# UBC-ECE-Sasha/PIM-Embedding-Lookup

Hardware: AMD Instinct MI355X
Metric: pooled-lookups/sec + achieved HBM GB/s, 26-table dim-16 Kaggle, 1/2/4/8 GPU (higher is better)
Workload: dtype f32

## Files before the change

include/pimemb.h:

```cpp
#ifndef PIMEMB_H
#define PIMEMB_H

#include <stddef.h>
#include <stdint.h>

#ifdef __cplusplus
extern "C" {
#endif

#define EMB_OK 0
#define EMB_ERR_INVALID (-1)
#define EMB_ERR_NOMEM (-2)
#define EMB_ERR_DEVICE (-3)
#define EMB_ERR_UNSUPPORTED (-4)
#define EMB_ERR_RANGE (-5)

typedef enum emb_dtype {
    EMB_F32 = 0,
    EMB_F16 = 1,
    EMB_FIXED32 = 2,
    EMB_BF16 = 3
} emb_dtype;
#define EMB_F8_E4M3 ((emb_dtype)8)
#define EMB_F8_E5M2 ((emb_dtype)9)
#define EMB_MXFP4 ((emb_dtype)10)
#define EMB_MXFP4_ROW_BYTES(dim) ((dim) / 2u + (dim) / 32u)
#define EMB_MXFP4_ROW_STRIDE(dim) ((EMB_MXFP4_ROW_BYTES(dim) + 15u) & ~15u)

typedef enum emb_index_type { EMB_IDX_U32 = 0, EMB_IDX_I64 = 1 } emb_index_type;

typedef enum emb_memspace {
    EMB_MEM_HOST = 0,
    EMB_MEM_DEVICE = 1
} emb_memspace;

typedef struct emb_engine emb_engine;
typedef struct emb_plan emb_plan;

typedef struct emb_config {
    int32_t device;
    uint32_t max_tables;
    uint32_t flags;
} emb_config;
#define EMB_FLAG_STAGE_TIMING 1u
#define EMB_FLAG_CHECK_INPUTS 2u
#define EMB_FLAG_DEFER_CHECK 4u

typedef struct emb_lookup_desc {
    uint32_t table_id;
    uint32_t fixed_pooling;
    const void *indices;
    const void *offsets;
    uint64_t n_indices;
    uint64_t n_bags;
    float *pooled;
} emb_lookup_desc;

typedef struct emb_stats {
    uint64_t n_lookup_calls;
    uint64_t n_kernel_launches;
    uint64_t n_bags;
    uint64_t n_indices;
    uint64_t table_bytes;
    double us_copy_in_indices;
    double us_copy_in_lengths;
    double us_launch;
    double us_copy_out;
    double us_post_process;
    double us_sync;
    uint64_t n_launches_by_kind[5];
} emb_stats;


const char *emb_last_error(void);

const char *emb_version(void);

int emb_create(const emb_config *cfg, emb_engine **out);

int emb_destroy(emb_engine *e);

int emb_load_table(emb_engine *e, uint32_t table_id, uint64_t nr_rows, uint32_t dim, emb_dtype dtype,
                   const void *rows, emb_memspace space);

int emb_alloc_table(emb_engine *e, uint32_t table_id, uint64_t nr_rows, uint32_t dim, emb_dtype dtype);

int emb_load_table_column(emb_engine *e, uint32_t table_id, uint32_t col, const int32_t *column,
                          uint64_t nr_rows);

int emb_set_hot_rows(emb_engine *e, uint32_t table_id, const uint64_t *row_ids, uint32_t n_rows);
int emb_learn_hot_rows(emb_engine *e, uint32_t table_id, const void *indices, uint64_t n_indices, emb_index_type itype,
                       emb_memspace space, uint32_t max_rows, float min_share, void *stream, uint32_t *n_chosen, float *share);

int emb_table_info(emb_engine *e, uint32_t table_id, void **device_rows, uint64_t *nr_rows,
                   uint32_t *dim, emb_dtype *dtype);

int emb_lookup(emb_engine *e, uint32_t table_id, const void *indices, uint64_t n_indices,
               const void *offsets, uint64_t n_bags, float *pooled, emb_index_type itype,
               emb_memspace space, void *stream);

int emb_lookup_batched(emb_engine *e, const emb_lookup_desc *descs, uint32_t n_descs,
                       emb_index_type itype, emb_memspace space, void *stream);

int emb_lookup_ranged(emb_engine *e, const emb_lookup_desc *descs, const uint64_t *row_lo, uint32_t n_descs, void *stream);
int emb_plan_create_ranged(emb_engine *e, const emb_lookup_desc *descs, const uint64_t *row_lo, uint32_t n_descs,
                           emb_plan **out);
#define EMB_SERVED_LANES 64u
#define EMB_SERVED_STRIDE 256u
#define EMB_SERVED_BYTES (EMB_SERVED_LANES * EMB_SERVED_STRIDE)
int emb_lookup_ranged_counted(emb_engine *e, const emb_lookup_desc *descs, const uint64_t *row_lo, uint32_t *const *served,
                              uint32_t n_descs, void *stream);
int emb_plan_create_ranged_counted(emb_engine *e, const emb_lookup_desc *descs, const uint64_t *row_lo,
                                   uint32_t *const *served, uint32_t n_descs, emb_plan **out);
#define EMB_RANGE_OPEN_END (1ull << 63)
int emb_lookup_ranged_typed(emb_engine *e, const emb_lookup_desc *descs, const uint64_t *row_lo, uint32_t *const *served,
                            uint32_t n_descs, emb_index_type itype, void *stream);
int emb_plan_create_ranged_typed(emb_engine *e, const emb_lookup_desc *descs, const uint64_t *row_lo, uint32_t *const *served,
                                 uint32_t n_descs, emb_index_type itype, emb_plan **out);

int emb_plan_create(emb_engine *e, const emb_lookup_desc *descs, uint32_t n_descs,
                    emb_index_type itype, emb_plan **out);
int emb_plan_launch(emb_plan *p, void *stream);
int emb_plan_destroy(emb_plan *p);
int emb_plan_bytes(const emb_plan *p, uint64_t *algorithmic_bytes, uint64_t *n_bags,
                   uint64_t *n_indices);
int emb_plan_signature(const emb_plan *p, uint64_t *signature);
int emb_plan_describe(const emb_plan *p, char *buf, size_t capacity);
int emb_plan_time(emb_plan *p, void *stream, uint32_t warmup, uint32_t iters, float *avg_us);

#define EMB_POOL_SUM 0u
#define EMB_POOL_MEAN 1u
#define EMB_POOL_MAX 2u
#define EMB_POOL_PADDING 1u
#define EMB_POOL_OUT_TABLE_DTYPE 2u
typedef struct emb_pool_spec {
    uint32_t mode;
    uint32_t flags;
    const float *per_sample_weights;
    int64_t padding_idx;
} emb_pool_spec;
int emb_lookup_pooled(emb_engine *e, const emb_lookup_desc *descs, const emb_pool_spec *pools, uint32_t n_descs,
                      emb_index_type itype, emb_memspace space, void *stream, uint32_t check, uint64_t *n_bad);
int emb_plan_create_pooled(emb_engine *e, const emb_lookup_desc *descs, const emb_pool_spec *pools, uint32_t n_descs,
                           emb_index_type itype, emb_plan **out);

int emb_validate_inputs(emb_engine *e, const emb_lookup_desc *descs, uint32_t n_descs,
                        emb_index_type itype, emb_memspace space, uint64_t *n_bad);
int emb_validate_inputs_on(emb_engine *e, const emb_lookup_desc *descs, uint32_t n_descs,
                           emb_index_type itype, emb_memspace space, void *stream, uint64_t *n_bad);
int emb_lookup_batched_checked(emb_engine *e, const emb_lookup_desc *descs, uint32_t n_descs,
                               emb_index_type itype, emb_memspace space, void *stream, uint64_t *n_bad);
int emb_lookup_batched_checked_deferred(emb_engine *e, const emb_lookup_desc *descs, uint32_t n_descs,
                                        emb_index_type itype, emb_memspace space, void *stream);
int emb_check_report(emb_engine *e, uint64_t *n_bad);

int emb_get_stats(emb_engine *e, emb_stats *out);
int emb_reset_stats(emb_engine *e);
int emb_set_stage_timing(emb_engine *e, int on);

#define EMB_STAGE_COPY_IN 0
#define EMB_STAGE_DESCRIPTORS 1
#define EMB_STAGE_LAUNCH 2
#define EMB_STAGE_COPY_OUT 3
#define EMB_STAGE_SYNC 4
typedef struct emb_trace_event {
    uint32_t stage;
    uint32_t call_id;
    double start_us;
    double stop_us;
} emb_trace_event;
int emb_trace_enable(emb_engine *e, uint32_t capacity);
int emb_trace_read(emb_engine *e, emb_trace_event *out, uint32_t max_events, uint32_t *n_events);

int emb_device_alloc(emb_engine *e, size_t bytes, void **out);
int emb_device_free(emb_engine *e, void *ptr);
int emb_copy_to_device(emb_engine *e, void *dst_device, const void *src_host, size_t bytes);
int emb_copy_to_host(emb_engine *e, void *dst_host, const void *src_device, size_t bytes);
int emb_memset_device(emb_engine *e, void *dst_device, int value, size_t bytes);
int emb_synchronize(emb_engine *e, void *stream);
int emb_stream_create(emb_engine *e, void **stream);
int emb_stream_destroy(emb_engine *e, void *stream);
int emb_device_of(emb_engine *e, int32_t *device);

typedef struct emb_queue emb_queue;
int emb_queue_create(emb_engine *e, emb_index_type itype, emb_memspace space, emb_queue **out);
int emb_queue_add(emb_queue *q, const emb_lookup_desc *descs, uint32_t n_descs, uint64_t *ticket);
int emb_queue_add_many(emb_queue *q, const emb_lookup_desc *descs, const uint32_t *n_descs, uint32_t n_requests,
                       uint64_t *first_ticket);
int emb_queue_flush(emb_queue *q, void *stream, uint32_t *n_requests);
int emb_queue_wait(emb_queue *q, uint64_t ticket);
int emb_queue_destroy(emb_queue *q);

typedef struct emb_route_table {
    const void *indices;
    const void *offsets;
    uint64_t n_indices;
    uint32_t fixed_pooling;
    uint32_t rows_per_shard;
} emb_route_table;
int emb_route_bags_sizes(uint32_t n_tables, uint64_t n_bags, uint64_t total_indices, uint32_t n_shards,
                         uint64_t *send_bytes, uint64_t *meta_bytes, uint64_t *slots_bytes, uint64_t *work_bytes);
int emb_route_bags(emb_engine *e, const emb_route_table *tables , uint32_t n_tables,
                   uint64_t n_bags, uint32_t n_shards, void *send, uint32_t *meta, uint32_t *slots,
                   void *work, void *stream);
int emb_route_bags_typed(emb_engine *e, const emb_route_table *tables , uint32_t n_tables,
                         emb_index_type itype, uint64_t n_bags, uint32_t n_shards, void *send, uint32_t *meta,
                         uint32_t *slots, void *work, void *stream);
int emb_unroute_bags(emb_engine *e, const float *recv, const uint32_t *meta, const uint32_t *slots,
                     uint32_t n_tables, uint64_t n_bags, uint32_t n_shards, uint32_t dim,
                     float *pooled , void *stream);

int emb_route_exchange_sizes(const uint32_t *sent, const uint32_t *received, uint32_t n_tables, uint32_t n_shards,
                             uint32_t dim, uint64_t *req_out_words, uint64_t *req_in_words, uint64_t *ret_rows_back,
                             uint64_t *ret_rows_served, uint64_t *peak_req_bytes, uint64_t *peak_ret_bytes);
int emb_route_serve_descs(const uint32_t *received, uint32_t n_tables, uint32_t n_shards, uint32_t dim,
                          const uint32_t *shard_table_ids, const void *req_recv, float *ret_send,
                          emb_lookup_desc *descs, uint32_t *n_descs, uint64_t *algorithmic_bytes);

typedef struct emb_comm emb_comm;
int emb_comm_unique_id(void *id128);
int emb_comm_create(emb_engine *e, const void *id128, int32_t rank, int32_t world, emb_comm **out);
int emb_comm_all_to_all(emb_comm *c, const void *send, const uint64_t *send_off, void *recv,
                        const uint64_t *recv_off, void *stream);
int emb_comm_destroy(emb_comm *c);

typedef struct emb_comm_op {
    int32_t peer;
    int32_t is_recv;
    void *ptr;
    uint64_t bytes;
} emb_comm_op;
int emb_comm_exchange(emb_comm *c, const emb_comm_op *ops, uint32_t n_ops, void *stream);
int emb_comm_rank(const emb_comm *c, int32_t *rank, int32_t *world);

typedef struct emb_peer emb_peer;
int emb_peer_create(emb_engine *e, const char *job_tag, int32_t rank, int32_t world, uint64_t arena_bytes, emb_peer **out);
int emb_peer_alloc(emb_peer *p, uint64_t bytes, void **ptr);
int emb_peer_info(emb_peer *p, int32_t *rank, int32_t *world, void **arena, uint64_t *arena_bytes, uint64_t *used,
                  int32_t *fine_grained);
int emb_peer_barrier(emb_peer *p);
int emb_peer_destroy(emb_peer *p);
int emb_peer_last_words(const char *line, int fd, int status);

typedef struct emb_shard emb_shard;
#define EMB_PLACE_REPLICATED 0u
#define EMB_PLACE_WHOLE 1u
#define EMB_PLACE_ROWS 2u
typedef struct emb_shard_table {
    uint32_t placement;
    int32_t owner;
    uint32_t engine_table;
    uint32_t rows_per_shard;
} emb_shard_table;
typedef struct emb_shard_input {
    const void *indices;
    const void *offsets;
    uint64_t n_indices;
    uint32_t fixed_pooling;
    uint32_t index_type;
    float *pooled;
} emb_shard_input;
#define EMB_SHARD_SELF_VIA_COMM 1u
#define EMB_SHARD_CHECK_SERVED 2u
#define EMB_SHARD_PEER_STORES 4u
#define EMB_SHARD_NO_DIRECT 8u
#define EMB_SHARD_DEFER_REPORT 16u
typedef struct emb_shard_config {
    uint32_t n_tables;
    uint32_t dim;
    uint32_t depth;
    uint32_t flags;
    const emb_shard_table *tables;
    emb_peer *peer;
} emb_shard_config;
typedef struct emb_shard_stats {
    uint64_t n_batches;
    uint64_t bytes_to_peers;
    uint64_t bytes_to_self;
    uint64_t served_algorithmic_bytes;
    uint64_t local_algorithmic_bytes;
    uint64_t served_sub_bags, served_indices;
    double us_host_submit;
    double us_host_wait_counts;
    double us_host_wait_served;
    double us_kernel_route, us_kernel_local, us_kernel_serve, us_kernel_unroute;
    uint64_t n_timed_batches;
    double us_kernel_direct;
} emb_shard_stats;
int emb_shard_create(emb_engine *e, emb_comm *comm, const emb_shard_config *cfg, emb_shard **out);
int emb_shard_submit(emb_shard *s, const emb_shard_input *in, uint64_t n_bags, void *stream, uint64_t *seq);
int emb_shard_flush(emb_shard *s);
int emb_shard_wait(emb_shard *s, uint64_t seq, void *stream);
int emb_shard_lookup(emb_shard *s, const emb_shard_input *in, uint64_t n_bags, void *stream);
int emb_shard_report(emb_shard *s);
int emb_shard_get_stats(emb_shard *s, emb_shard_stats *out, int reset);
int emb_shard_set_kernel_timing(emb_shard *s, int on);
int emb_shard_sent_counts(emb_shard *s, uint64_t seq, uint32_t *counts, uint32_t capacity_words);
int emb_shard_destroy(emb_shard *s);


struct dpu_set_t;

typedef struct dpu_runtime_totals {
    double execution_time_prepare;
    double execution_time_populate_copy_in;
    double execution_time_copy_in;
    double execution_time_copy_out;
    double execution_time_aggregate_result;
    double execution_time_launch;
} dpu_runtime_totals;

int emb_configure(uint32_t nr_tables, uint32_t nr_cols, uint32_t max_nr_batches,
                  uint32_t max_indices_per_batch);

struct dpu_set_t *populate_mram(uint32_t table_id, uint64_t nr_rows, uint32_t col,
                                int32_t *table_data, dpu_runtime_totals *runtime);

int32_t *lookup(uint32_t **indices, uint32_t **offsets, float **final_results,
                void *dpu_set_ptr_untyped, int64_t latency_print);

emb_engine *emb_compat_engine(void);
int emb_compat_reset(void);

#ifdef __cplusplus
}
#endif
#endif
```

pim-embedding-lookup_amd/csrc/pimemb_engine.cpp:

```cpp
#include <algorithm>
#include <atomic>
#include <chrono>
#include <condition_variable>
#include <cstdarg>
#include <cstdio>
#include <cstring>
#include <deque>
#include <map>
#include <mutex>
#include <new>
#include <string>
#include <thread>
#include <tuple>
#include <utility>
#include <unordered_map>
#include <vector>

#include "pimemb_hostcopy.h"
#include "pimemb_hot_rows.h"
#include "pimemb_internal.h"
#include "pimemb_xcd_map.h"

namespace pimemb {
hipError_t launch_store_word(volatile unsigned long long *dst, unsigned long long value, hipStream_t stream);
}
using pimemb::DevDesc;
using pimemb::KernelKind;
using pimemb::LaunchGeom;

namespace {

thread_local std::string g_last_error;
using pimemb::fail;

#define HIP_TRY(expr)                                                                       \
    do {                                                                                    \
        hipError_t _e = (expr);                                                             \
        if (_e != hipSuccess)                                                               \
            return fail(_e == hipErrorOutOfMemory ? EMB_ERR_NOMEM : EMB_ERR_DEVICE,         \
                        "%s failed: %s (%s:%d)", #expr, hipGetErrorString(_e), __FILE__,    \
                        __LINE__);                                                          \
    } while (0)
#define EMB_TRY(expr)                  \
    do {                               \
        int _rc = (expr);              \
        if (_rc != EMB_OK) return _rc; \
    } while (0)

double now_us() {
    using namespace std::chrono;
    return duration<double, std::micro>(steady_clock::now().time_since_epoch()).count();
}

size_t row_stride(int dtype, uint32_t dim) { return (size_t)pimemb::row_stride_bytes(dtype, dim); }
size_t index_size(emb_index_type t) { return t == EMB_IDX_I64 ? 8 : 4; }

struct Table {
    void *rows = nullptr;
    uint64_t nr_rows = 0;
    uint32_t dim = 0;
    int dtype = EMB_F32;
    LaunchGeom geom{};
    size_t bytes = 0;
    uint64_t generation = 0;
    void *hot_rows = nullptr;
    uint64_t *hot_hash = nullptr;
    uint32_t n_hot = 0, hot_log2 = 0;
    size_t hot_lds = 0;
};

struct DescSlot {
    char *h = nullptr;
    char *d = nullptr;
    size_t cap = 0;
    size_t used = 0;
    hipStream_t stream = nullptr;
    hipEvent_t done = nullptr;
    bool pending = false;
};
constexpr int kSlots = 4;
constexpr size_t kSlotBytes = 256u << 10;
constexpr int kRingPool = 8;
inline int ring_of_thread() {
    static const bool one = getenv("PIMEMB_RING_POOL") && atoi(getenv("PIMEMB_RING_POOL")) == 1;
    return one ? 0 : (int)(std::hash<std::thread::id>()(std::this_thread::get_id()) % (size_t)kRingPool);
}
struct ImageRing {
    DescSlot slots[kSlots];
    int next_slot = 0;
    int desc_mode = 1;
    unsigned slot_flags = 0;
    void release() {
        for (DescSlot &sl : slots) {
            if (sl.h) (void)hipHostFree(sl.h);
            if (sl.d) (void)hipFree(sl.d);
            if (sl.done) (void)hipEventDestroy(sl.done);
            sl = DescSlot{};
        }
    }
};

struct XmapCacheEntry {
    std::vector<uint64_t> key;
    uint32_t *d_map = nullptr;
    uint32_t xgrid = 0;
    bool direct = false;
    uint64_t last_use = 0;
    size_t bytes = 0;
    hipStream_t streams[4] = {};
    uint32_t n_streams = 0;
    bool many_streams = false;
};
struct XmapGrave {
    uint32_t *d_map = nullptr;
    size_t bytes = 0;
    hipEvent_t ev[4] = {};
    uint32_t n_ev = 0;
    bool needs_device_wait = false;
};
constexpr size_t kXmapCacheEntries = 32;
constexpr size_t kXmapSeenEntries = 256;
constexpr size_t kXmapGraveBytes = 64u << 20;

}

struct emb_engine {
    int device = 0;
    std::vector<Table> tables;
    std::mutex mu;
    std::mutex host_mu;
    pimemb::HostCopier copier;
    hipEvent_t pipe_ev[4] = {};
    hipStream_t host_s2 = nullptr;
    hipEvent_t split_ev[2] = {};
    ImageRing ring[kRingPool];
    std::mutex ring_mu[kRingPool];
    std::vector<XmapCacheEntry> xmap_cache;
    uint64_t xmap_clock = 0;
    std::vector<uint64_t> xmap_seen;
    size_t xmap_seen_at = 0;
    std::vector<XmapGrave> xmap_graveyard;
    size_t xmap_grave_bytes = 0;
    char *h_stage = nullptr;
    size_t h_stage_cap = 0;
    char *d_stage = nullptr;
    size_t d_stage_cap = 0;
    static constexpr uint32_t kValSlots = 64;
    pimemb::ValidateCtl *d_val = nullptr;
    unsigned long long val_seq = 0;
    struct PendingVerdict {
        unsigned long long seq;
        hipStream_t stream;
        uint32_t n_groups;
        KernelKind kinds[8];
        bool launched;
    };
    std::deque<PendingVerdict> val_pending;
    bool defer_check = false;
    unsigned long long val_owed_bad = 0, val_owed_first = 0;
    std::mutex val_mu;
    volatile unsigned long long *val_result = nullptr;
    volatile unsigned long long *host_done = nullptr;
    unsigned long long host_seq = 0;
    std::atomic<uint64_t> n_lookup_calls{0}, n_kernel_launches{0}, n_bags{0}, n_indices{0};
    std::atomic<uint64_t> n_by_kind[5] = {};
    uint64_t table_bytes = 0;
    double us_copy_in_indices = 0, us_copy_in_lengths = 0, us_launch = 0, us_copy_out = 0,
           us_sync = 0;
    bool stage_timing = false;
    bool check_inputs = false;
    std::atomic<uint32_t> live_plans{0};
    uint64_t next_generation = 1;
    std::deque<emb_trace_event> trace;
    uint32_t trace_cap = 0;
    uint32_t host_call_id = 0;
    void record(uint32_t stage, double a, double b) {
        if (!trace_cap) return;
        if (trace.size() >= trace_cap) trace.pop_front();
        trace.push_back(emb_trace_event{stage, host_call_id, a, b});
    }
};

struct PlanGroup {
    DevDesc *d_descs = nullptr;
    uint32_t n = 0;
    uint32_t max_tiles = 0;
    int dtype = EMB_F32;
    LaunchGeom geom{};
    KernelKind kind = pimemb::KERNEL_WAVEBATCH;
    uint32_t *d_xmap = nullptr;
    uint32_t xgrid = 0;
    bool xdirect = false;
    uint32_t hot_wgs = 0;
    uint32_t hot_lds = 0;
    uint32_t *cached_xmap = nullptr;
    bool ranged = false;
    uint32_t pool = 0;
    uint32_t n_weighted = 0, n_padding = 0;
    bool out_half = false;
    size_t desc_off = 0, xmap_off = 0;
    std::vector<uint32_t> xmap_words;
};

struct emb_plan {
    emb_engine *e = nullptr;
    emb_index_type itype = EMB_IDX_U32;
    std::vector<PlanGroup> groups;
    char *d_image = nullptr;
    uint64_t bytes = 0, n_bags = 0, n_indices = 0;
    uint64_t signature = 0;
    std::vector<std::pair<uint32_t, uint64_t>> table_gens;
};

namespace {

void clear_hot(Table &t) {
    if (t.hot_rows) (void)hipFree(t.hot_rows);
    if (t.hot_hash) (void)hipFree(t.hot_hash);
    t.hot_rows = nullptr;
    t.hot_hash = nullptr;
    t.n_hot = t.hot_log2 = 0;
    t.hot_lds = 0;
}

struct DeviceGuard {
    int prev = -1;
    bool switched = false;
    explicit DeviceGuard(int dev) {
        if (hipGetDevice(&prev) == hipSuccess && prev != dev) {
            switched = hipSetDevice(dev) == hipSuccess;
        }
    }
    ~DeviceGuard() {
        if (switched) (void)hipSetDevice(prev);
    }
};

struct Resolved {
    std::vector<DevDesc> descs;
    std::vector<PlanGroup> groups;
    uint64_t bytes = 0, n_bags = 0, n_indices = 0;
    std::vector<char> image;
    hipStream_t stream = nullptr;

    void build_image() {
        size_t off = 0, di = 0;
        for (PlanGroup &g : groups) {
            g.desc_off = off;
            off += sizeof(DevDesc) * g.n;
        }
        for (PlanGroup &g : groups) {
            g.xmap_off = off;
            off += (g.xmap_words.size() * 4 + 63) / 64 * 64;
        }
        image.assign(off ? off : 64, 0);
        for (PlanGroup &g : groups) {
            memcpy(image.data() + g.desc_off, descs.data() + di, sizeof(DevDesc) * g.n);
            di += g.n;
            if (!g.xmap_words.empty())
                memcpy(image.data() + g.xmap_off, g.xmap_words.data(), g.xmap_words.size() * 4);
        }
    }
    void bind(char *d_base) {
        for (PlanGroup &g : groups) {
            g.d_descs = reinterpret_cast<DevDesc *>(d_base + g.desc_off);
            g.d_xmap = g.cached_xmap ? g.cached_xmap
                       : g.xmap_words.empty() ? nullptr : reinterpret_cast<uint32_t *>(d_base + g.xmap_off);
        }
    }
};

void reap_xmap_graveyard(emb_engine *e, bool wait_oldest) {
    size_t kept = 0;
    for (size_t i = 0; i < e->xmap_graveyard.size(); i++) {
        XmapGrave &gv = e->xmap_graveyard[i];
        const bool over = wait_oldest && e->xmap_grave_bytes > kXmapGraveBytes;
        bool done = !gv.needs_device_wait;
        if (gv.needs_device_wait && over) done = hipDeviceSynchronize() == hipSuccess;
        for (uint32_t k = 0; k < gv.n_ev && done; k++) {
            hipError_t q = over ? hipEventSynchronize(gv.ev[k]) : hipEventQuery(gv.ev[k]);
            if (q != hipSuccess) {
                (void)hipGetLastError();
                done = false;
            }
        }
        if (done) {
            for (uint32_t k = 0; k < gv.n_ev; k++) (void)hipEventDestroy(gv.ev[k]);
            (void)hipFree(gv.d_map);
            e->xmap_grave_bytes -= gv.bytes;
        } else {
            e->xmap_graveyard[kept++] = gv;
        }
    }
    e->xmap_graveyard.resize(kept);
}

int cached_xcd_map(emb_engine *e, PlanGroup &g, uint32_t bpt, const std::vector<uint32_t> &tiles_of,
                   const std::vector<uint64_t> &bytes_of, hipStream_t stream) {
    std::vector<uint64_t> key;
    key.reserve(2 + 2 * tiles_of.size());
    key.push_back((uint64_t)g.kind);
    key.push_back(bpt);
    for (size_t i = 0; i < tiles_of.size(); i++) {
        key.push_back(tiles_of[i]);
        key.push_back(bytes_of[i]);
    }
    static const bool cache_off = getenv("PIMEMB_XMAP_CACHE") && atoi(getenv("PIMEMB_XMAP_CACHE")) == 0;
    if (cache_off) return EMB_ERR_UNSUPPORTED;
    std::lock_guard<std::mutex> lk(e->mu);
    ++e->xmap_clock;
    auto note_stream = [stream](XmapCacheEntry &c) {
        for (uint32_t k = 0; k < c.n_streams; k++)
            if (c.streams[k] == stream) return;
        if (c.n_streams < 4) c.streams[c.n_streams++] = stream;
        else c.many_streams = true;
    };
    for (XmapCacheEntry &c : e->xmap_cache)
        if (c.key == key) {
            c.last_use = e->xmap_clock;
            note_stream(c);
            g.cached_xmap = c.d_map;
            g.xgrid = c.xgrid;
            g.xdirect = c.direct;
            return EMB_OK;
        }
    uint64_t h = 1469598103934665603ull;
    for (uint64_t v : key) h = (h ^ v) * 1099511628211ull;
    bool seen = false;
    for (uint64_t v : e->xmap_seen) seen = seen || v == h;
    if (!seen) {
        if (e->xmap_seen.size() < kXmapSeenEntries) e->xmap_seen.push_back(h);
        else e->xmap_seen[e->xmap_seen_at++ % kXmapSeenEntries] = h;
        return EMB_ERR_UNSUPPORTED;
    }
    size_t victim = 0;
    if (e->xmap_cache.size() >= kXmapCacheEntries) {
        for (size_t i = 1; i < e->xmap_cache.size(); i++)
            if (e->xmap_cache[i].last_use < e->xmap_cache[victim].last_use) victim = i;
        if (e->xmap_clock - e->xmap_cache[victim].last_use < 4 * kXmapCacheEntries) return EMB_ERR_UNSUPPORTED;
    }
    XmapCacheEntry n;
    std::vector<uint32_t> words;
    n.xgrid = pimemb::build_xcd_map(tiles_of, bytes_of, &words, 1);
    if (n.xgrid <= (1u << 20)) {
        std::vector<uint32_t> direct;
        pimemb::expand_xcd_map(words, n.xgrid, &direct);
        words.swap(direct);
        n.direct = true;
    }
    if (hipMalloc((void **)&n.d_map, words.size() * 4) != hipSuccess) return EMB_ERR_NOMEM;
    if (hipMemcpy(n.d_map, words.data(), words.size() * 4, hipMemcpyHostToDevice) != hipSuccess) {
        (void)hipFree(n.d_map);
        return EMB_ERR_DEVICE;
    }
    if (e->xmap_cache.size() >= kXmapCacheEntries) {
        const XmapCacheEntry &v = e->xmap_cache[victim];
        XmapGrave gv;
        gv.d_map = v.d_map;
        gv.bytes = v.bytes;
        gv.needs_device_wait = v.many_streams;
        for (uint32_t k = 0; k < v.n_streams && !gv.needs_device_wait; k++) {
            hipEvent_t ev = nullptr;
            if (hipEventCreateWithFlags(&ev, hipEventDisableTiming) == hipSuccess && hipEventRecord(ev, v.streams[k]) == hipSuccess) {
                gv.ev[gv.n_ev++] = ev;
            } else {
                if (ev) (void)hipEventDestroy(ev);
                (void)hipGetLastError();
                gv.needs_device_wait = true;
            }
        }
        e->xmap_grave_bytes += gv.bytes;
        e->xmap_graveyard.push_back(gv);
        e->xmap_cache.erase(e->xmap_cache.begin() + (long)victim);
        reap_xmap_graveyard(e, true);
    }
    n.key.swap(key);
    n.bytes = words.size() * 4;
    note_stream(n);
    n.last_use = e->xmap_clock;
    g.cached_xmap = n.d_map;
    g.xgrid = n.xgrid;
    g.xdirect = n.direct;
    e->xmap_cache.push_back(std::move(n));
    return EMB_OK;
}

bool is_plain_sum(const emb_pool_spec &ps) {
    return ps.mode == EMB_POOL_SUM && ps.per_sample_weights == nullptr && ps.flags == 0;
}
bool is_plain_sum_half_out(const emb_pool_spec &ps) {
    return ps.mode == EMB_POOL_SUM && ps.per_sample_weights == nullptr && ps.flags == EMB_POOL_OUT_TABLE_DTYPE;
}
bool wants_half_out(const emb_pool_spec *pools, uint32_t i) { return pools && (pools[i].flags & EMB_POOL_OUT_TABLE_DTYPE) != 0; }
size_t out_elem_size(const emb_pool_spec *pools, uint32_t i) { return wants_half_out(pools, i) ? 2 : 4; }

int resolve(emb_engine *e, const emb_lookup_desc *descs, uint32_t n_descs, emb_index_type itype,
            const std::vector<const void *> *st_indices, const std::vector<const void *> *st_offsets,
            const std::vector<float *> *st_out, Resolved *r, bool cache_maps = false, const uint64_t *row_lo = nullptr,
            uint32_t *const *served = nullptr, const emb_pool_spec *pools = nullptr,
            const std::vector<const float *> *st_weights = nullptr) {
    if (itype != EMB_IDX_U32 && itype != EMB_IDX_I64) return fail(EMB_ERR_INVALID, "bad index type");
    std::map<std::tuple<int, uint32_t, uint32_t, uint32_t>, std::vector<uint32_t>> by_shape;
    for (uint32_t i = 0; i < n_descs; i++) {
        const emb_lookup_desc &u = descs[i];
        if (u.table_id >= e->tables.size() || e->tables[u.table_id].rows == nullptr)
            return fail(EMB_ERR_INVALID, "desc %u: table %u is not loaded", i, u.table_id);
        if (u.n_bags > 0 && u.pooled == nullptr) return fail(EMB_ERR_INVALID, "desc %u: pooled is NULL", i);
        if (u.n_indices > 0 && u.indices == nullptr)
            return fail(EMB_ERR_INVALID, "desc %u: indices is NULL", i);
        if (u.offsets == nullptr) {
            if (u.n_bags > 0 && u.fixed_pooling == 0)
                return fail(EMB_ERR_INVALID, "desc %u: offsets is NULL and fixed_pooling is 0", i);
            if ((uint64_t)u.fixed_pooling * u.n_bags != u.n_indices)
                return fail(EMB_ERR_INVALID, "desc %u: fixed_pooling*n_bags != n_indices", i);
        }
        const Table &t = e->tables[u.table_id];
        if (row_lo) {
            if (u.offsets != nullptr || u.fixed_pooling != 1)
                return fail(EMB_ERR_INVALID, "ranged lookup: desc %u: one index per bag only (offsets NULL, fixed_pooling 1)", i);
            if (t.geom.scalar_lanes)
                return fail(EMB_ERR_UNSUPPORTED, "ranged lookup: desc %u: rows must be 16-byte multiples up to 1 KiB", i);
            if (t.dtype == pimemb::kMXFP4)
                return fail(EMB_ERR_UNSUPPORTED, "ranged lookup: desc %u: table %u is MXFP4, which the lane-group kernels serve only "
                            "(no ranged, counted or typed lookup)", i, u.table_id);
        }
        uint32_t pool_kind = 0;
        if (pools && !is_plain_sum(pools[i])) {
            const emb_pool_spec &ps = pools[i];
            if (ps.mode > EMB_POOL_MAX || (ps.flags & ~(EMB_POOL_PADDING | EMB_POOL_OUT_TABLE_DTYPE)) != 0)
                return fail(EMB_ERR_INVALID, "desc %u: bad pooling spec (mode %u, flags 0x%x)", i, ps.mode, ps.flags);
            if ((ps.flags & EMB_POOL_OUT_TABLE_DTYPE) && t.dtype == pimemb::kMXFP4)
                return fail(EMB_ERR_UNSUPPORTED, "desc %u: EMB_POOL_OUT_TABLE_DTYPE: table %u is MXFP4, whose pooled rows are fp32 only", i, u.table_id);
            if ((ps.flags & EMB_POOL_OUT_TABLE_DTYPE) && t.dtype != EMB_F16 && t.dtype != EMB_BF16)
                return fail(EMB_ERR_UNSUPPORTED, "desc %u: EMB_POOL_OUT_TABLE_DTYPE needs an fp16 or bf16 table (table %u has dtype %d)", i,
                            u.table_id, (int)t.dtype);
            if (ps.per_sample_weights != nullptr && ps.mode != EMB_POOL_SUM)
                return fail(EMB_ERR_INVALID, "desc %u: per_sample_weights need EMB_POOL_SUM (as in torch)", i);
            if (t.dtype == EMB_FIXED32)
                return fail(EMB_ERR_UNSUPPORTED, "desc %u: fixed-point tables pool by plain sum only", i);
            if ((ps.flags & EMB_POOL_PADDING) && (ps.padding_idx < 0 || (uint64_t)ps.padding_idx >= t.nr_rows))
                return fail(EMB_ERR_INVALID, "desc %u: padding_idx %lld outside table %u (%llu rows)", i, (long long)ps.padding_idx,
                            u.table_id, (unsigned long long)t.nr_rows);
            if (row_lo) return fail(EMB_ERR_UNSUPPORTED, "ranged lookups pool by plain sum only");
            if (!is_plain_sum_half_out(ps)) pool_kind = 1u + ps.mode;
        }
        by_shape[{(int)t.dtype, t.dim, pool_kind, wants_half_out(pools, i) ? 1u : 0u}].push_back(i);
    }
    const size_t isz = index_size(itype);
    for (auto &kv : by_shape) {
        PlanGroup g;
        g.dtype = std::get<0>(kv.first);
        g.pool = std::get<2>(kv.first);
        g.out_half = std::get<3>(kv.first) != 0;
        g.n = (uint32_t)kv.second.size();
        const Table &t0 = e->tables[descs[kv.second[0]].table_id];
        g.geom = t0.geom;
        uint64_t group_bags = 0, group_idx = 0;
        for (uint32_t i : kv.second) {
            group_bags += descs[i].n_bags;
            group_idx += descs[i].n_indices;
        }
        g.kind = pimemb::choose_kernel(group_bags, group_idx, g.geom);
        {
            static const char *force = getenv("PIMEMB_FORCE_KERNEL");
            if (force && g.kind != pimemb::KERNEL_ANYDIM && group_idx <= 2 * group_bags)
                g.kind = force[0] == 'g' ? pimemb::KERNEL_GROUP : pimemb::KERNEL_WAVEBATCH;
        }
        if (g.dtype == pimemb::kMXFP4) g.kind = pimemb::KERNEL_GROUP;
        g.ranged = row_lo != nullptr;
        if (g.ranged && g.kind == pimemb::KERNEL_GROUP) g.kind = pimemb::KERNEL_WAVEBATCH;
        if (g.pool && g.kind == pimemb::KERNEL_WAVEBATCH2) g.kind = pimemb::KERNEL_WAVEBATCH;
        if (g.kind == pimemb::KERNEL_GROUP && !g.pool && !g.out_half) {
            for (uint32_t i : kv.second) {
                const Table &t = e->tables[descs[i].table_id];
                if (t.n_hot && t.hot_lds > g.hot_lds) g.hot_lds = (uint32_t)t.hot_lds;
            }
            if (g.hot_lds) g.kind = pimemb::KERNEL_HOT;
        }
        const uint32_t bpt = pimemb::bags_per_tile(g.kind, g.geom);
        std::vector<uint32_t> tiles_of;
        std::vector<uint64_t> bytes_of;
        for (uint32_t i : kv.second) {
            const emb_lookup_desc &u = descs[i];
            const Table &t = e->tables[u.table_id];
            uint64_t tiles = (u.n_bags + bpt - 1) / bpt;
            if (tiles > 0x0fffffffull) return fail(EMB_ERR_UNSUPPORTED, "desc %u: too many bags", i);
            DevDesc d{};
            d.weights = t.rows;
            d.indices = st_indices ? (*st_indices)[i] : u.indices;
            d.offsets = st_offsets ? (*st_offsets)[i] : u.offsets;
            d.out = st_out ? (*st_out)[i] : u.pooled;
            d.n_idx = u.n_indices;
            d.n_bags = u.n_bags;
            d.nr_rows = t.nr_rows;
            d.fixed_pooling = u.offsets ? 0u : u.fixed_pooling;
            d.n_tiles = (uint32_t)tiles;
            if (row_lo) d.ranged.row_lo = row_lo[i];
            if (row_lo && served) d.ranged.served = served[i];
            if (g.pool) {
                const emb_pool_spec &ps = pools[i];
                const bool weighted = ps.per_sample_weights != nullptr, padded = (ps.flags & EMB_POOL_PADDING) != 0;
                const uint32_t op = ps.mode == EMB_POOL_MAX ? pimemb::kPoolOpMax
                                    : !weighted          ? pimemb::kPoolOpAdd
                                    : padded             ? pimemb::kPoolOpMulAdd
                                                         : pimemb::kPoolOpFma;
                d.pool.weights = st_weights && weighted ? (*st_weights)[i] : ps.per_sample_weights;
                d.pool.padding_row = padded ? (uint64_t)ps.padding_idx : ~0ull;
                d.pool.op = op | (ps.mode == EMB_POOL_MEAN ? pimemb::kPoolMean : 0u);
                g.n_weighted += weighted;
                g.n_padding += padded;
                if (weighted) r->bytes += u.n_indices * 4;
            }
            if (g.kind == pimemb::KERNEL_HOT) {
                d.hot_rows = t.hot_rows;
                d.hot_hash = t.hot_hash;
                d.n_hot = t.n_hot;
                d.hot_log2 = t.hot_log2;
            }
            if (d.n_tiles > g.max_tiles) g.max_tiles = d.n_tiles;
            tiles_of.push_back(d.n_tiles);
            bytes_of.push_back(t.bytes);
            r->descs.push_back(d);
            r->n_bags += u.n_bags;
            r->n_indices += u.n_indices;
            r->bytes += u.n_indices * ((uint64_t)row_stride(t.dtype, t.dim) + isz) +
                        (u.offsets ? u.n_bags * isz : 0) + u.n_bags * (uint64_t)t.dim * (g.out_half ? 2 : 4);
        }
        if (g.n > 1 && g.max_tiles > 0 &&
            (g.kind == pimemb::KERNEL_WAVEBATCH || g.kind == pimemb::KERNEL_WAVEBATCH2)) {
            if (cache_maps)
                for (uint32_t &v : tiles_of)
                    if (v > 16) {
                        uint32_t q = 1;
                        while ((q << 1) <= v) q <<= 1;
                        q >>= 4;
                        v = (v + q - 1) / q * q;
                    }
            uint64_t total_tiles = 0;
            for (uint32_t t : tiles_of) total_tiles += t;
            if (total_tiles + 8 * (uint64_t)g.n > 0x7fffffffull)
                return fail(EMB_ERR_UNSUPPORTED, "launch too large for one grid");
            if (!cache_maps || cached_xcd_map(e, g, bpt, tiles_of, bytes_of, r->stream) != EMB_OK) {
                g.xgrid = pimemb::build_xcd_map(tiles_of, bytes_of, &g.xmap_words, 1);
                if (g.xgrid <= (1u << 20)) {
                    std::vector<uint32_t> direct;
                    pimemb::expand_xcd_map(g.xmap_words, g.xgrid, &direct);
                    g.xmap_words.swap(direct);
                    g.xdirect = true;
                }
            }
        } else if (g.n > 65535u) {
            return fail(EMB_ERR_UNSUPPORTED, "more than 65535 descriptors of one shape");
        }
        if (g.kind == pimemb::KERNEL_HOT) {
            static const uint32_t total = getenv("PIMEMB_HOT_WGS_TOTAL") ? (uint32_t)atoi(getenv("PIMEMB_HOT_WGS_TOTAL")) : 8192u;
            const uint32_t cap = g.max_tiles / 2u ? g.max_tiles / 2u : 1u;
            uint32_t w = total / g.n;
            g.hot_wgs = w < 1u ? 1u : (w > cap ? cap : w);
        }
        r->groups.push_back(std::move(g));
    }
    r->build_image();
    return EMB_OK;
}

int launch_groups(emb_engine *e, const std::vector<PlanGroup> &groups, emb_index_type itype,
                  hipStream_t s) {
    for (const PlanGroup &g : groups) {
        if (g.pool)
            HIP_TRY(pimemb::launch_bag_pool(g.d_descs, g.n, g.max_tiles, g.dtype, itype, g.geom, g.kind, g.d_xmap, g.xgrid,
                                            g.xdirect, s, g.out_half));
        else if (g.kind == pimemb::KERNEL_HOT)
            HIP_TRY(pimemb::launch_bag_sum_hot(g.d_descs, g.n, g.hot_wgs, g.hot_lds, g.dtype, itype, g.geom, s));
        else
            HIP_TRY(pimemb::launch_bag_sum(g.d_descs, g.n, g.max_tiles, g.dtype, itype, g.geom, g.kind, g.d_xmap,
                                           g.xgrid, g.xdirect, s, g.ranged, g.out_half));
        e->n_kernel_launches.fetch_add(1, std::memory_order_relaxed);
        e->n_by_kind[g.kind].fetch_add(1, std::memory_order_relaxed);
    }
    return EMB_OK;
}

int take_image_space(ImageRing &r, size_t n, hipStream_t s, char **h, char **d) {
    n = (n + 127) / 128 * 128;
    DescSlot *sl = &r.slots[r.next_slot];
    if (sl->used && (sl->used + n > sl->cap || sl->stream != s)) {
        if (hipEventRecord(sl->done, sl->stream) == hipSuccess) {
            sl->pending = true;
            r.next_slot = (r.next_slot + 1) % kSlots;
            sl = &r.slots[r.next_slot];
        } else {
            (void)hipGetLastError();
            HIP_TRY(hipDeviceSynchronize());
            sl->used = 0;
        }
    }
    if (sl->pending) {
        HIP_TRY(hipEventSynchronize(sl->done));
        sl->pending = false;
        sl->used = 0;
    }
    if (sl->cap < n) {
        if (sl->used) {
            HIP_TRY(hipDeviceSynchronize());
            sl->used = 0;
        }
        if (sl->h) (void)hipHostFree(sl->h);
        if (sl->d) (void)hipFree(sl->d);
        sl->h = nullptr;
        sl->d = nullptr;
        sl->cap = 0;
        const size_t cap = n < kSlotBytes ? kSlotBytes : n + n / 4;
        HIP_TRY(hipHostMalloc((void **)&sl->h, cap, r.slot_flags));
        if (r.desc_mode == 0) HIP_TRY(hipMalloc((void **)&sl->d, cap));
        sl->cap = cap;
    }
    if (!sl->done) HIP_TRY(hipEventCreateWithFlags(&sl->done, hipEventDisableTiming));
    *h = sl->h + sl->used;
    *d = sl->d ? sl->d + sl->used : nullptr;
    sl->used += n;
    sl->stream = s;
    return EMB_OK;
}

struct HostProfile {
    bool on = getenv("PIMEMB_HOST_PROFILE") != nullptr;
    double resolve = 0, slot = 0, image = 0, h2d = 0, launch = 0;
    uint64_t calls = 0;
};
HostProfile g_prof;

int launch_resolved(emb_engine *e, Resolved &r, emb_index_type itype, hipStream_t s,
                    bool descriptors_in_host_memory = false) {
    if (r.descs.empty()) return EMB_OK;
    const int rk = ring_of_thread();
    std::lock_guard<std::mutex> lk(e->ring_mu[rk]);
    const double p0 = g_prof.on ? now_us() : 0;
    char *h = nullptr, *d = nullptr;
    int rc = take_image_space(e->ring[rk], r.image.size(), s, &h, &d);
    if (rc) return rc;
    const double p1 = g_prof.on ? now_us() : 0;
    memcpy(h, r.image.data(), r.image.size());
    const double p2 = g_prof.on ? now_us() : 0;
    if (d == nullptr || descriptors_in_host_memory) {
        r.bind(h);
    } else {
        HIP_TRY(hipMemcpyAsync(d, h, r.image.size(), hipMemcpyHostToDevice, s));
        r.bind(d);
    }
    const double p3 = g_prof.on ? now_us() : 0;
    rc = launch_groups(e, r.groups, itype, s);
    if (rc) return rc;
    if (g_prof.on) {
        g_prof.slot += p1 - p0; g_prof.image += p2 - p1; g_prof.h2d += p3 - p2; g_prof.launch += now_us() - p3;
        g_prof.calls++;
    }
    return EMB_OK;
}

int ensure_stage(emb_engine *e, size_t h_bytes, size_t d_bytes) {
    if (e->h_stage_cap < h_bytes) {
        if (e->h_stage) (void)hipHostFree(e->h_stage);
        e->h_stage = nullptr;
        e->h_stage_cap = 0;
        size_t cap = h_bytes + h_bytes / 4 + 4096;
        HIP_TRY(hipHostMalloc((void **)&e->h_stage, cap, hipHostMallocMapped | hipHostMallocCoherent));
        e->h_stage_cap = cap;
    }
    if (e->d_stage_cap < d_bytes) {
        if (e->d_stage) (void)hipFree(e->d_stage);
        e->d_stage = nullptr;
        e->d_stage_cap = 0;
        size_t cap = d_bytes + d_bytes / 4 + 4096;
        HIP_TRY(hipMalloc((void **)&e->d_stage, cap));
        e->d_stage_cap = cap;
        if (cap >= (8u << 20) && !e->host_s2) {
            HIP_TRY(hipStreamCreateWithFlags(&e->host_s2, hipStreamNonBlocking));
            for (hipEvent_t &ev : e->split_ev)
                if (!ev) HIP_TRY(hipEventCreateWithFlags(&ev, hipEventDisableTiming));
            HIP_TRY(pimemb::launch_zero_words(reinterpret_cast<uint32_t *>(e->d_stage), 1, e->host_s2));
            HIP_TRY(hipStreamSynchronize(e->host_s2));
        }
    }
    return EMB_OK;
}

size_t align_up(size_t v, size_t a) { return (v + a - 1) / a * a; }

struct HostStage {
    std::vector<const void *> d_indices, d_offsets;
    std::vector<const float *> d_weights;
    std::vector<float *> d_out;
    size_t in_bytes = 0, out_bytes = 0;
    char *h_out = nullptr;
    bool zero_copy = false;
    bool h2d_deferred = false;
};

static const size_t kZeroCopyBytes = getenv("PIMEMB_ZERO_COPY_BYTES") ? strtoull(getenv("PIMEMB_ZERO_COPY_BYTES"), nullptr, 10) : (40u << 20);
static const size_t kStagedOutBytes = kZeroCopyBytes > (1u << 20) ? kZeroCopyBytes : (1u << 20);
static const size_t kFastPieceBytes = getenv("PIMEMB_FAST_PIECE_BYTES") ? strtoull(getenv("PIMEMB_FAST_PIECE_BYTES"), nullptr, 10) : 1500000;

static const size_t kSplitInBytes = getenv("PIMEMB_HOST_SPLIT_BYTES") ? strtoull(getenv("PIMEMB_HOST_SPLIT_BYTES"), nullptr, 10) : (1u << 20);

int stage_host_inputs(emb_engine *e, const emb_lookup_desc *descs, uint32_t n, emb_index_type itype,
                      hipStream_t s, HostStage *hs, bool with_outputs, bool allow_zero_copy = false, bool allow_split = false,
                      const emb_pool_spec *pools = nullptr) {
    const size_t isz = index_size(itype);
    size_t in_bytes = 0, out_bytes = 0, min_piece = SIZE_MAX;
    for (uint32_t i = 0; i < n; i++) {
        if (descs[i].table_id >= e->tables.size() || !e->tables[descs[i].table_id].rows)
            return fail(EMB_ERR_INVALID, "desc %u: table %u is not loaded", i, descs[i].table_id);
        in_bytes += align_up(descs[i].n_indices * isz, 16);
        if (descs[i].offsets) in_bytes += align_up(descs[i].n_bags * isz, 16);
        if (pools && pools[i].per_sample_weights) in_bytes += align_up(descs[i].n_indices * 4, 16);
        const size_t piece = descs[i].n_bags * (size_t)e->tables[descs[i].table_id].dim * out_elem_size(pools, i);
        out_bytes += align_up(piece, 16);
        if (piece && piece < min_piece) min_piece = piece;
    }
    const bool fast_pieces = min_piece != SIZE_MAX && min_piece >= kFastPieceBytes;
    if (!with_outputs) out_bytes = 0;
    const size_t h_out_bytes = (out_bytes <= kStagedOutBytes && !fast_pieces) ? out_bytes : 0;
    int rc = ensure_stage(e, in_bytes + h_out_bytes, in_bytes + out_bytes);
    if (rc) return rc;
    hs->h_out = h_out_bytes ? e->h_stage + in_bytes : nullptr;
    hs->zero_copy = allow_zero_copy && with_outputs && h_out_bytes == out_bytes && !fast_pieces &&
                    in_bytes + out_bytes <= kZeroCopyBytes;
    char *in_base = hs->zero_copy ? e->h_stage : e->d_stage;
    size_t off = 0;
    hs->d_indices.resize(n);
    hs->d_offsets.resize(n);
    hs->d_weights.assign(n, nullptr);
    hs->d_out.resize(n);
    std::vector<pimemb::CopyPiece> pack;
    pack.reserve(3 * n);
    for (uint32_t i = 0; i < n; i++) {
        const emb_lookup_desc &u = descs[i];
        if (u.n_indices && !u.indices) return fail(EMB_ERR_INVALID, "desc %u: indices is NULL", i);
        pack.push_back({e->h_stage + off, u.indices, u.n_indices * isz});
        hs->d_indices[i] = in_base + off;
        off += align_up(u.n_indices * isz, 16);
        if (u.offsets) {
            pack.push_back({e->h_stage + off, u.offsets, u.n_bags * isz});
            hs->d_offsets[i] = in_base + off;
            off += align_up(u.n_bags * isz, 16);
        } else {
            hs->d_offsets[i] = nullptr;
        }
        if (pools && pools[i].per_sample_weights) {
            pack.push_back({e->h_stage + off, pools[i].per_sample_weights, u.n_indices * 4});
            hs->d_weights[i] = reinterpret_cast<const float *>(in_base + off);
            off += align_up(u.n_indices * 4, 16);
        }
    }
    e->copier.copy(pack);
    size_t oo = in_bytes;
    for (uint32_t i = 0; i < n; i++) {
        hs->d_out[i] = reinterpret_cast<float *>((hs->zero_copy ? e->h_stage : e->d_stage) + oo);
        if (with_outputs)
            oo += align_up(descs[i].n_bags * (size_t)e->tables[descs[i].table_id].dim * out_elem_size(pools, i), 16);
    }
    hs->in_bytes = in_bytes;
    hs->out_bytes = out_bytes;
    hs->h2d_deferred = allow_split && !hs->zero_copy && with_outputs && fast_pieces && n >= 2 && in_bytes >= kSplitInBytes;
    if (in_bytes && !hs->zero_copy && !hs->h2d_deferred)
        HIP_TRY(hipMemcpyAsync(e->d_stage, e->h_stage, in_bytes, hipMemcpyHostToDevice, s));
    return EMB_OK;
}

constexpr size_t kPipelineBytes = 4u << 20;

int lookup_host_pipelined(emb_engine *e, const emb_lookup_desc *descs, uint32_t n, emb_index_type itype,
                          hipStream_t s, const HostStage &hs, double t0) {
    auto piece = [&](uint32_t i) { return descs[i].n_bags * (size_t)e->tables[descs[i].table_id].dim * 4; };
    const uint32_t parts = n < 4 ? n : 4;
    uint32_t bounds[5] = {0, 0, 0, 0, 0};
    {
        size_t acc = 0;
        uint32_t k = 1;
        for (uint32_t i = 0; i < n && k < parts; i++) {
            acc += piece(i);
            if (acc * parts >= hs.out_bytes * k && n - (i + 1) >= parts - k) bounds[k++] = i + 1;
        }
        for (; k < parts; k++) bounds[k] = bounds[k - 1] + 1;
        bounds[parts] = n;
    }
    uint64_t bags = 0, idx = 0;
    for (uint32_t k = 0; k < parts; k++) {
        const uint32_t lo = bounds[k], cnt = bounds[k + 1] - lo;
        std::vector<const void *> di(hs.d_indices.begin() + lo, hs.d_indices.begin() + lo + cnt);
        std::vector<const void *> dof(hs.d_offsets.begin() + lo, hs.d_offsets.begin() + lo + cnt);
        std::vector<float *> dout(hs.d_out.begin() + lo, hs.d_out.begin() + lo + cnt);
        Resolved r;
        r.stream = s;
        int rc = resolve(e, descs + lo, cnt, itype, &di, &dof, &dout, &r, true);
        if (rc == EMB_OK) rc = launch_resolved(e, r, itype, s, true);
        if (rc) {
            (void)hipStreamSynchronize(s);
            return rc;
        }
        if (!e->pipe_ev[k]) HIP_TRY(hipEventCreateWithFlags(&e->pipe_ev[k], hipEventDisableTiming));
        HIP_TRY(hipEventRecord(e->pipe_ev[k], s));
        bags += r.n_bags;
        idx += r.n_indices;
    }
    std::vector<pimemb::CopyPiece> unpack;
    for (uint32_t k = 0; k < parts; k++) {
        HIP_TRY(hipEventSynchronize(e->pipe_ev[k]));
        unpack.clear();
        for (uint32_t i = bounds[k]; i < bounds[k + 1]; i++)
            if (piece(i)) unpack.push_back({descs[i].pooled, hs.d_out[i], piece(i)});
        e->copier.copy(unpack);
    }
    e->us_sync += now_us() - t0;
    e->n_bags.fetch_add(bags, std::memory_order_relaxed);
    e->n_indices.fetch_add(idx, std::memory_order_relaxed);
    return EMB_OK;
}

int lookup_host_split(emb_engine *e, const emb_lookup_desc *descs, uint32_t n, emb_index_type itype, hipStream_t s, const HostStage &hs, double t0) {
    if (!e->host_s2) HIP_TRY(hipStreamCreateWithFlags(&e->host_s2, hipStreamNonBlocking));
    for (hipEvent_t &ev : e->split_ev)
        if (!ev) HIP_TRY(hipEventCreateWithFlags(&ev, hipEventDisableTiming));
    const char *in_base = e->d_stage;
    auto in_off = [&](uint32_t i) { return i < n ? (size_t)(static_cast<const char *>(hs.d_indices[i]) - in_base) : hs.in_bytes; };
    auto out_bytes_of = [&](uint32_t i) { return descs[i].n_bags * (double)e->tables[descs[i].table_id].dim * 4.0; };
    uint32_t m = 1;
    {
        double best = 1e300, out_a = 0;
        for (uint32_t c = 1; c < n; c++) {
            out_a += out_bytes_of(c - 1);
            const double in_a = (double)in_off(c), in_b = (double)hs.in_bytes - in_a, out_b = (double)hs.out_bytes - out_a;
            const double second_ready = in_b / 53e3 + 30.0, first_out = out_a / 46e3;
            const double total = in_a / 53e3 + 20.0 + (first_out > second_ready ? first_out : second_ready) + out_b / 46e3;
            if (total < best) {
                best = total;
                m = c;
            }
        }
    }
    const uint32_t bounds[3] = {0, m, n};
    hipStream_t on[2] = {s, e->host_s2};
    HIP_TRY(hipEventRecord(e->split_ev[0], s));
    HIP_TRY(hipStreamWaitEvent(e->host_s2, e->split_ev[0], 0));
    uint64_t bags = 0, idx = 0;
    for (uint32_t k = 0; k < 2; k++) {
        const uint32_t lo = bounds[k], cnt = bounds[k + 1] - lo;
        const size_t b0 = in_off(lo), b1 = in_off(bounds[k + 1]);
        int rc = EMB_OK;
        if (b1 > b0 && hipMemcpyAsync(e->d_stage + b0, e->h_stage + b0, b1 - b0, hipMemcpyHostToDevice, on[k]) != hipSuccess)
            rc = fail(EMB_ERR_DEVICE, "host-pointer call: copy-in of part %u failed: %s", k, hipGetErrorString(hipGetLastError()));
        std::vector<const void *> di(hs.d_indices.begin() + lo, hs.d_indices.begin() + lo + cnt);
        std::vector<const void *> dof(hs.d_offsets.begin() + lo, hs.d_offsets.begin() + lo + cnt);
        std::vector<float *> dout(hs.d_out.begin() + lo, hs.d_out.begin() + lo + cnt);
        Resolved r;
        r.stream = on[k];
        if (rc == EMB_OK) rc = resolve(e, descs + lo, cnt, itype, &di, &dof, &dout, &r, true);
        if (rc == EMB_OK) rc = launch_resolved(e, r, itype, on[k], false);
        if (rc) {
            (void)hipStreamSynchronize(s);
            (void)hipStreamSynchronize(e->host_s2);
            return rc;
        }
        bags += r.n_bags;
        idx += r.n_indices;
    }
    hipError_t err = hipEventRecord(e->split_ev[1], e->host_s2);
    for (uint32_t k = 0; k < 2 && err == hipSuccess; k++) {
        if (k == 1) err = hipStreamWaitEvent(s, e->split_ev[1], 0);
        for (uint32_t i = bounds[k]; i < bounds[k + 1] && err == hipSuccess; i++) {
            const size_t bytes = descs[i].n_bags * (size_t)e->tables[descs[i].table_id].dim * 4;
            if (bytes) err = hipMemcpyAsync(descs[i].pooled, hs.d_out[i], bytes, hipMemcpyDeviceToHost, s);
        }
    }
    if (err == hipSuccess) err = hipStreamSynchronize(s);
    if (err != hipSuccess) {
        (void)hipStreamSynchronize(e->host_s2);
        (void)hipStreamSynchronize(s);
        return fail(EMB_ERR_DEVICE, "host-pointer call (two parts): %s", hipGetErrorString(err));
    }
    e->us_sync += now_us() - t0;
    e->n_bags.fetch_add(bags, std::memory_order_relaxed);
    e->n_indices.fetch_add(idx, std::memory_order_relaxed);
    return EMB_OK;
}

int lookup_host(emb_engine *e, const emb_lookup_desc *descs, uint32_t n, emb_index_type itype,
                hipStream_t s, const emb_pool_spec *pools = nullptr) {
    std::lock_guard<std::mutex> host_lk(e->host_mu);
    const bool timed = e->stage_timing || e->trace_cap != 0;
    HostStage hs;
    const double t0 = now_us();
    {
        std::lock_guard<std::mutex> lk(e->mu);
        int rc = stage_host_inputs(e, descs, n, itype, s, &hs, true, true, !timed && !pools, pools);
        if (rc) return rc;
    }
    if (hs.h2d_deferred) return lookup_host_split(e, descs, n, itype, s, hs, t0);
    if (timed) HIP_TRY(hipStreamSynchronize(s));
    const double t1 = now_us();
    if (hs.zero_copy && !timed && hs.out_bytes >= kPipelineBytes && n >= 2 && !pools)
        return lookup_host_pipelined(e, descs, n, itype, s, hs, t0);
    Resolved r;
    r.stream = s;
    int rc = resolve(e, descs, n, itype, &hs.d_indices, &hs.d_offsets, &hs.d_out, &r, true, nullptr, nullptr,
                     pools, &hs.d_weights);
    if (rc) return rc;
    rc = launch_resolved(e, r, itype, s, hs.zero_copy);
    if (rc) return rc;
    const double t2 = now_us();
    if (timed) HIP_TRY(hipStreamSynchronize(s));
    const double t3 = now_us();
    const bool staged_out = hs.out_bytes > 0 && hs.out_bytes <= kStagedOutBytes && hs.h_out != nullptr;
    if (hs.zero_copy) {
    } else if (staged_out) {
        HIP_TRY(hipMemcpyAsync(hs.h_out, hs.d_out[0], hs.out_bytes, hipMemcpyDeviceToHost, s));
    } else {
        for (uint32_t i = 0; i < n; i++) {
            size_t bytes = descs[i].n_bags * (size_t)e->tables[descs[i].table_id].dim * out_elem_size(pools, i);
            if (bytes)
                HIP_TRY(hipMemcpyAsync(descs[i].pooled, hs.d_out[i], bytes, hipMemcpyDeviceToHost, s));
        }
    }
    const double t4 = now_us();
    if (hs.zero_copy && !timed) {
        if (!e->host_done) {
            void *p = nullptr;
            HIP_TRY(hipHostMalloc(&p, 64, hipHostMallocMapped | hipHostMallocCoherent));
            e->host_done = static_cast<volatile unsigned long long *>(p);
            *e->host_done = 0;
        }
        const unsigned long long seq = ++e->host_seq;
        HIP_TRY(pimemb::launch_store_word(e->host_done, seq, s));
        bool done = false;
        for (int spin = 0; spin < 400000 && !(done = *e->host_done == seq); spin++) {
        }
        if (!done) HIP_TRY(hipStreamSynchronize(s));
    } else {
        HIP_TRY(hipStreamSynchronize(s));
    }
    if (staged_out) {
        std::vector<pimemb::CopyPiece> unpack;
        unpack.reserve(n);
        for (uint32_t i = 0; i < n; i++) {
            size_t bytes = descs[i].n_bags * (size_t)e->tables[descs[i].table_id].dim * out_elem_size(pools, i);
            if (bytes)
                unpack.push_back({descs[i].pooled, hs.h_out + (reinterpret_cast<char *>(hs.d_out[i]) -
                                                                reinterpret_cast<char *>(hs.d_out[0])), bytes});
        }
        e->copier.copy(unpack);
    }
    const double t5 = now_us();
    if (timed) {
        e->us_copy_in_indices += t1 - t0;
        e->us_copy_in_lengths += t2 - t1;
        e->us_launch += t3 - t2;
        e->us_copy_out += t4 - t3;
        e->us_sync += t5 - t4;
        if (e->trace_cap) {
            std::lock_guard<std::mutex> lk(e->mu);
            e->record(EMB_STAGE_COPY_IN, t0, t1);
            e->record(EMB_STAGE_DESCRIPTORS, t1, t2);
            e->record(EMB_STAGE_LAUNCH, t2, t3);
            e->record(EMB_STAGE_COPY_OUT, t3, t4);
            e->record(EMB_STAGE_SYNC, t4, t5);
            e->host_call_id++;
        }
    } else {
        e->us_sync += t5 - t0;
    }
    e->n_bags.fetch_add(r.n_bags, std::memory_order_relaxed);
    e->n_indices.fetch_add(r.n_indices, std::memory_order_relaxed);
    return EMB_OK;
}

}

int pimemb::fail(int code, const char *fmt, ...) {
    char buf[512];
    va_list ap;
    va_start(ap, fmt);
    vsnprintf(buf, sizeof buf, fmt, ap);
    va_end(ap);
    g_last_error = buf;
    return code;
}

extern "C" {

const char *emb_last_error(void) { return g_last_error.c_str(); }

const char *emb_version(void) { return "pimemb 0.1 gfx950"; }

int emb_create(const emb_config *cfg, emb_engine **out) {
    if (!out) return fail(EMB_ERR_INVALID, "emb_create: out is NULL");
    *out = nullptr;
    int dev = cfg ? cfg->device : -1;
    int count = 0;
    HIP_TRY(hipGetDeviceCount(&count));
    if (count <= 0) return fail(EMB_ERR_DEVICE, "emb_create: no HIP device visible");
    if (dev < 0) HIP_TRY(hipGetDevice(&dev));
    if (dev >= count) return fail(EMB_ERR_INVALID, "emb_create: device %d of %d", dev, count);
    emb_engine *e = new (std::nothrow) emb_engine();
    if (!e) return fail(EMB_ERR_NOMEM, "emb_create: out of host memory");
    e->device = dev;
    e->stage_timing = cfg && (cfg->flags & EMB_FLAG_STAGE_TIMING);
    e->check_inputs = cfg && (cfg->flags & EMB_FLAG_CHECK_INPUTS);
    e->defer_check = cfg && (cfg->flags & EMB_FLAG_DEFER_CHECK);
    {
        const char *m = getenv("PIMEMB_DESC_MODE");
        for (ImageRing &rg : e->ring) {
            rg.desc_mode = (m && m[0] == 'c') ? 0 : 1;
            rg.slot_flags = hipHostMallocMapped | hipHostMallocCoherent;
        }
    }
    uint32_t max_tables = (cfg && cfg->max_tables) ? cfg->max_tables : 1024;
    e->tables.resize(max_tables);
    *out = e;
    return EMB_OK;
}

static int read_verdicts(emb_engine *e, bool wait, unsigned long long own_seq = 0, unsigned long long *own_bad = nullptr);

int emb_destroy(emb_engine *e) {
    if (!e) return EMB_OK;
    if (e->live_plans.load() != 0)
        return fail(EMB_ERR_INVALID, "emb_destroy: %u prepared plan(s) still reference this engine; destroy them first",
                    e->live_plans.load());
    DeviceGuard g(e->device);
    (void)hipDeviceSynchronize();
    {
        std::lock_guard<std::mutex> vlk(e->val_mu);
        if (!e->val_pending.empty()) (void)read_verdicts(e, true);
        if (e->val_owed_bad)
            fprintf(stderr, "[pimemb] emb_destroy: an unread verdict: %llu out-of-range indices / broken offsets in checked call number %llu\n",
                    e->val_owed_bad, e->val_owed_first);
    }
    if (g_prof.on && g_prof.calls) {
        const double n = (double)g_prof.calls;
        fprintf(stderr, "[pimemb host profile] %llu transient calls, us/call: resolve %.2f  slot %.2f  image memcpy %.2f  "
                        "h2d enqueue %.2f  kernel enqueue %.2f\n", (unsigned long long)g_prof.calls,
                g_prof.resolve / n, g_prof.slot / n, g_prof.image / n, g_prof.h2d / n, g_prof.launch / n);
    }
    for (Table &t : e->tables) {
        clear_hot(t);
        if (t.rows) (void)hipFree(t.rows);
    }
    for (ImageRing &rg : e->ring) rg.release();
    for (XmapCacheEntry &c : e->xmap_cache) (void)hipFree(c.d_map);
    for (XmapGrave &gv : e->xmap_graveyard) {
        for (uint32_t k = 0; k < gv.n_ev; k++) (void)hipEventDestroy(gv.ev[k]);
        (void)hipFree(gv.d_map);
    }
    for (hipEvent_t ev : e->pipe_ev)
        if (ev) (void)hipEventDestroy(ev);
    for (hipEvent_t ev : e->split_ev)
        if (ev) (void)hipEventDestroy(ev);
    if (e->host_s2) (void)hipStreamDestroy(e->host_s2);
    if (e->h_stage) (void)hipHostFree(e->h_stage);
    if (e->d_stage) (void)hipFree(e->d_stage);
    if (e->d_val) (void)hipFree(e->d_val);
    if (e->val_result) (void)hipHostFree(const_cast<unsigned long long *>(e->val_result));
    if (e->host_done) (void)hipHostFree(const_cast<unsigned long long *>(e->host_done));
    delete e;
    return EMB_OK;
}

static int alloc_table(emb_engine *e, uint32_t table_id, uint64_t nr_rows, uint32_t dim, int dtype,
                       bool zero_fill) {
    if (!e) return fail(EMB_ERR_INVALID, "engine is NULL");
    if (table_id >= e->tables.size())
        return fail(EMB_ERR_INVALID, "table id %u >= max_tables %zu", table_id, e->tables.size());
    if (nr_rows == 0) return fail(EMB_ERR_INVALID, "table %u: nr_rows is 0", table_id);
    LaunchGeom geom;
    int rc = pimemb::geometry_for(dtype, dim, &geom);
    if (dtype == pimemb::kMXFP4 && rc == EMB_ERR_INVALID)
        return fail(rc, "table %u: MXFP4 rows are blocks of 32 elements: dim %u is no multiple of 32", table_id, dim);
    if (dtype == pimemb::kMXFP4 && rc == EMB_ERR_UNSUPPORTED)
        return fail(rc, "table %u: MXFP4 tables take dim 32 .. 2048 (64 lanes per row), not %u", table_id, dim);
    if (rc == EMB_ERR_UNSUPPORTED)
        return fail(rc, "table %u: dim %u of dtype %d is not supported (dim must be > 0)", table_id, dim, (int)dtype);
    if (rc) return fail(rc, "table %u: bad dtype %d", table_id, (int)dtype);
    DeviceGuard g(e->device);
    std::lock_guard<std::mutex> lk(e->mu);
    Table &t = e->tables[table_id];
    size_t bytes = (size_t)nr_rows * row_stride(dtype, dim);
    if (t.n_hot) {
        HIP_TRY(hipDeviceSynchronize());
        clear_hot(t);
        t.generation = e->next_generation++;
    }
    if (t.rows && t.bytes != bytes) {
        HIP_TRY(hipDeviceSynchronize());
        HIP_TRY(hipFree(t.rows));
        e->table_bytes -= t.bytes;
        t = Table{};
    }
    if (!t.rows) {
        HIP_TRY(hipMalloc(&t.rows, bytes));
        e->table_bytes += bytes;
        t.generation = e->next_generation++;
    }
    if (zero_fill) HIP_TRY(hipMemset(t.rows, 0, bytes));
    if (t.nr_rows != nr_rows || t.dim != dim || t.dtype != dtype)
        t.generation = e->next_generation++;
    t.nr_rows = nr_rows;
    t.dim = dim;
    t.dtype = dtype;
    t.geom = geom;
    t.bytes = bytes;
    return EMB_OK;
}

int emb_alloc_table(emb_engine *e, uint32_t table_id, uint64_t nr_rows, uint32_t dim, emb_dtype dtype) {
    return alloc_table(e, table_id, nr_rows, dim, pimemb::dtype_value(dtype), true);
}

int emb_load_table(emb_engine *e, uint32_t table_id, uint64_t nr_rows, uint32_t dim, emb_dtype dtype,
                   const void *rows, emb_memspace space) {
    if (!rows) return fail(EMB_ERR_INVALID, "table %u: rows is NULL", table_id);
    int rc = alloc_table(e, table_id, nr_rows, dim, pimemb::dtype_value(dtype), false);
    if (rc) return rc;
    DeviceGuard g(e->device);
    Table &t = e->tables[table_id];
    HIP_TRY(hipMemcpy(t.rows, rows, t.bytes,
                      space == EMB_MEM_DEVICE ? hipMemcpyDeviceToDevice : hipMemcpyHostToDevice));
    return EMB_OK;
}

int emb_load_table_column(emb_engine *e, uint32_t table_id, uint32_t col, const int32_t *column,
                          uint64_t nr_rows) {
    if (!e || !column) return fail(EMB_ERR_INVALID, "engine or column is NULL");
    if (table_id >= e->tables.size() || !e->tables[table_id].rows)
        return fail(EMB_ERR_INVALID, "table %u is not allocated", table_id);
    Table &t = e->tables[table_id];
    if (t.dtype == pimemb::kMXFP4)
        return fail(EMB_ERR_UNSUPPORTED, "emb_load_table_column: table %u is MXFP4: a row interleaves 32-element blocks and their scales, it has no columns to load", table_id);
    if (t.dtype != EMB_FIXED32) return fail(EMB_ERR_INVALID, "table %u is not EMB_FIXED32", table_id);
    if (col >= t.dim) return fail(EMB_ERR_INVALID, "table %u: col %u >= dim %u", table_id, col, t.dim);
    if (nr_rows > t.nr_rows)
        return fail(EMB_ERR_INVALID, "table %u: %llu rows > allocated %llu", table_id,
                    (unsigned long long)nr_rows, (unsigned long long)t.nr_rows);
    DeviceGuard g(e->device);
    std::lock_guard<std::mutex> host_lk(e->host_mu);
    std::lock_guard<std::mutex> lk(e->mu);
    if (t.n_hot) {
        HIP_TRY(hipDeviceSynchronize());
        clear_hot(t);
        t.generation = e->next_generation++;
    }
    size_t bytes = nr_rows * sizeof(int32_t);
    int rc = ensure_stage(e, bytes, bytes);
    if (rc) return rc;
    std::vector<pimemb::CopyPiece> pack{{e->h_stage, column, bytes}};
    e->copier.copy(pack);
    HIP_TRY(hipMemcpyAsync(e->d_stage, e->h_stage, bytes, hipMemcpyHostToDevice, nullptr));
    HIP_TRY(pimemb::launch_scatter_column(static_cast<int32_t *>(t.rows),
                                          reinterpret_cast<const int32_t *>(e->d_stage), nr_rows,
                                          t.dim, col, nullptr));
    HIP_TRY(hipStreamSynchronize(nullptr));
    return EMB_OK;
}

int emb_set_hot_rows(emb_engine *e, uint32_t table_id, const uint64_t *row_ids, uint32_t n_rows) {
    if (!e) return fail(EMB_ERR_INVALID, "engine is NULL");
    if (table_id >= e->tables.size() || !e->tables[table_id].rows)
        return fail(EMB_ERR_INVALID, "table %u is not loaded", table_id);
    if (n_rows && !row_ids) return fail(EMB_ERR_INVALID, "row_ids is NULL");
    if (e->tables[table_id].dtype == pimemb::kMXFP4)
        return fail(EMB_ERR_UNSUPPORTED, "emb_set_hot_rows: table %u is MXFP4, which has no hot-row kernel", table_id);
    DeviceGuard g(e->device);
    std::lock_guard<std::mutex> lk(e->mu);
    Table &t = e->tables[table_id];
    HIP_TRY(hipDeviceSynchronize());
    clear_hot(t);
    t.generation = e->next_generation++;
    if (n_rows == 0) return EMB_OK;
    if (t.geom.scalar_lanes) return EMB_OK;
    const uint32_t row_bytes = t.geom.chunks * 16u;
    pimemb::HotSet hs = pimemb::build_hot_set(row_ids, n_rows, t.nr_rows, row_bytes, pimemb::kHotLdsBudget);
    if (hs.rows.empty()) return EMB_OK;
    HIP_TRY(hipMalloc(&t.hot_rows, hs.rows.size() * (size_t)row_bytes));
    hipError_t err = hipMalloc((void **)&t.hot_hash, hs.hash.size() * 8);
    {
        unsigned long long *d_ids = nullptr;
        std::vector<unsigned long long> ids(hs.rows.begin(), hs.rows.end());
        if (err == hipSuccess) err = hipMalloc((void **)&d_ids, ids.size() * 8);
        if (err == hipSuccess) err = hipMemcpy(d_ids, ids.data(), ids.size() * 8, hipMemcpyHostToDevice);
        if (err == hipSuccess) err = pimemb::launch_gather_rows(t.hot_rows, t.rows, d_ids, (uint32_t)ids.size(), row_bytes, nullptr);
        if (err == hipSuccess) err = hipStreamSynchronize(nullptr);
        if (d_ids) (void)hipFree(d_ids);
    }
    if (err == hipSuccess) err = hipMemcpy(t.hot_hash, hs.hash.data(), hs.hash.size() * 8, hipMemcpyHostToDevice);
    if (err != hipSuccess) {
        clear_hot(t);
        return fail(EMB_ERR_DEVICE, "emb_set_hot_rows: %s", hipGetErrorString(err));
    }
    t.n_hot = (uint32_t)hs.rows.size();
    t.hot_log2 = hs.log2size;
    t.hot_lds = hs.lds_bytes(row_bytes);
    return EMB_OK;
}

int emb_learn_hot_rows(emb_engine *e, uint32_t table_id, const void *indices, uint64_t n_indices, emb_index_type itype,
                       emb_memspace space, uint32_t max_rows, float min_share, void *stream, uint32_t *n_chosen, float *share) {
    if (!e) return fail(EMB_ERR_INVALID, "engine is NULL");
    if (table_id >= e->tables.size() || !e->tables[table_id].rows) return fail(EMB_ERR_INVALID, "table %u is not loaded", table_id);
    if (itype != EMB_IDX_U32 && itype != EMB_IDX_I64) return fail(EMB_ERR_INVALID, "bad index type");
    if (n_indices && !indices) return fail(EMB_ERR_INVALID, "emb_learn_hot_rows: indices is NULL");
    if (e->tables[table_id].dtype == pimemb::kMXFP4)
        return fail(EMB_ERR_UNSUPPORTED, "emb_learn_hot_rows: table %u is MXFP4, which has no hot-row kernel", table_id);
    if (n_chosen) *n_chosen = 0;
    if (share) *share = 0.f;
    constexpr uint64_t kRun = 65536, kRuns = 4;
    const size_t isz = index_size(itype);
    std::vector<char> host;
    uint64_t n_sample = 0;
    if (n_indices) {
        DeviceGuard g(e->device);
        const uint64_t runs = n_indices <= kRun * kRuns ? 1 : kRuns;
        const uint64_t len = runs == 1 ? n_indices : kRun;
        host.resize((size_t)(runs * len) * isz);
        hipStream_t s = static_cast<hipStream_t>(stream);
        for (uint64_t r = 0; r < runs; r++) {
            const uint64_t at = runs == 1 ? 0 : r * ((n_indices - len) / (runs - 1));
            const char *src = static_cast<const char *>(indices) + at * isz;
            if (space == EMB_MEM_DEVICE) HIP_TRY(hipMemcpyAsync(host.data() + (size_t)(r * len) * isz, src, (size_t)len * isz, hipMemcpyDeviceToHost, s));
            else memcpy(host.data() + (size_t)(r * len) * isz, src, (size_t)len * isz);
        }
        if (space == EMB_MEM_DEVICE) HIP_TRY(hipStreamSynchronize(s));
        n_sample = runs * len;
    }
    const uint64_t nr_rows = e->tables[table_id].nr_rows;
    std::unordered_map<uint64_t, uint32_t> count;
    count.reserve((size_t)std::min<uint64_t>(n_sample, 1u << 20));
    for (uint64_t i = 0; i < n_sample; i++) {
        const uint64_t id = itype == EMB_IDX_I64 ? (uint64_t)reinterpret_cast<const int64_t *>(host.data())[i]
                                                 : (uint64_t)reinterpret_cast<const uint32_t *>(host.data())[i];
        if (id < nr_rows) count[id]++;
    }
    std::vector<std::pair<uint32_t, uint64_t>> by_count;
    by_count.reserve(count.size());
    for (const auto &kv : count) by_count.emplace_back(kv.second, kv.first);
    const size_t k = std::min<size_t>(max_rows, by_count.size());
    std::partial_sort(by_count.begin(), by_count.begin() + (long)k, by_count.end(),
                      [](const std::pair<uint32_t, uint64_t> &a, const std::pair<uint32_t, uint64_t> &b) {
                          return a.first != b.first ? a.first > b.first : a.second < b.second;
                      });
    uint64_t covered = 0;
    std::vector<uint64_t> ids(k);
    for (size_t i = 0; i < k; i++) {
        ids[i] = by_count[i].second;
        covered += by_count[i].first;
    }
    const float sh = n_sample ? (float)((double)covered / (double)n_sample) : 0.f;
    if (share) *share = sh;
    if (k == 0 || sh < min_share) return emb_set_hot_rows(e, table_id, nullptr, 0);
    int rc = emb_set_hot_rows(e, table_id, ids.data(), (uint32_t)k);
    if (rc == EMB_OK && n_chosen) *n_chosen = e->tables[table_id].n_hot;
    return rc;
}

int emb_table_info(emb_engine *e, uint32_t table_id, void **device_rows, uint64_t *nr_rows,
                   uint32_t *dim, emb_dtype *dtype) {
    if (!e) return fail(EMB_ERR_INVALID, "engine is NULL");
    if (table_id >= e->tables.size() || !e->tables[table_id].rows)
        return fail(EMB_ERR_INVALID, "table %u is not loaded", table_id);
    const Table &t = e->tables[table_id];
    if (device_rows) *device_rows = t.rows;
    if (nr_rows) *nr_rows = t.nr_rows;
    if (dim) *dim = t.dim;
    if (dtype) pimemb::dtype_store(dtype, t.dtype);
    return EMB_OK;
}

static int validate_on(emb_engine *e, const emb_lookup_desc *descs, uint32_t n_descs, emb_index_type itype,
                       emb_memspace space, hipStream_t s, uint64_t *n_bad);
static int checked_launch(emb_engine *e, Resolved &r, emb_index_type itype, hipStream_t s, bool launch, uint64_t *n_bad, bool defer = false);

static int lookup_batched_impl(emb_engine *e, const emb_lookup_desc *descs, uint32_t n_descs, emb_index_type itype,
                               emb_memspace space, void *stream, bool check, uint64_t *n_bad, bool defer = false,
                               const emb_pool_spec *pools = nullptr) {
    if (n_bad) *n_bad = 0;
    if (!e) return fail(EMB_ERR_INVALID, "engine is NULL");
    if (n_descs == 0) return EMB_OK;
    if (!descs) return fail(EMB_ERR_INVALID, "descs is NULL");
    DeviceGuard g(e->device);
    hipStream_t s = static_cast<hipStream_t>(stream);
    e->n_lookup_calls.fetch_add(1, std::memory_order_relaxed);
    if (space == EMB_MEM_HOST) {
        if (check) {
            int vrc = validate_on(e, descs, n_descs, itype, space, s, n_bad);
            if (vrc) return vrc;
        }
        return lookup_host(e, descs, n_descs, itype, s, pools);
    }
    Resolved r;
    r.stream = s;
    const double p0 = g_prof.on ? now_us() : 0;
    int rc = resolve(e, descs, n_descs, itype, nullptr, nullptr, nullptr, &r, true, nullptr, nullptr, pools);
    if (rc) return rc;
    if (g_prof.on) g_prof.resolve += now_us() - p0;
    rc = check ? checked_launch(e, r, itype, s, true, n_bad, defer) : launch_resolved(e, r, itype, s);
    if (rc != EMB_OK && !(defer && rc == EMB_ERR_RANGE)) return rc;
    e->n_bags.fetch_add(r.n_bags, std::memory_order_relaxed);
    e->n_indices.fetch_add(r.n_indices, std::memory_order_relaxed);
    return rc;
}

int emb_lookup_batched(emb_engine *e, const emb_lookup_desc *descs, uint32_t n_descs,
                       emb_index_type itype, emb_memspace space, void *stream) {
    return lookup_batched_impl(e, descs, n_descs, itype, space, stream, e && e->check_inputs, nullptr, e && e->defer_check);
}

int emb_lookup_batched_checked_deferred(emb_engine *e, const emb_lookup_desc *descs, uint32_t n_descs,
                                        emb_index_type itype, emb_memspace space, void *stream) {
    return lookup_batched_impl(e, descs, n_descs, itype, space, stream, true, nullptr, space == EMB_MEM_DEVICE);
}

int emb_lookup_batched_checked(emb_engine *e, const emb_lookup_desc *descs, uint32_t n_descs,
                               emb_index_type itype, emb_memspace space, void *stream, uint64_t *n_bad) {
    return lookup_batched_impl(e, descs, n_descs, itype, space, stream, true, n_bad);
}

static const emb_pool_spec *live_pools(const emb_pool_spec *pools, uint32_t n_descs) {
    if (pools)
        for (uint32_t i = 0; i < n_descs; i++)
            if (!is_plain_sum(pools[i])) return pools;
    return nullptr;
}

int emb_lookup_pooled(emb_engine *e, const emb_lookup_desc *descs, const emb_pool_spec *pools, uint32_t n_descs,
                      emb_index_type itype, emb_memspace space, void *stream, uint32_t check, uint64_t *n_bad) {
    if (n_bad) *n_bad = 0;
    if (!e) return fail(EMB_ERR_INVALID, "engine is NULL");
    if (check > 2) return fail(EMB_ERR_INVALID, "emb_lookup_pooled: check must be 0, 1 or 2 (got %u)", check);
    if (n_descs && !descs) return fail(EMB_ERR_INVALID, "descs is NULL");
    const emb_pool_spec *live = live_pools(pools, n_descs);
    if (check == 0)
        return lookup_batched_impl(e, descs, n_descs, itype, space, stream, e->check_inputs, nullptr, e->defer_check, live);
    return lookup_batched_impl(e, descs, n_descs, itype, space, stream, true, n_bad, check == 2 && space == EMB_MEM_DEVICE, live);
}

int emb_lookup(emb_engine *e, uint32_t table_id, const void *indices, uint64_t n_indices,
               const void *offsets, uint64_t n_bags, float *pooled, emb_index_type itype,
               emb_memspace space, void *stream) {
    emb_lookup_desc d{};
    d.table_id = table_id;
    d.indices = indices;
    d.offsets = offsets;
    d.n_indices = n_indices;
    d.n_bags = n_bags;
    d.pooled = pooled;
    if (!offsets && n_bags) {
        if (n_indices % n_bags) return fail(EMB_ERR_INVALID, "offsets is NULL and n_indices %% n_bags != 0");
        d.fixed_pooling = (uint32_t)(n_indices / n_bags);
    }
    return emb_lookup_batched(e, &d, 1, itype, space, stream);
}

int emb_lookup_ranged(emb_engine *e, const emb_lookup_desc *descs, const uint64_t *row_lo, uint32_t n_descs, void *stream) {
    return emb_lookup_ranged_counted(e, descs, row_lo, nullptr, n_descs, stream);
}

int emb_lookup_ranged_counted(emb_engine *e, const emb_lookup_desc *descs, const uint64_t *row_lo, uint32_t *const *served,
                              uint32_t n_descs, void *stream) {
    return emb_lookup_ranged_typed(e, descs, row_lo, served, n_descs, EMB_IDX_U32, stream);
}

int emb_lookup_ranged_typed(emb_engine *e, const emb_lookup_desc *descs, const uint64_t *row_lo, uint32_t *const *served,
                            uint32_t n_descs, emb_index_type itype, void *stream) {
    if (!e) return fail(EMB_ERR_INVALID, "engine is NULL");
    if (n_descs == 0) return EMB_OK;
    if (!descs || !row_lo) return fail(EMB_ERR_INVALID, "emb_lookup_ranged: NULL argument");
    DeviceGuard g(e->device);
    Resolved r;
    r.stream = static_cast<hipStream_t>(stream);
    int rc = resolve(e, descs, n_descs, itype, nullptr, nullptr, nullptr, &r, true, row_lo, served);
    if (rc) return rc;
    rc = launch_resolved(e, r, itype, static_cast<hipStream_t>(stream));
    if (rc) return rc;
    e->n_lookup_calls.fetch_add(1, std::memory_order_relaxed);
    e->n_bags.fetch_add(r.n_bags, std::memory_order_relaxed);
    e->n_indices.fetch_add(r.n_indices, std::memory_order_relaxed);
    return EMB_OK;
}

static int plan_create(emb_engine *e, const emb_lookup_desc *descs, const uint64_t *row_lo, uint32_t *const *served,
                       uint32_t n_descs, emb_index_type itype, emb_plan **out, const emb_pool_spec *pools = nullptr);

int emb_plan_create_ranged(emb_engine *e, const emb_lookup_desc *descs, const uint64_t *row_lo, uint32_t n_descs,
                           emb_plan **out) {
    if (!row_lo) return fail(EMB_ERR_INVALID, "emb_plan_create_ranged: row_lo is NULL");
    return plan_create(e, descs, row_lo, nullptr, n_descs, EMB_IDX_U32, out);
}

int emb_plan_create_ranged_counted(emb_engine *e, const emb_lookup_desc *descs, const uint64_t *row_lo, uint32_t *const *served,
                                   uint32_t n_descs, emb_plan **out) {
    if (!row_lo) return fail(EMB_ERR_INVALID, "emb_plan_create_ranged_counted: row_lo is NULL");
    return plan_create(e, descs, row_lo, served, n_descs, EMB_IDX_U32, out);
}

int emb_plan_create_ranged_typed(emb_engine *e, const emb_lookup_desc *descs, const uint64_t *row_lo, uint32_t *const *served,
                                 uint32_t n_descs, emb_index_type itype, emb_plan **out) {
    if (!row_lo) return fail(EMB_ERR_INVALID, "emb_plan_create_ranged_typed: row_lo is NULL");
    return plan_create(e, descs, row_lo, served, n_descs, itype, out);
}

int emb_plan_create(emb_engine *e, const emb_lookup_desc *descs, uint32_t n_descs,
                    emb_index_type itype, emb_plan **out) {
    return plan_create(e, descs, nullptr, nullptr, n_descs, itype, out);
}

int emb_plan_create_pooled(emb_engine *e, const emb_lookup_desc *descs, const emb_pool_spec *pools, uint32_t n_descs,
                           emb_index_type itype, emb_plan **out) {
    return plan_create(e, descs, nullptr, nullptr, n_descs, itype, out, live_pools(pools, n_descs));
}

static int plan_create(emb_engine *e, const emb_lookup_desc *descs, const uint64_t *row_lo, uint32_t *const *served,
                       uint32_t n_descs, emb_index_type itype, emb_plan **out, const emb_pool_spec *pools) {
    if (!e || !out) return fail(EMB_ERR_INVALID, "engine or out is NULL");
    *out = nullptr;
    if (!descs || n_descs == 0) return fail(EMB_ERR_INVALID, "plan needs at least one descriptor");
    DeviceGuard g(e->device);
    Resolved r;
    int rc = resolve(e, descs, n_descs, itype, nullptr, nullptr, nullptr, &r, false, row_lo, served, pools);
    if (rc) return rc;
    emb_plan *p = new (std::nothrow) emb_plan();
    if (!p) return fail(EMB_ERR_NOMEM, "out of host memory");
    p->e = e;
    p->itype = itype;
    {
        uint64_t h = 1469598103934665603ull;
        auto mix = [&h](uint64_t v) { h = (h ^ v) * 1099511628211ull; };
        mix((uint64_t)itype);
        size_t di = 0;
        for (const PlanGroup &g : r.groups) {
            mix(g.kind); mix((uint64_t)g.dtype); mix(g.geom.lanes_per_row); mix(g.geom.chunks); mix(g.geom.scalar_lanes); mix(g.n); mix(g.max_tiles);
            mix(g.xgrid); mix(g.xdirect); mix(g.ranged); mix(g.hot_wgs); mix(g.hot_lds); mix(pimemb::bags_per_tile(g.kind, g.geom));
            if (g.pool) mix(0x706f6f6c00ull | g.pool);
            if (g.out_half) mix(0x6f757400ull | 1u);
            for (uint32_t w : g.xmap_words) mix(w);
            for (uint32_t i = 0; i < g.n; i++, di++) {
                const DevDesc &d = r.descs[di];
                mix(d.n_tiles); mix(d.n_bags); mix(d.n_idx); mix(d.nr_rows); mix(d.fixed_pooling); mix(d.offsets != nullptr); mix(d.n_hot);
                if (g.pool) {
                    mix(d.pool.weights != nullptr); mix(d.pool.padding_row); mix(d.pool.op);
                } else {
                    mix(d.ranged.row_lo); mix(d.ranged.served != nullptr);
                }
            }
        }
        p->signature = h;
    }
    p->bytes = r.bytes;
    p->n_bags = r.n_bags;
    p->n_indices = r.n_indices;
    char *d = nullptr;
    hipError_t err = hipMalloc((void **)&d, r.image.size());
    if (err == hipSuccess) err = hipMemcpy(d, r.image.data(), r.image.size(), hipMemcpyHostToDevice);
    if (err != hipSuccess) {
        if (d) (void)hipFree(d);
        delete p;
        return fail(EMB_ERR_DEVICE, "emb_plan_create: %s", hipGetErrorString(err));
    }
    r.bind(d);
    p->d_image = d;
    p->groups = r.groups;
    for (uint32_t i = 0; i < n_descs; i++)
        p->table_gens.emplace_back(descs[i].table_id, e->tables[descs[i].table_id].generation);
    e->live_plans.fetch_add(1);
    *out = p;
    return EMB_OK;
}

int emb_plan_launch(emb_plan *p, void *stream) {
    if (!p) return fail(EMB_ERR_INVALID, "plan is NULL");
    emb_engine *e = p->e;
    for (const auto &tg : p->table_gens)
        if (e->tables[tg.first].generation != tg.second)
            return fail(EMB_ERR_INVALID, "plan is stale: table %u was re-allocated after emb_plan_create", tg.first);
    DeviceGuard g(e->device);
    int rc = launch_groups(e, p->groups, p->itype, static_cast<hipStream_t>(stream));
    if (rc) return rc;
    e->n_lookup_calls.fetch_add(1, std::memory_order_relaxed);
    e->n_bags.fetch_add(p->n_bags, std::memory_order_relaxed);
    e->n_indices.fetch_add(p->n_indices, std::memory_order_relaxed);
    return EMB_OK;
}

int emb_plan_destroy(emb_plan *p) {
    if (!p) return EMB_OK;
    DeviceGuard g(p->e->device);
    (void)hipDeviceSynchronize();
    if (p->d_image) (void)hipFree(p->d_image);
    p->e->live_plans.fetch_sub(1);
    delete p;
    return EMB_OK;
}

int emb_plan_bytes(const emb_plan *p, uint64_t *algorithmic_bytes, uint64_t *n_bags,
                   uint64_t *n_indices) {
    if (!p) return fail(EMB_ERR_INVALID, "plan is NULL");
    if (algorithmic_bytes) *algorithmic_bytes = p->bytes;
    if (n_bags) *n_bags = p->n_bags;
    if (n_indices) *n_indices = p->n_indices;
    return EMB_OK;
}

int emb_plan_describe(const emb_plan *p, char *buf, size_t capacity) {
    if (!p || !buf || capacity == 0) return fail(EMB_ERR_INVALID, "emb_plan_describe: NULL argument");
    size_t at = 0;
    buf[0] = 0;
    for (const PlanGroup &g : p->groups) {
        const uint32_t block = g.kind == pimemb::KERNEL_ANYDIM ? 256u : (g.geom.lanes_per_row ? pimemb::bags_per_tile(g.kind, g.geom) : 0u);
        const int n = snprintf(buf + at, capacity - at, "%skind=%u dtype=%d itype=%d lanes_per_row=%u chunks=%u scalar_lanes=%u anydim_vec=%d ranged=%d descs=%u "
                               "grid=%u bags_per_tile=%u", at ? ";" : "", (unsigned)g.kind, (int)g.dtype, (int)p->itype, g.geom.lanes_per_row, g.geom.chunks,
                               g.geom.scalar_lanes, (int)g.geom.anydim_vec, (int)g.ranged, g.n, g.d_xmap ? g.xgrid : g.max_tiles * g.n, block);
        if (n < 0 || (size_t)n >= capacity - at) return fail(EMB_ERR_INVALID, "emb_plan_describe: %zu bytes do not hold the text", capacity);
        at += (size_t)n;
        if (g.pool) {
            const int m = snprintf(buf + at, capacity - at, " pool=%u weighted=%u padding=%u", g.pool - 1u, g.n_weighted, g.n_padding);
            if (m < 0 || (size_t)m >= capacity - at) return fail(EMB_ERR_INVALID, "emb_plan_describe: %zu bytes do not hold the text", capacity);
            at += (size_t)m;
        }
        if (g.out_half) {
            const int m = snprintf(buf + at, capacity - at, " out=1");
            if (m < 0 || (size_t)m >= capacity - at) return fail(EMB_ERR_INVALID, "emb_plan_describe: %zu bytes do not hold the text", capacity);
            at += (size_t)m;
        }
    }
    return EMB_OK;
}

int emb_plan_signature(const emb_plan *p, uint64_t *signature) {
    if (!p || !signature) return fail(EMB_ERR_INVALID, "emb_plan_signature: NULL argument");
    *signature = p->signature;
    return EMB_OK;
}

int emb_plan_time(emb_plan *p, void *stream, uint32_t warmup, uint32_t iters, float *avg_us) {
    if (!p || !avg_us || iters == 0) return fail(EMB_ERR_INVALID, "bad argument to emb_plan_time");
    DeviceGuard g(p->e->device);
    hipStream_t s = static_cast<hipStream_t>(stream);
    for (uint32_t i = 0; i < warmup; i++) {
        int rc = emb_plan_launch(p, stream);
        if (rc) return rc;
    }
    hipEvent_t a, b;
    HIP_TRY(hipEventCreate(&a));
    HIP_TRY(hipEventCreate(&b));
    HIP_TRY(hipEventRecord(a, s));
    for (uint32_t i = 0; i < iters; i++) {
        int rc = emb_plan_launch(p, stream);
        if (rc) return rc;
    }
    HIP_TRY(hipEventRecord(b, s));
    HIP_TRY(hipEventSynchronize(b));
    float ms = 0.f;
    HIP_TRY(hipEventElapsedTime(&ms, a, b));
    (void)hipEventDestroy(a);
    (void)hipEventDestroy(b);
    *avg_us = ms * 1000.f / (float)iters;
    return EMB_OK;
}

static void resync_validation(emb_engine *e) {
    (void)hipDeviceSynchronize();
    if (e->d_val) (void)hipMemset(e->d_val, 0, sizeof(pimemb::ValidateCtl) * emb_engine::kValSlots);
    e->val_pending.clear();
    (void)hipGetLastError();
}

static int read_verdicts(emb_engine *e, bool wait, unsigned long long own_seq, unsigned long long *own_bad) {
    if (own_bad) *own_bad = 0;
    while (!e->val_pending.empty()) {
        const emb_engine::PendingVerdict pv = e->val_pending.front();
        const uint32_t slot = (uint32_t)(pv.seq % emb_engine::kValSlots);
        volatile unsigned long long *result = e->val_result + slot;
        unsigned long long word = *result;
        if ((word >> 24) != pv.seq) {
            if (!wait) break;
            for (int spin = 0; spin < 200000 && ((word = *result) >> 24) != pv.seq; spin++) {
            }
            if ((word >> 24) != pv.seq) {
                if (hipStreamSynchronize(pv.stream) != hipSuccess) {
                    (void)hipGetLastError();
                    HIP_TRY(hipDeviceSynchronize());
                }
                if (((word = *result) >> 24) != pv.seq) {
                    resync_validation(e);
                    return fail(EMB_ERR_DEVICE, "validation kernel of checked call %llu did not report", pv.seq);
                }
            }
        }
        e->val_pending.pop_front();
        const unsigned long long bad = word & pimemb::kValCountMask;
        if (bad) {
            if (own_bad && pv.seq == own_seq) {
                *own_bad = bad;
            } else {
                if (!e->val_owed_bad) e->val_owed_first = pv.seq;
                e->val_owed_bad += bad;
            }
            if (pv.launched) {
                e->n_kernel_launches.fetch_sub(pv.n_groups, std::memory_order_relaxed);
                for (uint32_t g = 0; g < pv.n_groups && g < 8; g++) e->n_by_kind[pv.kinds[g]].fetch_sub(1, std::memory_order_relaxed);
            }
        }
    }
    return EMB_OK;
}

static int checked_launch(emb_engine *e, Resolved &r, emb_index_type itype, hipStream_t s, bool launch, uint64_t *n_bad, bool defer) {
    if (n_bad) *n_bad = 0;
    if (r.descs.empty()) return EMB_OK;
    if (r.descs.size() > 65535u) return fail(EMB_ERR_UNSUPPORTED, "a checked call takes at most 65535 descriptors (%zu given)", r.descs.size());
    std::lock_guard<std::mutex> vlk(e->val_mu);
    unsigned long long seq = 0;
    if (defer && !e->val_pending.empty()) EMB_TRY(read_verdicts(e, false));
    if (e->val_pending.size() + 1 >= emb_engine::kValSlots) EMB_TRY(read_verdicts(e, true));
    volatile unsigned long long *result = nullptr;
    uint32_t slot = 0;
    {
        const int rk = ring_of_thread();
        std::lock_guard<std::mutex> lk(e->ring_mu[rk]);
        if (!e->d_val) {
            HIP_TRY(hipMalloc((void **)&e->d_val, sizeof(pimemb::ValidateCtl) * emb_engine::kValSlots));
            HIP_TRY(hipMemset(e->d_val, 0, sizeof(pimemb::ValidateCtl) * emb_engine::kValSlots));
        }
        if (!e->val_result) {
            void *p = nullptr;
            HIP_TRY(hipHostMalloc(&p, 8 * emb_engine::kValSlots, hipHostMallocMapped | hipHostMallocCoherent));
            memset(p, 0, 8 * emb_engine::kValSlots);
            e->val_result = static_cast<volatile unsigned long long *>(p);
        }
        seq = ++e->val_seq;
        slot = (uint32_t)(seq % emb_engine::kValSlots);
        result = e->val_result + slot;
        char *h = nullptr, *d = nullptr;
        int rc = take_image_space(e->ring[rk], r.image.size(), s, &h, &d);
        if (rc) return rc;
        memcpy(h, r.image.data(), r.image.size());
        char *base = h;
        if (d != nullptr) {
            HIP_TRY(hipMemcpyAsync(d, h, r.image.size(), hipMemcpyHostToDevice, s));
            base = d;
        }
        r.bind(base);
        uint64_t max_items = 1;
        for (const DevDesc &dd : r.descs) max_items = std::max<uint64_t>(max_items, std::max<uint64_t>(dd.n_idx, dd.n_bags));
        const uint32_t wgs = pimemb::validate_workgroups(max_items, itype);
        hipError_t err = pimemb::launch_validate(reinterpret_cast<DevDesc *>(base + r.groups[0].desc_off), (uint32_t)r.descs.size(),
                                                 itype, e->d_val + slot, const_cast<unsigned long long *>(result), seq, wgs,
                                                 launch, s);
        if (err != hipSuccess) {
            resync_validation(e);
            return fail(EMB_ERR_DEVICE, "validation kernel: %s", hipGetErrorString(err));
        }
        if (launch) {
            rc = launch_groups(e, r.groups, itype, s);
            if (rc) {
                resync_validation(e);
                return rc;
            }
        }
        emb_engine::PendingVerdict pv{seq, s, (uint32_t)r.groups.size(), {}, launch};
        for (size_t g = 0; g < r.groups.size() && g < 8; g++) pv.kinds[g] = r.groups[g].kind;
        e->val_pending.push_back(pv);
    }
    unsigned long long bad = 0;
    if (!defer) EMB_TRY(read_verdicts(e, true, seq, &bad));
    const unsigned long long earlier_bad = e->val_owed_bad, earlier_seq = e->val_owed_first;
    e->val_owed_bad = e->val_owed_first = 0;
    if (n_bad) *n_bad = bad + earlier_bad;
    if (bad) {
        if (earlier_bad)
            return fail(EMB_ERR_RANGE, "%llu out-of-range indices / broken offsets (and %llu in EARLIER checked calls whose verdict was deferred, "
                        "the first of them number %llu of this engine)", bad, earlier_bad, earlier_seq);
        return fail(EMB_ERR_RANGE, "%llu out-of-range indices / broken offsets", bad);
    }
    if (earlier_bad)
        return fail(EMB_ERR_RANGE, "%llu out-of-range indices / broken offsets in an EARLIER checked call (number %llu of this engine; its "
                    "lookup was disarmed on the device: outputs untouched) -- reported now: the verdict was deferred", earlier_bad, earlier_seq);
    return EMB_OK;
}

static int validate_on(emb_engine *e, const emb_lookup_desc *descs, uint32_t n_descs, emb_index_type itype,
                       emb_memspace space, hipStream_t s, uint64_t *n_bad) {
    HostStage hs;
    Resolved r;
    r.stream = s;
    int rc;
    std::unique_lock<std::mutex> host_lk(e->host_mu, std::defer_lock);
    if (space == EMB_MEM_HOST) host_lk.lock();
    std::vector<emb_lookup_desc> tmp(descs, descs + n_descs);
    for (uint32_t i = 0; i < n_descs; i++)
        if (!tmp[i].pooled) tmp[i].pooled = (float *)16;
    if (space == EMB_MEM_HOST) {
        {
            std::lock_guard<std::mutex> lk(e->mu);
            rc = stage_host_inputs(e, descs, n_descs, itype, s, &hs, false);
        }
        if (rc) return rc;
        rc = resolve(e, tmp.data(), n_descs, itype, &hs.d_indices, &hs.d_offsets, nullptr, &r, true);
    } else {
        rc = resolve(e, tmp.data(), n_descs, itype, nullptr, nullptr, nullptr, &r, true);
    }
    if (rc) return rc;
    return checked_launch(e, r, itype, s, false, n_bad);
}

int emb_validate_inputs(emb_engine *e, const emb_lookup_desc *descs, uint32_t n_descs,
                        emb_index_type itype, emb_memspace space, uint64_t *n_bad) {
    return emb_validate_inputs_on(e, descs, n_descs, itype, space, nullptr, n_bad);
}

int emb_validate_inputs_on(emb_engine *e, const emb_lookup_desc *descs, uint32_t n_descs, emb_index_type itype,
                           emb_memspace space, void *stream, uint64_t *n_bad) {
    if (!e || !descs) return fail(EMB_ERR_INVALID, "engine or descs is NULL");
    DeviceGuard g(e->device);
    return validate_on(e, descs, n_descs, itype, space, static_cast<hipStream_t>(stream), n_bad);
}

int emb_check_report(emb_engine *e, uint64_t *n_bad) {
    if (n_bad) *n_bad = 0;
    if (!e) return fail(EMB_ERR_INVALID, "engine is NULL");
    DeviceGuard g(e->device);
    std::lock_guard<std::mutex> vlk(e->val_mu);
    EMB_TRY(read_verdicts(e, true));
    const unsigned long long bad = e->val_owed_bad, first = e->val_owed_first;
    e->val_owed_bad = e->val_owed_first = 0;
    if (n_bad) *n_bad = bad;
    if (bad)
        return fail(EMB_ERR_RANGE, "%llu out-of-range indices / broken offsets in checked call number %llu of this engine (its lookup was "
                    "disarmed on the device: outputs untouched)", bad, first);
    return EMB_OK;
}

int emb_get_stats(emb_engine *e, emb_stats *out) {
    if (!e || !out) return fail(EMB_ERR_INVALID, "engine or out is NULL");
    memset(out, 0, sizeof *out);
    out->n_lookup_calls = e->n_lookup_calls.load();
    out->n_kernel_launches = e->n_kernel_launches.load();
    out->n_bags = e->n_bags.load();
    out->n_indices = e->n_indices.load();
    out->table_bytes = e->table_bytes;
    out->us_copy_in_indices = e->us_copy_in_indices;
    out->us_copy_in_lengths = e->us_copy_in_lengths;
    out->us_launch = e->us_launch;
    out->us_copy_out = e->us_copy_out;
    out->us_post_process = 0.0;
    out->us_sync = e->us_sync;
    for (int k = 0; k < 5; k++) out->n_launches_by_kind[k] = e->n_by_kind[k].load();
    return EMB_OK;
}

int emb_reset_stats(emb_engine *e) {
    if (!e) return fail(EMB_ERR_INVALID, "engine is NULL");
    e->n_lookup_calls = 0;
    e->n_kernel_launches = 0;
    e->n_bags = 0;
    e->n_indices = 0;
    for (auto &k : e->n_by_kind) k = 0;
    e->us_copy_in_indices = e->us_copy_in_lengths = e->us_launch = e->us_copy_out = e->us_sync = 0;
    return EMB_OK;
}

int emb_set_stage_timing(emb_engine *e, int on) {
    if (!e) return fail(EMB_ERR_INVALID, "engine is NULL");
    e->stage_timing = on != 0;
    return EMB_OK;
}

int emb_trace_enable(emb_engine *e, uint32_t capacity) {
    if (!e) return fail(EMB_ERR_INVALID, "engine is NULL");
    std::lock_guard<std::mutex> lk(e->mu);
    e->trace_cap = capacity;
    e->trace.clear();
    e->host_call_id = 0;
    return EMB_OK;
}

int emb_trace_read(emb_engine *e, emb_trace_event *out, uint32_t max_events, uint32_t *n_events) {
    if (!e || !n_events || (max_events && !out)) return fail(EMB_ERR_INVALID, "bad argument to emb_trace_read");
    std::lock_guard<std::mutex> lk(e->mu);
    uint32_t n = 0;
    while (n < max_events && !e->trace.empty()) {
        out[n++] = e->trace.front();
        e->trace.pop_front();
    }
    *n_events = n;
    return EMB_OK;
}

int emb_device_alloc(emb_engine *e, size_t bytes, void **out) {
    if (!e || !out) return fail(EMB_ERR_INVALID, "engine or out is NULL");
    DeviceGuard g(e->device);
    *out = nullptr;
    HIP_TRY(hipMalloc(out, bytes ? bytes : 16));
    return EMB_OK;
}

int emb_device_free(emb_engine *e, void *ptr) {
    if (!e) return fail(EMB_ERR_INVALID, "engine is NULL");
    if (!ptr) return EMB_OK;
    DeviceGuard g(e->device);
    HIP_TRY(hipFree(ptr));
    return EMB_OK;
}

int emb_copy_to_device(emb_engine *e, void *dst_device, const void *src_host, size_t bytes) {
    if (!e) return fail(EMB_ERR_INVALID, "engine is NULL");
    if (!bytes) return EMB_OK;
    DeviceGuard g(e->device);
    HIP_TRY(hipMemcpy(dst_device, src_host, bytes, hipMemcpyHostToDevice));
    return EMB_OK;
}

int emb_copy_to_host(emb_engine *e, void *dst_host, const void *src_device, size_t bytes) {
    if (!e) return fail(EMB_ERR_INVALID, "engine is NULL");
    if (!bytes) return EMB_OK;
    DeviceGuard g(e->device);
    HIP_TRY(hipMemcpy(dst_host, src_device, bytes, hipMemcpyDeviceToHost));
    return EMB_OK;
}

int emb_memset_device(emb_engine *e, void *dst_device, int value, size_t bytes) {
    if (!e) return fail(EMB_ERR_INVALID, "engine is NULL");
    if (!bytes) return EMB_OK;
    DeviceGuard g(e->device);
    HIP_TRY(hipMemset(dst_device, value, bytes));
    return EMB_OK;
}

int emb_stream_create(emb_engine *e, void **stream) {
    if (!e || !stream) return fail(EMB_ERR_INVALID, "engine or stream is NULL");
    DeviceGuard g(e->device);
    hipStream_t st = nullptr;
    HIP_TRY(hipStreamCreateWithFlags(&st, hipStreamNonBlocking));
// ... 492 lines not shown
```

pim-embedding-lookup_amd/csrc/pimemb_hot_rows.h:

```cpp
#pragma once

#include <stdint.h>

#include <unordered_set>
#include <vector>

namespace pimemb {

struct HotSet {
    std::vector<uint64_t> rows;
    std::vector<uint64_t> hash;
    uint32_t log2size = 0;
    size_t lds_bytes(uint32_t row_bytes) const { return rows.size() * (size_t)row_bytes + hash.size() * 8; }
};

inline HotSet build_hot_set(const uint64_t *ids, uint32_t n, uint64_t nr_rows, uint32_t row_bytes,
                            size_t lds_budget) {
    HotSet hs;
    if (n == 0 || row_bytes == 0) return hs;
    size_t max_rows = lds_budget / ((size_t)row_bytes + 64);
    if (max_rows > n) max_rows = n;
    if (max_rows == 0) return hs;
    uint32_t log2 = 2;
    while ((1ull << log2) < 4 * max_rows) log2++;
    while (max_rows && max_rows * (size_t)row_bytes + (8ull << log2) > lds_budget) max_rows--;
    const uint32_t mask = (1u << log2) - 1u;
    hs.log2size = log2;
    hs.hash.assign((size_t)1 << log2, ~0ull);
    std::unordered_set<uint64_t> seen;
    for (uint32_t i = 0; i < n && hs.rows.size() < max_rows; i++) {
        const uint64_t r = ids[i];
        if (r >= nr_rows || r >= 0xffffffffull || !seen.insert(r).second) continue;
        const uint32_t key = (uint32_t)r, home = (key * 0x9E3779B1u) >> (32u - log2);
        for (uint32_t p = 0; p < 2; p++) {
            uint64_t &e = hs.hash[(home + p) & mask];
            if (e == ~0ull) {
                e = ((uint64_t)hs.rows.size() << 32) | key;
                hs.rows.push_back(r);
                break;
            }
        }
    }
    if (hs.rows.empty()) {
        hs.hash.clear();
        hs.log2size = 0;
    }
    return hs;
}

}
```

pim-embedding-lookup_amd/engine.py:

```python
from __future__ import annotations

import ctypes as C
import struct
import threading
from typing import Sequence

import numpy as np

from . import lib as _l

_NP_TABLE_DTYPES = {np.dtype(np.float32): _l.EMB_F32, np.dtype(np.float16): _l.EMB_F16,
                    np.dtype(np.int32): _l.EMB_FIXED32}
POOL_MODES = {"sum": _l.EMB_POOL_SUM, "mean": _l.EMB_POOL_MEAN, "max": _l.EMB_POOL_MAX}
_HALF_OUT_NP = {_l.EMB_F16: np.dtype(np.float16), _l.EMB_BF16: np.dtype(np.uint16)}
_HALF_OUT_TORCH = {_l.EMB_F16: "torch.float16", _l.EMB_BF16: "torch.bfloat16"}
_F8_TORCH = {_l.EMB_F8_E4M3: "float8_e4m3fn", _l.EMB_F8_E5M2: "float8_e5m2"}


_MARSHAL = [False]


def _marshal():
    m = _MARSHAL[0]
    if m is False:
        import importlib.util
        import os
        m = None
        path = os.path.join(os.path.dirname(os.path.abspath(__file__)), "lib", "_pimemb_marshal.so")
        if os.path.exists(path) and os.environ.get("PIMEMB_NO_MARSHAL") != "1":
            import torch
            try:
                spec = importlib.util.spec_from_file_location("_pimemb_marshal", path)
                m = importlib.util.module_from_spec(spec)
                spec.loader.exec_module(m)
            except (ImportError, OSError) as ex:
                import warnings
                warnings.warn(f"_pimemb_marshal.so could not be loaded ({ex}); tensor lists are unpacked in Python")
                m = None
        _MARSHAL[0] = m
    return m


def _is_torch(x) -> bool:
    return type(x).__module__.startswith("torch") and hasattr(x, "data_ptr")


def _index_type_of(dtype) -> int:
    name = str(dtype).replace("torch.", "")
    if name in ("uint32", "int32"):
        return _l.EMB_IDX_U32
    if name == "int64":
        return _l.EMB_IDX_I64
    raise TypeError(f"indices/offsets must be uint32/int32 or int64, got {dtype}")


def _check_half_out(out, table_dtype: int | None = None, table_id=None) -> None:
    name = str(getattr(out, "dtype", type(out).__name__))
    if table_dtype is None:
        ok = name.replace("torch.", "") in ("float16", "bfloat16", "uint16")
        want = "a 2-byte table dtype"
    else:
        want = _HALF_OUT_TORCH[table_dtype] if _is_torch(out) else str(_HALF_OUT_NP[table_dtype])
        ok = name == want
    if not ok:
        where = "" if table_id is None else f"table {table_id}: "
        raise TypeError(f'{where}out_dtype="table" needs an output of {want}, got {name}')


def _half_out_list(out_dtype, n: int, outs=None) -> list | None:
    if out_dtype is None:
        return None
    per = [out_dtype] * n if isinstance(out_dtype, str) else list(out_dtype)
    if len(per) != n or any(v not in (None, "table") for v in per):
        raise ValueError('out_dtype must be None or "table" (or one of those per table)')
    half = [v == "table" for v in per]
    if outs is not None:
        for h, o in zip(half, outs):
            if h:
                _check_half_out(o)
    return half if any(half) else None


class DeviceBuffer:

    def __init__(self, engine: "EmbeddingEngine", nbytes: int, dtype=np.uint8, shape=None):
        self.engine = engine
        self.nbytes = int(nbytes)
        self.dtype = np.dtype(dtype)
        self.shape = tuple(shape) if shape is not None else (self.nbytes // self.dtype.itemsize,)
        p = C.c_void_p()
        _l.check(engine._L.emb_device_alloc(engine._h, self.nbytes, C.byref(p)))
        self.ptr = p.value

    @classmethod
    def from_numpy(cls, engine: "EmbeddingEngine", a: np.ndarray) -> "DeviceBuffer":
        a = np.ascontiguousarray(a)
        buf = cls(engine, a.nbytes, a.dtype, a.shape)
        if a.nbytes:
            _l.check(engine._L.emb_copy_to_device(engine._h, buf.ptr, a.ctypes.data, a.nbytes))
        return buf

    def numpy(self) -> np.ndarray:
        out = np.empty(self.shape, dtype=self.dtype)
        if out.nbytes:
            _l.check(self.engine._L.emb_copy_to_host(self.engine._h, out.ctypes.data, self.ptr, out.nbytes))
        return out

    def fill(self, byte: int = 0) -> None:
        _l.check(self.engine._L.emb_memset_device(self.engine._h, self.ptr, byte, self.nbytes))

    def free(self) -> None:
        if self.ptr and self.engine._h:
            self.engine._L.emb_device_free(self.engine._h, self.ptr)
        self.ptr = None

    def __len__(self):
        return self.shape[0]


class _Arg:
    __slots__ = ("ptr", "space", "n", "dtype", "keep")

    def __init__(self, x):
        if x is None:
            self.ptr, self.space, self.n, self.dtype, self.keep = None, None, 0, None, None
        elif isinstance(x, DeviceBuffer):
            self.ptr, self.space, self.n, self.dtype, self.keep = x.ptr, _l.EMB_MEM_DEVICE, x.shape[0], x.dtype, x
        elif _is_torch(x):
            if not x.is_contiguous():
                raise ValueError("torch tensors passed to the engine must be contiguous")
            space = _l.EMB_MEM_DEVICE if x.is_cuda else _l.EMB_MEM_HOST
            self.ptr, self.space, self.n, self.dtype, self.keep = x.data_ptr(), space, x.shape[0], x.dtype, x
        else:
            a = np.ascontiguousarray(x)
            self.ptr, self.space, self.n, self.dtype, self.keep = a.ctypes.data, _l.EMB_MEM_HOST, a.shape[0], a.dtype, a


def _current_stream_for(*objs) -> int | None:
    for o in objs:
        if _is_torch(o) and o.is_cuda:
            import torch
            return torch.cuda.current_stream(o.device).cuda_stream
    return None


class Plan:

    def __init__(self, engine: "EmbeddingEngine", handle: int, outputs, keep):
        self.engine, self._p, self.outputs, self._keep = engine, handle, outputs, keep

    def launch(self, stream: int | None = None) -> None:
        _l.check(self.engine._L.emb_plan_launch(self._p, stream))

    def bytes(self) -> tuple[int, int, int]:
        b, nb, ni = C.c_uint64(), C.c_uint64(), C.c_uint64()
        _l.check(self.engine._L.emb_plan_bytes(self._p, C.byref(b), C.byref(nb), C.byref(ni)))
        return b.value, nb.value, ni.value

    def time_us(self, warmup: int = 5, iters: int = 20, stream: int | None = None) -> float:
        us = C.c_float()
        _l.check(self.engine._L.emb_plan_time(self._p, stream, warmup, iters, C.byref(us)))
        return us.value

    def signature(self) -> int:
        v = C.c_uint64()
        _l.check(self.engine._L.emb_plan_signature(self._p, C.byref(v)))
        return v.value

    def describe(self) -> list[dict]:
        buf = C.create_string_buffer(4096)
        _l.check(self.engine._L.emb_plan_describe(self._p, buf, len(buf)))
        return [{k: int(v) for k, v in (kv.split("=") for kv in rec.split())} for rec in buf.value.decode().split(";") if rec]

    def destroy(self) -> None:
        if self._p:
            self.engine._L.emb_plan_destroy(self._p)
            self._p = None


class RequestQueue:

    def __init__(self, engine: "EmbeddingEngine", itype: int = _l.EMB_IDX_U32, space: int = _l.EMB_MEM_HOST):
        self.engine, self._L, self.itype, self.space = engine, engine._L, itype, space
        h = C.c_void_p()
        _l.check(self._L.emb_queue_create(engine._h, itype, space, C.byref(h)))
        self._h = h
        self._keep = {}

    def descriptors(self, table_ids, indices, offsets, outs, fixed_pooling=0):
        arr, n, itype, space, results, keep = self.engine._descs(table_ids, indices, offsets, outs, fixed_pooling)
        if itype != self.itype or space != self.space:
            raise TypeError("request buffers do not match the queue's index width / memory space")
        return arr, n, results, keep

    def add(self, table_ids, indices, offsets, outs, fixed_pooling=0) -> int:
        arr, n, _res, keep = self.descriptors(table_ids, indices, offsets, outs, fixed_pooling)
        t = self.add_descriptors(arr, n)
        self._keep[t] = keep
        return t

    def add_descriptors(self, arr, n: int) -> int:
        t = C.c_uint64()
        _l.check(self._L.emb_queue_add(self._h, arr, n, C.byref(t)))
        return t.value

    def add_many(self, arr, counts) -> int:
        t = C.c_uint64()
        _l.check(self._L.emb_queue_add_many(self._h, arr, counts, len(counts), C.byref(t)))
        return t.value

    def flush(self, stream: int | None = None) -> int:
        n = C.c_uint32()
        _l.check(self._L.emb_queue_flush(self._h, stream, C.byref(n)))
        return n.value

    def wait(self, ticket: int) -> None:
        _l.check(self._L.emb_queue_wait(self._h, ticket))
        self._keep.pop(ticket, None)

    def close(self) -> None:
        if self._h:
            self._L.emb_queue_destroy(self._h)
            self._h = None


class NativeExchange:

    def __init__(self, engine: "EmbeddingEngine", rank: int, world: int, broadcast):
        self._L = engine._L
        buf = C.create_string_buffer(128)
        if rank == 0:
            _l.check(self._L.emb_comm_unique_id(buf))
        uid = broadcast(buf.raw)
        self._h = C.c_void_p()
        _l.check(self._L.emb_comm_create(engine._h, C.create_string_buffer(uid, 128), rank, world, C.byref(self._h)))
        self.world = world
        self._offs = {}

    def offsets(self, offsets):
        return self._arr(offsets)

    def _arr(self, offsets):
        if isinstance(offsets, C.Array):
            return offsets
        key = tuple(int(x) for x in offsets)
        a = self._offs.get(key)
        if a is None:
            if len(key) != self.world + 1:
                raise ValueError("need world+1 byte offsets")
            a = self._offs[key] = (C.c_uint64 * len(key))(*key)
        return a

    def all_to_all(self, send_ptr: int, send_off, recv_ptr: int, recv_off, stream: int | None = None) -> None:
        _l.check(self._L.emb_comm_all_to_all(self._h, send_ptr, self._arr(send_off), recv_ptr, self._arr(recv_off), stream))

    def close(self) -> None:
        if self._h:
            self._L.emb_comm_destroy(self._h)
            self._h = None


class EmbeddingEngine:

    def __init__(self, device: int = -1, max_tables: int = 1024, lib_path: str | None = None,
                 check_inputs: bool | str = False):
        self._L = _l.load(lib_path)
        flags = _l.EMB_FLAG_CHECK_INPUTS if check_inputs else 0
        if check_inputs == "deferred":
            flags |= _l.EMB_FLAG_DEFER_CHECK
        cfg = _l.EmbConfig(device, max_tables, flags)
        h = C.c_void_p()
        _l.check(self._L.emb_create(C.byref(cfg), C.byref(h)))
        self._h = h.value
        self._tables: dict[int, tuple[int, int, int]] = {}
        self._tls = threading.local()
        self._plan_lock = threading.Lock()
        self._plan_cache: dict[tuple, list] = {}
        self._plan_seen: dict[int, int] = {}
        self._plan_clock = 0
        self._plan_last_evict = -(1 << 30)
        self.plan_cache_size = 16
        self._check_inputs = bool(check_inputs)
        if self._check_inputs:
            self.plan_cache_size = 0
        self._same_dim: dict[tuple, int] = {}
        self.plan_cache_hits = 0

    def load_table(self, table_id: int, rows, dtype: int | None = None) -> None:
        if isinstance(rows, (tuple, list)) and len(rows) == 2:
            rows, dtype = self._fuse_mxfp4_pair(rows[0], rows[1], dtype), _l.EMB_MXFP4
        if _is_torch(rows):
            import torch
            tmap = {torch.float32: _l.EMB_F32, torch.float16: _l.EMB_F16, torch.int32: _l.EMB_FIXED32,
                    torch.bfloat16: _l.EMB_BF16, torch.float8_e4m3fn: _l.EMB_F8_E4M3, torch.float8_e5m2: _l.EMB_F8_E5M2}
            dt = tmap[rows.dtype] if dtype is None else dtype
            if not rows.is_contiguous():
                rows = rows.contiguous()
            space = _l.EMB_MEM_DEVICE if rows.is_cuda else _l.EMB_MEM_HOST
            if rows.is_cuda:
                torch.cuda.current_stream(rows.device).synchronize()
            ptr, shape = rows.data_ptr(), tuple(rows.shape)
        else:
            rows = np.ascontiguousarray(rows)
            dt = _NP_TABLE_DTYPES[rows.dtype] if dtype is None else dtype
            space, ptr, shape = _l.EMB_MEM_HOST, rows.ctypes.data, rows.shape
        if len(shape) != 2:
            raise ValueError("table must be 2-D [nr_rows, dim]")
        if dt == _l.EMB_MXFP4:
            from .formats import mxfp4_dim_of_stride
            if str(rows.dtype).replace("torch.", "") != "uint8":
                raise TypeError(f"an MXFP4 table is uint8 fused rows or an (elements, scales) pair, not {rows.dtype}")
            shape = (shape[0], mxfp4_dim_of_stride(shape[1]))
        _l.check(self._L.emb_load_table(self._h, table_id, shape[0], shape[1], dt, ptr, space))
        self._tables[table_id] = (shape[0], shape[1], dt)
        self._same_dim.clear()

    @staticmethod
    def _fuse_mxfp4_pair(elements, scales, dtype):
        if dtype not in (None, _l.EMB_MXFP4):
            raise TypeError("an (elements, scales) pair is an MXFP4 table: dtype is EMB_MXFP4 or left out")
        from .formats import mxfp4_join, mxfp4_row_stride
        if not (_is_torch(elements) and _is_torch(scales)):
            if _is_torch(elements) or _is_torch(scales):
                raise TypeError("MXFP4 pair: both numpy arrays or both torch tensors")
            if dtype is None:
                raise TypeError("a pair of plain uint8 arrays is an MXFP4 table only when dtype=EMB_MXFP4 says so")
            return mxfp4_join(elements, scales)
        import torch
        typed = elements.dtype == torch.float4_e2m1fn_x2 and scales.dtype == torch.float8_e8m0fnu
        if not typed and not (elements.dtype == torch.uint8 and scales.dtype == torch.uint8 and dtype == _l.EMB_MXFP4):
            raise TypeError("MXFP4 pair: torch.float4_e2m1fn_x2 elements with torch.float8_e8m0fnu scales, or two uint8 tensors "
                            f"with dtype=EMB_MXFP4; got {elements.dtype} and {scales.dtype}")
        el, sc = elements.contiguous().view(torch.uint8), scales.contiguous().view(torch.uint8)
        if el.dim() != 2 or sc.dim() != 2 or el.shape[0] != sc.shape[0] or sc.shape[1] == 0 or el.shape[1] != 16 * sc.shape[1] or el.device != sc.device:
            raise ValueError(f"MXFP4 pair: elements [rows, dim/2] and scales [rows, dim/32] on one device, got {tuple(el.shape)} and {tuple(sc.shape)}")
        pad = mxfp4_row_stride(2 * el.shape[1]) - el.shape[1] - sc.shape[1]
        return torch.cat([el, sc, torch.zeros((el.shape[0], pad), dtype=torch.uint8, device=el.device)], dim=1)

    def alloc_table(self, table_id: int, nr_rows: int, dim: int, dtype: int) -> None:
        _l.check(self._L.emb_alloc_table(self._h, table_id, nr_rows, dim, dtype))
        self._tables[table_id] = (nr_rows, dim, dtype)
        self._same_dim.clear()

    def load_table_column(self, table_id: int, col: int, column: np.ndarray) -> None:
        column = np.ascontiguousarray(column, dtype=np.int32)
        _l.check(self._L.emb_load_table_column(self._h, table_id, col, column.ctypes.data, column.shape[0]))

    def set_hot_rows(self, table_id: int, row_ids) -> None:
        ids = np.ascontiguousarray(row_ids, dtype=np.uint64)
        _l.check(self._L.emb_set_hot_rows(self._h, table_id, ids.ctypes.data_as(C.POINTER(C.c_uint64)), ids.shape[0]))

    def learn_hot_rows(self, table_id: int, indices, max_rows: int = 100, min_share: float = 0.05, stream: int | None = None):
        a = _Arg(indices)
        itype = _index_type_of(a.dtype)
        if stream is None and a.space == _l.EMB_MEM_DEVICE:
            stream = _current_stream_for(indices)
        n, sh = C.c_uint32(), C.c_float()
        _l.check(self._L.emb_learn_hot_rows(self._h, table_id, a.ptr, a.n, itype, a.space, int(max_rows), float(min_share), stream,
                                            C.byref(n), C.byref(sh)))
        return n.value, sh.value

    def table_tensor(self, table_id: int):
        import torch
        ptr, n, d, dt = self.table_info(table_id)
        if dt == _l.EMB_MXFP4:
            from .formats import mxfp4_row_stride
            d = mxfp4_row_stride(d)
        typestr = {_l.EMB_F32: "<f4", _l.EMB_F16: "<f2", _l.EMB_FIXED32: "<i4", _l.EMB_BF16: "<u2", _l.EMB_F8_E4M3: "|u1",
                   _l.EMB_F8_E5M2: "|u1", _l.EMB_MXFP4: "|u1"}[dt]

        class _View:
            __cuda_array_interface__ = {"shape": (n, d), "typestr": typestr, "data": (ptr, False), "version": 2,
                                        "strides": None}
        view = torch.as_tensor(_View(), device=torch.device("cuda", self.device))
        if dt in _F8_TORCH:
            return view.view(getattr(torch, _F8_TORCH[dt]))
        return view.view(torch.bfloat16) if dt == _l.EMB_BF16 else view

    def table_info(self, table_id: int):
        ptr, n, d, dt = C.c_void_p(), C.c_uint64(), C.c_uint32(), C.c_int()
        _l.check(self._L.emb_table_info(self._h, table_id, C.byref(ptr), C.byref(n), C.byref(d), C.byref(dt)))
        return ptr.value, n.value, d.value, dt.value

    def _alloc_out(self, like, n_bags: int, dim: int, half_of: int | None = None):
        np_dt = np.dtype(np.float32) if half_of is None else _HALF_OUT_NP[half_of]
        if isinstance(like, DeviceBuffer):
            return DeviceBuffer(self, n_bags * dim * np_dt.itemsize, np_dt, (n_bags, dim))
        if _is_torch(like):
            import torch
            dt = torch.float32 if half_of is None else (torch.float16 if half_of == _l.EMB_F16 else torch.bfloat16)
            return torch.empty((n_bags, dim), dtype=dt, device=like.device)
        return np.empty((n_bags, dim), dtype=np_dt)

    def _descs(self, table_ids, indices, offsets, outs, fixed_pooling, want_outputs=True, half=None):
        n = len(table_ids)
        if not (len(indices) == n and len(offsets) == n):
            raise ValueError("table_ids, indices and offsets must have equal length")
        if half is not None:
            for t, h in zip(table_ids, half):
                if h and t in self._tables and self._tables[t][2] == _l.EMB_MXFP4:
                    raise TypeError(f'table {t}: out_dtype="table" needs an fp16 or bf16 table; an MXFP4 table returns fp32 rows only')
                if h and t in self._tables and self._tables[t][2] in _F8_TORCH:
                    raise TypeError(f'table {t}: out_dtype="table" needs an fp16 or bf16 table; an fp8 table ({_F8_TORCH[self._tables[t][2]]}) '
                                    "returns fp32 rows only")
        arr = (_l.EmbLookupDesc * n)()
        keep, results = [], []
        itype = space = None
        for i, t in enumerate(table_ids):
            if t not in self._tables:
                raise KeyError(f"table {t} is not loaded")
            ia, oa = _Arg(indices[i]), _Arg(offsets[i])
            L = 0
            if oa.ptr is None:
                L = int(fixed_pooling[i] if isinstance(fixed_pooling, (list, tuple)) else fixed_pooling or 0)
                if L <= 0:
                    raise ValueError("offsets=None needs fixed_pooling > 0")
                n_bags = ia.n // L
            else:
                n_bags = oa.n
                if _index_type_of(oa.dtype) != _index_type_of(ia.dtype) or oa.space != ia.space:
                    raise TypeError("indices and offsets must share dtype width and placement")
            it = _index_type_of(ia.dtype)
            if itype is None:
                itype, space = it, ia.space
            elif it != itype or ia.space != space:
                raise TypeError("all tables of one batched lookup must share index width and placement")
            out_ptr = None
            if want_outputs:
                dim, tdt = self._tables[t][1], self._tables[t][2]
                half_of = tdt if half is not None and half[i] and tdt in _HALF_OUT_NP else None
                out = outs[i] if outs is not None else self._alloc_out(indices[i], n_bags, dim, half_of)
                ua = _Arg(out)
                if half_of is not None and outs is not None:
                    _check_half_out(out, half_of, t)
                if ua.space != space:
                    raise TypeError("output placement must match the inputs")
                out_ptr = ua.ptr
                keep.append(ua.keep)
                results.append(out)
            arr[i] = _l.EmbLookupDesc(t, L, ia.ptr, oa.ptr, ia.n, n_bags, out_ptr)
            keep += [ia.keep, oa.keep]
        return arr, n, itype, space, results, keep

    _DESC = struct.Struct("<IIQQQQQ")

    def _drop_plans(self) -> None:
        with self._plan_lock:
            for plan, _ in self._plan_cache.values():
                plan.destroy()
            self._plan_cache.clear()
            self._plan_seen.clear()

    def _desc_slot(self, n: int):
        try:
            bufs = self._tls.bufs
        except AttributeError:
            bufs = self._tls.bufs = {}
        slot = bufs.get(n)
        if slot is None:
            raw = C.create_string_buffer(self._DESC.size * n)
            slot = bufs[n] = (raw, C.cast(raw, C.POINTER(_l.EmbLookupDesc)), C.addressof(raw))
        return slot

    def _launch_cached(self, key, stream) -> bool:
        if self._check_inputs:
            return False
        with self._plan_lock:
            self._plan_clock += 1
            ent = self._plan_cache.get(key)
            if ent is None:
                return False
            if self._L.emb_plan_launch(ent[0]._p, stream) == _l.EMB_OK:
                ent[1] = self._plan_clock
                self.plan_cache_hits += 1
                return True
            ent[0].destroy()
            del self._plan_cache[key]
            return False

    def _raise_range(self, bad):
        raise IndexError(f"{bad} index / offset value(s) out of range for the embedding table(s) "
                         "(checked on the GPU before anything was launched)")

    def _checked_call(self, arr, n, itype, space, stream, check) -> None:
        if check == "deferred" and space == _l.EMB_MEM_DEVICE:
            rc = self._L.emb_lookup_batched_checked_deferred(self._h, arr, n, itype, space, stream)
            if rc == _l.EMB_ERR_RANGE:
                raise IndexError(self._L.emb_last_error().decode(errors="replace"))
            _l.check(rc)
            return
        bad = C.c_uint64()
        rc = self._L.emb_lookup_batched_checked(self._h, arr, n, itype, space, stream, C.byref(bad))
        if rc == _l.EMB_ERR_RANGE:
            if "EARLIER" in self._L.emb_last_error().decode(errors="replace"):
                raise IndexError(self._L.emb_last_error().decode(errors="replace"))
            self._raise_range(bad.value)
        _l.check(rc)

    def check_report(self) -> None:
        bad = C.c_uint64()
        rc = self._L.emb_check_report(self._h, C.byref(bad))
        if rc == _l.EMB_ERR_RANGE:
            raise IndexError(self._L.emb_last_error().decode(errors="replace"))
        _l.check(rc)

    def _lookup_batched_marshal(self, tb, table_ids, indices, offsets, outs, stream, check):
        import torch
        n = len(table_ids)
        _raw, buf_ptr, addr = self._desc_slot(n)
        r = tb.pack(addr, table_ids, indices, offsets, outs, self._tables)
        if r is None:
            return None
        itype, _dev, d0, nbs, key, cur_stream = r
        if outs is None:
            if not d0:
                return None
            one = torch.empty((sum(nbs), d0), dtype=torch.float32, device=indices[0].device)
            key = tb.fill_pooled(addr, n, one.data_ptr(), d0)
            res = list(one.split(nbs))
        else:
            res = list(outs)
        if stream is None:
            stream = cur_stream
        if check:
            self._checked_call(buf_ptr, n, itype, _l.EMB_MEM_DEVICE, stream, check)
            return res
        if self.plan_cache_size:
            key = (key, itype)
            if self._launch_cached(key, stream):
                return res
        _l.check(self._L.emb_lookup_batched(self._h, buf_ptr, n, itype, _l.EMB_MEM_DEVICE, stream))
        if self.plan_cache_size:
            self._remember_call(key, buf_ptr, n, itype)
        return res

    def _lookup_batched_cuda(self, table_ids, indices, offsets, outs, stream, check=False):
        import torch
        tb = _marshal()
        if tb is not None and type(table_ids) is list and type(indices) is list and type(offsets) is list:
            res = self._lookup_batched_marshal(tb, table_ids, indices, offsets, outs, stream, check)
            if res is not None:
                return res
        n = len(table_ids)
        i0 = indices[0]
        if type(i0) is not torch.Tensor or not i0.is_cuda or len(indices) != n or len(offsets) != n:
            return None
        dt, dev, tables = i0.dtype, i0.device, self._tables
        if dt is torch.int64:
            itype = _l.EMB_IDX_I64
        elif dt is torch.int32:
            itype = _l.EMB_IDX_U32
        else:
            return None
        if stream is None:
            stream = torch.cuda.current_stream(dev).cuda_stream
        key = one_buffer = None
        if self.plan_cache_size and not check:
            try:
                ptr = torch.Tensor.data_ptr
                ids_t = tuple(table_ids)
                nbs = tuple(map(len, offsets))
                if outs is None:
                    d0 = self._same_dim.get(ids_t)
                    if d0 is None:
                        ds = {tables[t][1] for t in table_ids}
                        d0 = self._same_dim[ids_t] = ds.pop() if len(ds) == 1 else 0
                    if d0:
                        one_buffer = torch.empty((sum(nbs), d0), dtype=torch.float32, device=dev)
                        out_key = one_buffer.data_ptr()
                else:
                    out_key = tuple(map(ptr, outs))
                if outs is not None or one_buffer is not None:
                    key = (ids_t, tuple(map(ptr, indices)), tuple(map(ptr, offsets)), tuple(map(len, indices)), nbs,
                           dt, offsets[0].dtype, dev.index, out_key)
            except (TypeError, KeyError):
                key = None
        if key is not None and self._launch_cached(key, stream):
            return list(one_buffer.split(nbs)) if outs is None else list(outs)
        buf, buf_ptr, _addr = self._desc_slot(n)
        pack, size = self._DESC.pack_into, self._DESC.size
        nbs, dims = [], []
        for t, ia, oa in zip(table_ids, indices, offsets):
            if type(ia) is not torch.Tensor or type(oa) is not torch.Tensor or ia.dtype is not dt or oa.dtype is not dt \
                    or ia.device != dev or oa.device != dev or not ia.is_contiguous() or not oa.is_contiguous() \
                    or ia.dim() != 1 or oa.dim() != 1:
                return None
            nbs.append(oa.numel())
            dims.append(tables[t][1])
        if outs is None:
            d0 = dims[0]
            if one_buffer is not None:
                outs = one_buffer.split(nbs)
            elif all(d == d0 for d in dims):
                outs = torch.empty((sum(nbs), d0), dtype=torch.float32, device=dev).split(nbs)
            else:
                outs = [torch.empty((b, d), dtype=torch.float32, device=dev) for b, d in zip(nbs, dims)]
        else:
            for o, b, d in zip(outs, nbs, dims):
                if type(o) is not torch.Tensor or o.device != dev or o.dtype is not torch.float32 \
                        or not o.is_contiguous() or o.numel() != b * d:
                    return None
        off = 0
        for t, ia, oa, b, o in zip(table_ids, indices, offsets, nbs, outs):
            pack(buf, off, t, 0, ia.data_ptr(), oa.data_ptr(), ia.numel(), b, o.data_ptr())
            off += size
        if check:
            self._checked_call(buf_ptr, n, itype, _l.EMB_MEM_DEVICE, stream, check)
            return list(outs)
        _l.check(self._L.emb_lookup_batched(self._h, buf_ptr, n, itype, _l.EMB_MEM_DEVICE, stream))
        if key is not None:
            self._remember_call(key, buf_ptr, n, itype)
        return list(outs)

    def _remember_call(self, key, desc_ptr, n, itype, pools=None) -> None:
        with self._plan_lock:
            self._remember_locked(key, desc_ptr, n, itype, pools)

    def _remember_locked(self, key, desc_ptr, n, itype, pools=None) -> None:
        if key in self._plan_cache or self._check_inputs:
            return
        h = hash(key)
        if self._plan_seen.pop(h, 0) < 1:
            if len(self._plan_seen) >= 4096:
                for old in list(self._plan_seen)[:2048]:
                    del self._plan_seen[old]
            self._plan_seen[h] = 1
            return
        if len(self._plan_cache) >= self.plan_cache_size:
            if self._plan_clock - self._plan_last_evict < 64:
                return
            self._plan_last_evict = self._plan_clock
            victim = min(self._plan_cache, key=lambda k: self._plan_cache[k][1])
            self._plan_cache.pop(victim)[0].destroy()
        p = C.c_void_p()
        rc = (self._L.emb_plan_create(self._h, desc_ptr, n, itype, C.byref(p)) if pools is None else
              self._L.emb_plan_create_pooled(self._h, desc_ptr, pools, n, itype, C.byref(p)))
        if rc != _l.EMB_OK:
            return
        self._plan_cache[key] = [Plan(self, p.value, None, None), self._plan_clock]

    _DESC_DT = np.dtype([("table_id", "<u4"), ("fixed_pooling", "<u4"), ("indices", "<u8"), ("offsets", "<u8"),
                         ("n_indices", "<u8"), ("n_bags", "<u8"), ("pooled", "<u8")])

    def lookup_stacked(self, table_ids: Sequence[int], indices, offsets, out=None, stream: int | None = None,
                       check: bool = False):
        import torch
        T = len(table_ids)
        if indices.dim() != 2 or offsets.dim() != 2 or indices.shape[0] != T or offsets.shape[0] != T:
            raise ValueError("indices must be [T, N] and offsets [T, B]")
        if not (indices.is_cuda and offsets.is_cuda and indices.is_contiguous() and offsets.is_contiguous()):
            raise ValueError("lookup_stacked needs contiguous CUDA tensors")
        if indices.dtype != offsets.dtype:
            raise TypeError("indices and offsets must share dtype width")
        itype = _index_type_of(indices.dtype)
        key = tuple(table_ids)
        try:
            stacked = self._tls.stacked
        except AttributeError:
            stacked = self._tls.stacked = {}
        cached = stacked.get(key)
        if cached is None:
            dims = {self._tables[t][1] for t in table_ids}
            if len(dims) != 1:
                raise ValueError("lookup_stacked needs tables of one dim")
            arr = np.zeros(T, dtype=self._DESC_DT)
            arr["table_id"] = np.asarray(table_ids, dtype=np.uint32)
            cached = stacked[key] = (arr, np.arange(T, dtype=np.uint64), dims.pop(),
                                           C.cast(arr.ctypes.data, C.POINTER(_l.EmbLookupDesc)))
        arr, steps, dim, arr_ptr = cached
        N, B = indices.shape[1], offsets.shape[1]
        if out is None:
            out = torch.empty((T, B, dim), dtype=torch.float32, device=indices.device)
        elif tuple(out.shape) != (T, B, dim) or not out.is_contiguous() or out.dtype != torch.float32:
            raise ValueError("out must be a contiguous float32 [T, B, dim] tensor")
        if stream is None:
            stream = torch.cuda.current_stream(indices.device).cuda_stream
        i_ptr, o_ptr, out_ptr = indices.data_ptr(), offsets.data_ptr(), out.data_ptr()
        pkey = None
        if self.plan_cache_size and not check:
            pkey = ("stacked", key, i_ptr, o_ptr, out_ptr, N, B, itype)
            if self._launch_cached(pkey, stream):
                return out
        esz = indices.element_size()
        arr["indices"] = i_ptr + steps * np.uint64(N * esz)
        arr["offsets"] = o_ptr + steps * np.uint64(B * esz)
        arr["pooled"] = out_ptr + steps * np.uint64(B * dim * 4)
        arr["n_indices"] = N
        arr["n_bags"] = B
        if check:
            self._checked_call(arr_ptr, T, itype, _l.EMB_MEM_DEVICE, stream, check)
            return out
        _l.check(self._L.emb_lookup_batched(self._h, arr_ptr, T, itype, _l.EMB_MEM_DEVICE, stream))
        if pkey is not None:
            self._remember_call(pkey, arr_ptr, T, itype)
        return out

    def lookup_descs(self, descs: np.ndarray, itype: int = _l.EMB_IDX_U32, stream: int | None = None) -> None:
        if descs.dtype != self._DESC_DT or not descs.flags["C_CONTIGUOUS"]:
            raise TypeError("descs must be a contiguous array of EmbeddingEngine._DESC_DT records")
        _l.check(self._L.emb_lookup_batched(self._h, C.cast(descs.ctypes.data, C.POINTER(_l.EmbLookupDesc)), len(descs),
                                            itype, _l.EMB_MEM_DEVICE, stream))

    def lookup_batched(self, table_ids: Sequence[int], indices: Sequence, offsets: Sequence,
                       outs: Sequence | None = None, fixed_pooling=0, stream: int | None = None, check: bool | str = False,
                       out_dtype=None):
        if _half_out_list(out_dtype, len(table_ids), outs) is not None:
            return self.lookup_pooled(table_ids, indices, offsets, "sum", outs=outs, fixed_pooling=fixed_pooling, stream=stream,
                                      check=check, out_dtype=out_dtype)
        if not fixed_pooling and len(table_ids) and _is_torch(indices[0]):
            res = self._lookup_batched_cuda(table_ids, indices, offsets, outs, stream, check)
            if res is not None:
                return res
        arr, n, itype, space, results, _keep = self._descs(table_ids, indices, offsets, outs, fixed_pooling)
        if stream is None and space == _l.EMB_MEM_DEVICE:
            stream = _current_stream_for(*indices)
        if check:
            self._checked_call(arr, n, itype, space, stream, check)
            return results
        _l.check(self._L.emb_lookup_batched(self._h, arr, n, itype, space, stream))
        return results

    def lookup(self, table_id: int, indices, offsets, out=None, fixed_pooling: int = 0,
               stream: int | None = None, check: bool = False, out_dtype=None):
        return self.lookup_batched([table_id], [indices], [offsets], None if out is None else [out],
                                   fixed_pooling, stream, check, out_dtype)[0]

    def plan(self, table_ids, indices, offsets, outs=None, fixed_pooling=0, modes=None, per_sample_weights=None,
             padding_idx=None, out_dtype=None) -> Plan:
        if modes is not None or per_sample_weights is not None or padding_idx is not None or out_dtype is not None:
            return self.plan_pooled(table_ids, indices, offsets, "sum" if modes is None else modes, per_sample_weights, padding_idx,
                                    outs, fixed_pooling, out_dtype)
        arr, n, itype, space, results, keep = self._descs(table_ids, indices, offsets, outs, fixed_pooling)
        if space != _l.EMB_MEM_DEVICE:
            raise TypeError("plans need device-resident buffers (torch CUDA tensors or DeviceBuffer)")
        p = C.c_void_p()
        _l.check(self._L.emb_plan_create(self._h, arr, n, itype, C.byref(p)))
        return Plan(self, p.value, results, keep)

    def _pools(self, n, descs, modes, per_sample_weights, padding_idx, space, half=None):
        def per_table(v, what):
            if v is None or isinstance(v, (str, int, np.integer)):
                return [v] * n
            v = list(v)
            if len(v) != n:
                raise ValueError(f"{what}: one entry per table expected ({n}), got {len(v)}")
            return v
        modes, weights, pads = per_table(modes, "modes"), per_table(per_sample_weights, "per_sample_weights"), \
            per_table(padding_idx, "padding_idx")
        arr = (_l.EmbPoolSpec * n)()
        keep = []
        for i in range(n):
            m = modes[i]
            mode = POOL_MODES[m] if isinstance(m, str) else int(m if m is not None else _l.EMB_POOL_SUM)
            wptr = None
            if weights[i] is not None:
                w = weights[i]
                if _is_torch(w):
                    if str(w.dtype) != "torch.float32":
                        raise TypeError("per_sample_weights must be float32")
                elif not isinstance(w, DeviceBuffer):
                    w = np.ascontiguousarray(w, dtype=np.float32)
                wa = _Arg(w)
                if wa.space != space:
                    raise TypeError("per_sample_weights must be placed like the indices")
                if wa.n != descs[i].n_indices:
                    raise ValueError(f"table {descs[i].table_id}: {wa.n} per_sample_weights for {descs[i].n_indices} indices")
                wptr = wa.ptr
                keep.append(wa.keep)
            flags, pad = (0, 0) if pads[i] is None else (_l.EMB_POOL_PADDING, int(pads[i]))
            if half is not None and half[i]:
                flags |= _l.EMB_POOL_OUT_TABLE_DTYPE
            arr[i] = _l.EmbPoolSpec(mode, flags, wptr, pad)
        return arr, keep

    def lookup_pooled(self, table_ids: Sequence[int], indices: Sequence, offsets: Sequence, modes, per_sample_weights=None,
                      padding_idx=None, outs: Sequence | None = None, fixed_pooling=0, stream: int | None = None,
                      check: bool | str = False, out_dtype=None):
        half = _half_out_list(out_dtype, len(table_ids), outs)
        arr, n, itype, space, results, keep = self._descs(table_ids, indices, offsets, outs, fixed_pooling, half=half)
        pools, pkeep = self._pools(n, arr, modes, per_sample_weights, padding_idx, space, half)
        if stream is None and space == _l.EMB_MEM_DEVICE:
            stream = _current_stream_for(*indices)
        c = 0 if not check else (2 if check == "deferred" else 1)
        key = None
        if c == 0 and space == _l.EMB_MEM_DEVICE and self.plan_cache_size:
            key = ("pooled", bytes(arr), bytes(pools), itype)
            if self._launch_cached(key, stream):
                return results
        bad = C.c_uint64()
        rc = self._L.emb_lookup_pooled(self._h, arr, pools, n, itype, space, stream, c, C.byref(bad))
        if rc == _l.EMB_ERR_RANGE:
            text = self._L.emb_last_error().decode(errors="replace")
            if c == 2 or "EARLIER" in text:
                raise IndexError(text)
            self._raise_range(bad.value)
        _l.check(rc)
        if key is not None:
            self._remember_call(key, arr, n, itype, pools)
        return results

    def plan_pooled(self, table_ids, indices, offsets, modes, per_sample_weights=None, padding_idx=None, outs=None,
                    fixed_pooling=0, out_dtype=None) -> Plan:
        half = _half_out_list(out_dtype, len(table_ids), outs)
        arr, n, itype, space, results, keep = self._descs(table_ids, indices, offsets, outs, fixed_pooling, half=half)
        if space != _l.EMB_MEM_DEVICE:
            raise TypeError("plans need device-resident buffers (torch CUDA tensors or DeviceBuffer)")
        pools, pkeep = self._pools(n, arr, modes, per_sample_weights, padding_idx, space, half)
        p = C.c_void_p()
        _l.check(self._L.emb_plan_create_pooled(self._h, arr, pools, n, itype, C.byref(p)))
        return Plan(self, p.value, results, keep + pkeep)

    def validate(self, table_ids, indices, offsets, fixed_pooling=0) -> int:
        arr, n, itype, space, _r, _k = self._descs(table_ids, indices, offsets, None, fixed_pooling,
                                                   want_outputs=False)
        bad = C.c_uint64()
        stream = _current_stream_for(*indices) if space == _l.EMB_MEM_DEVICE else None
        rc = self._L.emb_validate_inputs_on(self._h, arr, n, itype, space, stream, C.byref(bad))
        if rc not in (_l.EMB_OK, _l.EMB_ERR_RANGE):
            _l.check(rc)
        return bad.value

    def route_bags_sizes(self, n_tables: int, n_bags: int, total_indices: int, n_shards: int) -> dict:
        v = [C.c_uint64() for _ in range(4)]
        _l.check(self._L.emb_route_bags_sizes(n_tables, n_bags, total_indices, n_shards, *[C.byref(x) for x in v]))
        return dict(zip(("send", "meta", "slots", "work"), (x.value for x in v)))

    def route_bags(self, tables, n_bags: int, n_shards: int, send_ptr: int, meta_ptr: int, slots_ptr: int,
                   work_ptr: int, stream: int | None = None, itype: int = _l.EMB_IDX_U32) -> None:
        arr = tables if isinstance(tables, C.Array) else self.route_tables(tables)
        _l.check(self._L.emb_route_bags_typed(self._h, arr, len(arr), itype, n_bags, n_shards, send_ptr, meta_ptr, slots_ptr,
                                              work_ptr, stream))

    @staticmethod
    def route_tables(tables):
        arr = (_l.EmbRouteTable * len(tables))()
        for k, (ip, op, n, L, rps) in enumerate(tables):
            arr[k] = _l.EmbRouteTable(ip, op, int(n), int(L), int(rps))
        return arr

    def route_exchange_sizes(self, counts_host_ptr: int, n_tables: int, n_shards: int, dim: int):
        N = n_shards
        buf = self._tls.__dict__.get("xsz")
        if buf is None or len(buf[0]) != 4 * N:
            buf = self._tls.xsz = ((C.c_uint64 * (4 * N))(), C.c_uint64(), C.c_uint64())
        arr, pr, pt = buf
        base = C.addressof(arr)
        _l.check(self._L.emb_route_exchange_sizes(counts_host_ptr, counts_host_ptr + 8 * N * (n_tables + 1), n_tables, N, dim,
                                                  base, base + 8 * N, base + 16 * N, base + 24 * N, C.byref(pr), C.byref(pt)))
        v = arr[:]
        return v[:N], v[N:2 * N], v[2 * N:3 * N], v[3 * N:], pr.value, pt.value

    def lookup_served(self, received_host_ptr: int, n_tables: int, n_shards: int, dim: int, shard_table_ids,
                      req_recv_ptr: int, ret_send_ptr: int, stream: int | None = None) -> int:
        key = (n_tables, n_shards)
        cache = self._tls.__dict__.get("served")
        if cache is None or cache[0] != key or cache[1] != tuple(shard_table_ids):
            ids = (C.c_uint32 * n_tables)(*[int(x) for x in shard_table_ids])
            cache = self._tls.served = (key, tuple(shard_table_ids), ids, (_l.EmbLookupDesc * (n_tables * n_shards))(),
                                        C.c_uint32(), C.c_uint64())
        _k, _ids_t, ids, descs, n, nbytes = cache
        _l.check(self._L.emb_route_serve_descs(received_host_ptr, n_tables, n_shards, dim, ids, req_recv_ptr, ret_send_ptr,
                                               descs, C.byref(n), C.byref(nbytes)))
        if n.value:
            _l.check(self._L.emb_lookup_batched(self._h, descs, n.value, _l.EMB_IDX_U32, _l.EMB_MEM_DEVICE, stream))
        return nbytes.value

    def unroute_bags(self, recv_ptr: int, meta_ptr: int, slots_ptr: int, n_tables: int, n_bags: int, n_shards: int,
                     dim: int, pooled_ptr: int, stream: int | None = None) -> None:
        _l.check(self._L.emb_unroute_bags(self._h, recv_ptr, meta_ptr, slots_ptr, n_tables, n_bags, n_shards, dim,
                                          pooled_ptr, stream))

    def stats(self) -> dict:
        s = _l.EmbStats()
        _l.check(self._L.emb_get_stats(self._h, C.byref(s)))
        d = {k: getattr(s, k) for k, _ in s._fields_}
        d["n_launches_by_kind"] = list(d["n_launches_by_kind"])
        return d

    def reset_stats(self) -> None:
        _l.check(self._L.emb_reset_stats(self._h))

    def synchronize(self, stream: int | None = None) -> None:
        _l.check(self._L.emb_synchronize(self._h, stream))

    @property
    def device(self) -> int:
        d = C.c_int32()
        _l.check(self._L.emb_device_of(self._h, C.byref(d)))
        return d.value

    def close(self) -> None:
        if self._h:
            self._drop_plans()
            pending = None
            try:
                self.check_report()
            except (IndexError, _l.PimembError) as ex:
                pending = ex
            _l.check(self._L.emb_destroy(self._h))
            self._h = None
            if pending is not None:
                raise pending

    def __enter__(self):
        return self

    def __exit__(self, *exc):
        self.close()
```

pim-embedding-lookup_amd/lib.py:

```python
from __future__ import annotations

import ctypes as C
import os

from .build import LIB_PATH

EMB_OK = 0
EMB_ERR_INVALID, EMB_ERR_NOMEM, EMB_ERR_DEVICE, EMB_ERR_UNSUPPORTED, EMB_ERR_RANGE = -1, -2, -3, -4, -5
EMB_F32, EMB_F16, EMB_FIXED32, EMB_BF16 = 0, 1, 2, 3
EMB_F8_E4M3, EMB_F8_E5M2 = 8, 9
EMB_MXFP4 = 10
EMB_IDX_U32, EMB_IDX_I64 = 0, 1
EMB_MEM_HOST, EMB_MEM_DEVICE = 0, 1
EMB_FLAG_STAGE_TIMING, EMB_FLAG_CHECK_INPUTS, EMB_FLAG_DEFER_CHECK = 1, 2, 4


class EmbConfig(C.Structure):
    _fields_ = [("device", C.c_int32), ("max_tables", C.c_uint32), ("flags", C.c_uint32)]


class EmbLookupDesc(C.Structure):
    _fields_ = [("table_id", C.c_uint32), ("fixed_pooling", C.c_uint32),
                ("indices", C.c_void_p), ("offsets", C.c_void_p),
                ("n_indices", C.c_uint64), ("n_bags", C.c_uint64), ("pooled", C.c_void_p)]


class EmbStats(C.Structure):
    _fields_ = [("n_lookup_calls", C.c_uint64), ("n_kernel_launches", C.c_uint64),
                ("n_bags", C.c_uint64), ("n_indices", C.c_uint64), ("table_bytes", C.c_uint64),
                ("us_copy_in_indices", C.c_double), ("us_copy_in_lengths", C.c_double),
                ("us_launch", C.c_double), ("us_copy_out", C.c_double),
                ("us_post_process", C.c_double), ("us_sync", C.c_double),
                ("n_launches_by_kind", C.c_uint64 * 5)]


class EmbRouteTable(C.Structure):
    _fields_ = [("indices", C.c_void_p), ("offsets", C.c_void_p), ("n_indices", C.c_uint64),
                ("fixed_pooling", C.c_uint32), ("rows_per_shard", C.c_uint32)]


class EmbCommOp(C.Structure):
    _fields_ = [("peer", C.c_int32), ("is_recv", C.c_int32), ("ptr", C.c_void_p), ("bytes", C.c_uint64)]


EMB_PLACE_REPLICATED, EMB_PLACE_WHOLE, EMB_PLACE_ROWS = 0, 1, 2
EMB_SHARD_SELF_VIA_COMM, EMB_SHARD_CHECK_SERVED, EMB_SHARD_PEER_STORES, EMB_SHARD_NO_DIRECT, EMB_SHARD_DEFER_REPORT = 1, 2, 4, 8, 16
EMB_RANGE_OPEN_END = 1 << 63
EMB_POOL_SUM, EMB_POOL_MEAN, EMB_POOL_MAX = 0, 1, 2
EMB_POOL_PADDING = 1
EMB_POOL_OUT_TABLE_DTYPE = 2


class EmbPoolSpec(C.Structure):
    _fields_ = [("mode", C.c_uint32), ("flags", C.c_uint32), ("per_sample_weights", C.c_void_p), ("padding_idx", C.c_int64)]


class EmbShardTable(C.Structure):
    _fields_ = [("placement", C.c_uint32), ("owner", C.c_int32), ("engine_table", C.c_uint32), ("rows_per_shard", C.c_uint32)]


class EmbShardInput(C.Structure):
    _fields_ = [("indices", C.c_void_p), ("offsets", C.c_void_p), ("n_indices", C.c_uint64), ("fixed_pooling", C.c_uint32),
                ("index_type", C.c_uint32), ("pooled", C.c_void_p)]


class EmbShardConfig(C.Structure):
    _fields_ = [("n_tables", C.c_uint32), ("dim", C.c_uint32), ("depth", C.c_uint32), ("flags", C.c_uint32),
                ("tables", C.POINTER(EmbShardTable)), ("peer", C.c_void_p)]


class EmbShardStats(C.Structure):
    _fields_ = [("n_batches", C.c_uint64), ("bytes_to_peers", C.c_uint64), ("bytes_to_self", C.c_uint64),
                ("served_algorithmic_bytes", C.c_uint64), ("local_algorithmic_bytes", C.c_uint64),
                ("served_sub_bags", C.c_uint64), ("served_indices", C.c_uint64),
                ("us_host_submit", C.c_double), ("us_host_wait_counts", C.c_double), ("us_host_wait_served", C.c_double),
                ("us_kernel_route", C.c_double), ("us_kernel_local", C.c_double), ("us_kernel_serve", C.c_double),
                ("us_kernel_unroute", C.c_double), ("n_timed_batches", C.c_uint64), ("us_kernel_direct", C.c_double)]


class EmbTraceEvent(C.Structure):
    _fields_ = [("stage", C.c_uint32), ("call_id", C.c_uint32), ("start_us", C.c_double), ("stop_us", C.c_double)]


class DpuRuntimeTotals(C.Structure):
    _fields_ = [("execution_time_prepare", C.c_double),
                ("execution_time_populate_copy_in", C.c_double),
                ("execution_time_copy_in", C.c_double), ("execution_time_copy_out", C.c_double),
                ("execution_time_aggregate_result", C.c_double), ("execution_time_launch", C.c_double)]


_vp, _u32, _u64, _i32, _sz = C.c_void_p, C.c_uint32, C.c_uint64, C.c_int32, C.c_size_t
_pp = C.POINTER(C.c_void_p)

SIGNATURES = {
    "emb_last_error": (C.c_char_p, []),
    "emb_version": (C.c_char_p, []),
    "emb_create": (C.c_int, [C.POINTER(EmbConfig), _pp]),
    "emb_destroy": (C.c_int, [_vp]),
    "emb_load_table": (C.c_int, [_vp, _u32, _u64, _u32, C.c_int, _vp, C.c_int]),
    "emb_alloc_table": (C.c_int, [_vp, _u32, _u64, _u32, C.c_int]),
    "emb_load_table_column": (C.c_int, [_vp, _u32, _u32, _vp, _u64]),
    "emb_set_hot_rows": (C.c_int, [_vp, _u32, C.POINTER(_u64), _u32]),
    "emb_learn_hot_rows": (C.c_int, [_vp, _u32, _vp, _u64, C.c_int, C.c_int, _u32, C.c_float, _vp, C.POINTER(_u32), C.POINTER(C.c_float)]),
    "emb_comm_unique_id": (C.c_int, [_vp]),
    "emb_comm_create": (C.c_int, [_vp, _vp, C.c_int32, C.c_int32, _pp]),
    "emb_comm_all_to_all": (C.c_int, [_vp, _vp, C.POINTER(_u64), _vp, C.POINTER(_u64), _vp]),
    "emb_comm_destroy": (C.c_int, [_vp]),
    "emb_comm_exchange": (C.c_int, [_vp, C.POINTER(EmbCommOp), _u32, _vp]),
    "emb_comm_rank": (C.c_int, [_vp, C.POINTER(_i32), C.POINTER(_i32)]),
    "emb_peer_create": (C.c_int, [_vp, C.c_char_p, C.c_int32, C.c_int32, _u64, _pp]),
    "emb_peer_alloc": (C.c_int, [_vp, _u64, _pp]),
    "emb_peer_info": (C.c_int, [_vp, C.POINTER(_i32), C.POINTER(_i32), _pp, C.POINTER(_u64), C.POINTER(_u64), C.POINTER(_i32)]),
    "emb_peer_barrier": (C.c_int, [_vp]),
    "emb_peer_destroy": (C.c_int, [_vp]),
    "emb_peer_last_words": (C.c_int, [C.c_char_p, C.c_int, C.c_int]),
    "emb_shard_create": (C.c_int, [_vp, _vp, C.POINTER(EmbShardConfig), _pp]),
    "emb_shard_submit": (C.c_int, [_vp, C.POINTER(EmbShardInput), _u64, _vp, C.POINTER(_u64)]),
    "emb_shard_flush": (C.c_int, [_vp]),
    "emb_shard_wait": (C.c_int, [_vp, _u64, _vp]),
    "emb_shard_lookup": (C.c_int, [_vp, C.POINTER(EmbShardInput), _u64, _vp]),
    "emb_shard_report": (C.c_int, [_vp]),
    "emb_shard_get_stats": (C.c_int, [_vp, C.POINTER(EmbShardStats), C.c_int]),
    "emb_shard_set_kernel_timing": (C.c_int, [_vp, C.c_int]),
    "emb_shard_sent_counts": (C.c_int, [_vp, _u64, C.POINTER(_u32), _u32]),
    "emb_shard_destroy": (C.c_int, [_vp]),
    "emb_table_info": (C.c_int, [_vp, _u32, _pp, C.POINTER(_u64), C.POINTER(_u32), C.POINTER(C.c_int)]),
    "emb_lookup": (C.c_int, [_vp, _u32, _vp, _u64, _vp, _u64, _vp, C.c_int, C.c_int, _vp]),
    "emb_lookup_batched": (C.c_int, [_vp, C.POINTER(EmbLookupDesc), _u32, C.c_int, C.c_int, _vp]),
    "emb_queue_create": (C.c_int, [_vp, C.c_int, C.c_int, _pp]),
    "emb_queue_add": (C.c_int, [_vp, C.POINTER(EmbLookupDesc), _u32, C.POINTER(_u64)]),
    "emb_queue_add_many": (C.c_int, [_vp, C.POINTER(EmbLookupDesc), C.POINTER(_u32), _u32, C.POINTER(_u64)]),
    "emb_queue_flush": (C.c_int, [_vp, _vp, C.POINTER(_u32)]),
    "emb_queue_wait": (C.c_int, [_vp, _u64]),
    "emb_queue_destroy": (C.c_int, [_vp]),
    "emb_lookup_ranged": (C.c_int, [_vp, C.POINTER(EmbLookupDesc), C.POINTER(_u64), _u32, _vp]),
    "emb_plan_create_ranged": (C.c_int, [_vp, C.POINTER(EmbLookupDesc), C.POINTER(_u64), _u32, C.POINTER(_vp)]),
    "emb_lookup_ranged_counted": (C.c_int, [_vp, C.POINTER(EmbLookupDesc), C.POINTER(_u64), C.POINTER(_vp), _u32, _vp]),
    "emb_plan_create_ranged_counted": (C.c_int, [_vp, C.POINTER(EmbLookupDesc), C.POINTER(_u64), C.POINTER(_vp), _u32, C.POINTER(_vp)]),
    "emb_lookup_ranged_typed": (C.c_int, [_vp, C.POINTER(EmbLookupDesc), C.POINTER(_u64), C.POINTER(_vp), _u32, C.c_int, _vp]),
    "emb_plan_create_ranged_typed": (C.c_int, [_vp, C.POINTER(EmbLookupDesc), C.POINTER(_u64), C.POINTER(_vp), _u32, C.c_int, C.POINTER(_vp)]),
    "emb_plan_create": (C.c_int, [_vp, C.POINTER(EmbLookupDesc), _u32, C.c_int, _pp]),
    "emb_lookup_pooled": (C.c_int, [_vp, C.POINTER(EmbLookupDesc), C.POINTER(EmbPoolSpec), _u32, C.c_int, C.c_int, _vp, _u32,
                                    C.POINTER(_u64)]),
    "emb_plan_create_pooled": (C.c_int, [_vp, C.POINTER(EmbLookupDesc), C.POINTER(EmbPoolSpec), _u32, C.c_int, _pp]),
    "emb_plan_launch": (C.c_int, [_vp, _vp]),
    "emb_plan_destroy": (C.c_int, [_vp]),
    "emb_plan_bytes": (C.c_int, [_vp, C.POINTER(_u64), C.POINTER(_u64), C.POINTER(_u64)]),
    "emb_plan_signature": (C.c_int, [_vp, C.POINTER(_u64)]),
    "emb_plan_describe": (C.c_int, [_vp, C.c_char_p, _sz]),
    "emb_plan_time": (C.c_int, [_vp, _vp, _u32, _u32, C.POINTER(C.c_float)]),
    "emb_validate_inputs": (C.c_int, [_vp, C.POINTER(EmbLookupDesc), _u32, C.c_int, C.c_int,
                                      C.POINTER(_u64)]),
    "emb_validate_inputs_on": (C.c_int, [_vp, C.POINTER(EmbLookupDesc), _u32, C.c_int, C.c_int, _vp,
                                         C.POINTER(_u64)]),
    "emb_lookup_batched_checked": (C.c_int, [_vp, C.POINTER(EmbLookupDesc), _u32, C.c_int, C.c_int, _vp,
                                             C.POINTER(_u64)]),
    "emb_lookup_batched_checked_deferred": (C.c_int, [_vp, C.POINTER(EmbLookupDesc), _u32, C.c_int, C.c_int, _vp]),
    "emb_check_report": (C.c_int, [_vp, C.POINTER(_u64)]),
    "emb_get_stats": (C.c_int, [_vp, C.POINTER(EmbStats)]),
    "emb_reset_stats": (C.c_int, [_vp]),
    "emb_set_stage_timing": (C.c_int, [_vp, C.c_int]),
    "emb_trace_enable": (C.c_int, [_vp, _u32]),
    "emb_trace_read": (C.c_int, [_vp, C.POINTER(EmbTraceEvent), _u32, C.POINTER(_u32)]),
    "emb_device_alloc": (C.c_int, [_vp, _sz, _pp]),
    "emb_device_free": (C.c_int, [_vp, _vp]),
    "emb_copy_to_device": (C.c_int, [_vp, _vp, _vp, _sz]),
    "emb_copy_to_host": (C.c_int, [_vp, _vp, _vp, _sz]),
    "emb_memset_device": (C.c_int, [_vp, _vp, C.c_int, _sz]),
    "emb_synchronize": (C.c_int, [_vp, _vp]),
    "emb_stream_create": (C.c_int, [_vp, _pp]),
    "emb_stream_destroy": (C.c_int, [_vp, _vp]),
    "emb_device_of": (C.c_int, [_vp, C.POINTER(_i32)]),
    "emb_route_bags_sizes": (C.c_int, [_u32, _u64, _u64, _u32, C.POINTER(_u64), C.POINTER(_u64), C.POINTER(_u64),
                                       C.POINTER(_u64)]),
    "emb_route_bags": (C.c_int, [_vp, C.POINTER(EmbRouteTable), _u32, _u64, _u32, _vp, _vp, _vp, _vp, _vp]),
    "emb_route_bags_typed": (C.c_int, [_vp, C.POINTER(EmbRouteTable), _u32, C.c_int, _u64, _u32, _vp, _vp, _vp, _vp, _vp]),
    "emb_unroute_bags": (C.c_int, [_vp, _vp, _vp, _vp, _u32, _u64, _u32, _u32, _vp, _vp]),
    "emb_route_exchange_sizes": (C.c_int, [_vp, _vp, _u32, _u32, _u32, _vp, _vp, _vp, _vp, C.POINTER(_u64),
                                           C.POINTER(_u64)]),
    "emb_route_serve_descs": (C.c_int, [_vp, _u32, _u32, _u32, _vp, _vp, _vp, C.POINTER(EmbLookupDesc), C.POINTER(_u32),
                                        C.POINTER(_u64)]),
    "emb_configure": (C.c_int, [_u32, _u32, _u32, _u32]),
    "populate_mram": (_vp, [_u32, _u64, _u32, _vp, C.POINTER(DpuRuntimeTotals)]),
    "lookup": (_vp, [_pp, _pp, _pp, _vp, C.c_int64]),
    "emb_compat_engine": (_vp, []),
    "emb_compat_reset": (C.c_int, []),
}

_lib = None


class PimembError(RuntimeError):
    def __init__(self, code: int, text: str):
        super().__init__(f"pimemb error {code}: {text}")
        self.code = code


def load(path: str | None = None) -> C.CDLL:
    global _lib
    if _lib is not None and path is None:
        return _lib
    p = path or LIB_PATH
    if not os.path.exists(p):
        raise FileNotFoundError(
            f"{p} not found: build it with `python -c 'import __graft_entry__ as g; g.build()'` "
            "(hipcc --offload-arch=gfx950).  There is no fallback path.")
    try:
        import torch
    except ImportError:
        pass
    L = C.CDLL(p)
    for name, (res, args) in SIGNATURES.items():
        fn = getattr(L, name)
        fn.restype = res
        fn.argtypes = args
    if path is None:
        _lib = L
    return L


def check(rc: int) -> None:
    if rc != EMB_OK:
        raise PimembError(rc, load().emb_last_error().decode(errors="replace"))
```

Measured before the change: 51.44 billion.

## Learn hot rows automatically from sampled lookup indices and refresh plans

Adds an on-by-default automatic hot-row mechanism. On the first executions it asynchronously copies sampled index runs to the host. Once those copies finish, it counts the most frequent rows, stages up to 32 of them into device hot-row buffers (served from LDS by the HOT kernel), and bumps an epoch so cached plans re-resolve onto the hot-row kernel. The aim is to cut HBM gathers for skewed Kaggle tables. In exchange it adds host-side sampling and sorting, device-to-host copies and plan re-resolution, plus extra locking on the hot path.

```diff
diff --git a/include/pimemb.h b/include/pimemb.h
--- a/include/pimemb.h
+++ b/include/pimemb.h
@@ -45,6 +45,8 @@
 #define EMB_FLAG_STAGE_TIMING 1u
 #define EMB_FLAG_CHECK_INPUTS 2u
 #define EMB_FLAG_DEFER_CHECK 4u
+
+#define EMB_FLAG_NO_AUTO_HOT_ROWS 8u
 
 typedef struct emb_lookup_desc {
     uint32_t table_id;
@@ -91,6 +93,18 @@
 int emb_set_hot_rows(emb_engine *e, uint32_t table_id, const uint64_t *row_ids, uint32_t n_rows);
 int emb_learn_hot_rows(emb_engine *e, uint32_t table_id, const void *indices, uint64_t n_indices, emb_index_type itype,
                        emb_memspace space, uint32_t max_rows, float min_share, void *stream, uint32_t *n_chosen, float *share);
+
+int emb_set_auto_hot_rows(emb_engine *e, int on);
+typedef struct emb_auto_hot_stats {
+    uint64_t enabled;
+    uint64_t n_tables_learnt;
+    uint64_t n_tables_none;
+    uint64_t n_samples;
+    uint64_t n_plan_reresolves;
+} emb_auto_hot_stats;
+int emb_get_auto_hot_stats(emb_engine *e, emb_auto_hot_stats *out);
+int emb_pick_hot_rows(const void *sample, uint64_t n_sample, emb_index_type itype, uint64_t nr_rows, uint32_t max_rows, float min_share,
+                      uint64_t *row_ids, uint32_t *n_chosen, float *share);
 
 int emb_table_info(emb_engine *e, uint32_t table_id, void **device_rows, uint64_t *nr_rows,
                    uint32_t *dim, emb_dtype *dtype);
diff --git a/pim-embedding-lookup_amd/csrc/pimemb_engine.cpp b/pim-embedding-lookup_amd/csrc/pimemb_engine.cpp
--- a/pim-embedding-lookup_amd/csrc/pimemb_engine.cpp
+++ b/pim-embedding-lookup_amd/csrc/pimemb_engine.cpp
@@ -67,7 +67,13 @@
     uint64_t *hot_hash = nullptr;
     uint32_t n_hot = 0, hot_log2 = 0;
     size_t hot_lds = 0;
+    uint8_t auto_state = 0;
+    uint32_t auto_token = 0;
+    uint64_t hot_generation = 0;
 };
+enum : uint8_t { kAutoOpen = 0, kAutoSampling = 1, kAutoLearnt = 2, kAutoNone = 3, kAutoExplicit = 4 };
+constexpr uint32_t kAutoHotRows = 32;
+constexpr float kAutoMinShare = 0.05f;
 
 struct DescSlot {
     char *h = nullptr;
@@ -171,6 +177,22 @@
     bool check_inputs = false;
     std::atomic<uint32_t> live_plans{0};
     uint64_t next_generation = 1;
+    struct AutoSample {
+        uint32_t table, token;
+        size_t off;
+        uint64_t n;
+    };
+    struct AutoBatch {
+        char *h = nullptr;
+        hipEvent_t ev = nullptr;
+        emb_index_type itype = EMB_IDX_U32;
+        std::vector<AutoSample> items;
+    };
+    std::atomic<bool> auto_hot{true};
+    std::vector<AutoBatch> auto_batches;
+    std::atomic<uint32_t> auto_inflight{0};
+    std::atomic<uint64_t> hot_epoch{0};
+    std::atomic<uint64_t> n_auto_learnt{0}, n_auto_none{0}, n_auto_samples{0}, n_plan_reresolves{0};
     std::deque<emb_trace_event> trace;
     uint32_t trace_cap = 0;
     uint32_t host_call_id = 0;
@@ -202,14 +224,32 @@
     std::vector<uint32_t> xmap_words;
 };
 
+struct AutoCand {
+    uint32_t table = 0;
+    const void *indices = nullptr;
+    uint64_t n_indices = 0;
+};
+
+struct PlanImage {
+    std::vector<PlanGroup> groups;
+    char *d_image = nullptr;
+    uint64_t signature = 0;
+    std::atomic<uint64_t> hot_epoch{0};
+};
+
 struct emb_plan {
     emb_engine *e = nullptr;
     emb_index_type itype = EMB_IDX_U32;
-    std::vector<PlanGroup> groups;
-    char *d_image = nullptr;
+    std::atomic<PlanImage *> image{nullptr};
     uint64_t bytes = 0, n_bags = 0, n_indices = 0;
-    uint64_t signature = 0;
     std::vector<std::pair<uint32_t, uint64_t>> table_gens;
+    std::mutex swap_mu;
+    std::vector<PlanImage *> retired;
+    std::vector<emb_lookup_desc> descs;
+    std::vector<emb_pool_spec> pools;
+    std::vector<std::pair<uint32_t, uint64_t>> table_hot_gens;
+    std::vector<AutoCand> auto_cands;
+    std::atomic<bool> auto_open{false};
 };
 
 namespace {
@@ -236,12 +276,160 @@
     }
 };
 
+hipError_t stage_hot_rows(Table &t, const uint64_t *row_ids, uint32_t n_rows) {
+    if (n_rows == 0 || t.geom.scalar_lanes) return hipSuccess;
+    const uint32_t row_bytes = t.geom.chunks * 16u;
+    pimemb::HotSet hs = pimemb::build_hot_set(row_ids, n_rows, t.nr_rows, row_bytes, pimemb::kHotLdsBudget);
+    if (hs.rows.empty()) return hipSuccess;
+    hipError_t err = hipMalloc(&t.hot_rows, hs.rows.size() * (size_t)row_bytes);
+    if (err == hipSuccess) err = hipMalloc((void **)&t.hot_hash, hs.hash.size() * 8);
+    {
+        unsigned long long *d_ids = nullptr;
+        std::vector<unsigned long long> ids(hs.rows.begin(), hs.rows.end());
+        if (err == hipSuccess) err = hipMalloc((void **)&d_ids, ids.size() * 8);
+        if (err == hipSuccess) err = hipMemcpy(d_ids, ids.data(), ids.size() * 8, hipMemcpyHostToDevice);
+        if (err == hipSuccess) err = pimemb::launch_gather_rows(t.hot_rows, t.rows, d_ids, (uint32_t)ids.size(), row_bytes, nullptr);
+        if (err == hipSuccess) err = hipStreamSynchronize(nullptr);
+        if (d_ids) (void)hipFree(d_ids);
+    }
+    if (err == hipSuccess) err = hipMemcpy(t.hot_hash, hs.hash.data(), hs.hash.size() * 8, hipMemcpyHostToDevice);
+    if (err != hipSuccess) {
+        clear_hot(t);
+        return err;
+    }
+    t.n_hot = (uint32_t)hs.rows.size();
+    t.hot_log2 = hs.log2size;
+    t.hot_lds = hs.lds_bytes(row_bytes);
+    return hipSuccess;
+}
+
+
+#pragma weak hipStreamIsCapturing
+bool stream_is_capturing(hipStream_t s) {
+    if (!hipStreamIsCapturing) return false;
+    hipStreamCaptureStatus st = hipStreamCaptureStatusNone;
+    if (hipStreamIsCapturing(s, &st) != hipSuccess) {
+        (void)hipGetLastError();
+        return false;
+    }
+    return st != hipStreamCaptureStatusNone;
+}
+
+void auto_drop_batch(emb_engine::AutoBatch &b) {
+    if (b.ev) (void)hipEventDestroy(b.ev);
+    if (b.h) (void)hipHostFree(b.h);
+    b = emb_engine::AutoBatch{};
+}
+
+void auto_reset(Table &t, uint8_t state = kAutoOpen) {
+    t.auto_state = state;
+    t.auto_token++;
+}
+
+bool auto_hot_sample(emb_engine *e, const std::vector<AutoCand> &cands, emb_index_type itype, hipStream_t s) {
+    if (cands.empty() || !e->auto_hot.load(std::memory_order_relaxed)) return false;
+    std::lock_guard<std::mutex> lk(e->mu);
+    const size_t isz = index_size(itype);
+    emb_engine::AutoBatch b;
+    b.itype = itype;
+    size_t bytes = 0;
+    for (const AutoCand &c : cands) {
+        Table &t = e->tables[c.table];
+        bool twice = false;
+        for (const emb_engine::AutoSample &it : b.items) twice = twice || it.table == c.table;
+        if (t.auto_state != kAutoOpen || !t.rows || twice) continue;
+        const pimemb::HotSampleRuns runs(c.n_indices);
+        b.items.push_back(emb_engine::AutoSample{c.table, t.auto_token, bytes, runs.n_sample()});
+        bytes += (size_t)runs.n_sample() * isz;
+    }
+    if (b.items.empty()) return false;
+    if (stream_is_capturing(s)) return true;
+    hipError_t err = hipHostMalloc((void **)&b.h, bytes, hipHostMallocDefault);
+    if (err == hipSuccess) err = hipEventCreateWithFlags(&b.ev, hipEventDisableTiming);
+    for (size_t k = 0, ci = 0; k < b.items.size() && err == hipSuccess; k++) {
+        while (cands[ci].table != b.items[k].table) ci++;
+        const pimemb::HotSampleRuns runs(cands[ci].n_indices);
+        for (uint64_t r = 0; r < runs.runs && err == hipSuccess; r++)
+            err = hipMemcpyAsync(b.h + b.items[k].off + (size_t)(r * runs.len) * isz,
+                                 static_cast<const char *>(cands[ci].indices) + runs.run_start(r) * isz, (size_t)runs.len * isz,
+                                 hipMemcpyDeviceToHost, s);
+    }
+    if (err == hipSuccess) err = hipEventRecord(b.ev, s);
+    if (err != hipSuccess) {
+        (void)hipGetLastError();
+        (void)hipStreamSynchronize(s);
+        for (const emb_engine::AutoSample &it : b.items) auto_reset(e->tables[it.table], kAutoNone);
+        auto_drop_batch(b);
+        return false;
+    }
+    for (const emb_engine::AutoSample &it : b.items) e->tables[it.table].auto_state = kAutoSampling;
+    e->n_auto_samples.fetch_add(b.items.size(), std::memory_order_relaxed);
+    e->auto_batches.push_back(std::move(b));
+    e->auto_inflight.store((uint32_t)e->auto_batches.size(), std::memory_order_release);
+    return false;
+}
+
+void auto_hot_poll(emb_engine *e, hipStream_t s) {
+    if (e->auto_inflight.load(std::memory_order_acquire) == 0) return;
+    if (stream_is_capturing(s)) return;
+    std::lock_guard<std::mutex> lk(e->mu);
+    bool changed = false;
+    size_t kept = 0;
+    for (size_t bi = 0; bi < e->auto_batches.size(); bi++) {
+        emb_engine::AutoBatch &b = e->auto_batches[bi];
+        if (hipEventQuery(b.ev) != hipSuccess) {
+            (void)hipGetLastError();
+            if (kept != bi) e->auto_batches[kept] = std::move(b);
+            kept++;
+            continue;
+        }
+        std::vector<const emb_engine::AutoSample *> live;
+        for (const emb_engine::AutoSample &it : b.items) {
+            const Table &t = e->tables[it.table];
+            if (t.rows && t.auto_state == kAutoSampling && t.auto_token == it.token) live.push_back(&it);
+        }
+        std::vector<pimemb::HotPick> picks(live.size());
+        {
+            const size_t n_threads = std::min<size_t>(live.size(), 8);
+            std::atomic<size_t> next{0};
+            auto work = [&] {
+                for (size_t k = next.fetch_add(1); k < live.size(); k = next.fetch_add(1))
+                    picks[k] = pimemb::pick_hot_rows(b.h + live[k]->off, live[k]->n, b.itype == EMB_IDX_I64, e->tables[live[k]->table].nr_rows,
+                                                     kAutoHotRows, kAutoMinShare);
+            };
+            std::vector<std::thread> pool;
+            for (size_t k = 1; k < n_threads; k++) pool.emplace_back(work);
+            work();
+            for (std::thread &th : pool) th.join();
+        }
+        for (size_t k = 0; k < live.size(); k++) {
+            Table &t = e->tables[live[k]->table];
+            hipError_t err = picks[k].ids.empty() ? hipSuccess : stage_hot_rows(t, picks[k].ids.data(), (uint32_t)picks[k].ids.size());
+            if (err != hipSuccess) (void)hipGetLastError();
+            if (t.n_hot) {
+                t.auto_state = kAutoLearnt;
+                t.hot_generation++;
+                changed = true;
+                e->n_auto_learnt.fetch_add(1, std::memory_order_relaxed);
+            } else {
+                t.auto_state = kAutoNone;
+                e->n_auto_none.fetch_add(1, std::memory_order_relaxed);
+            }
+        }
+        auto_drop_batch(b);
+    }
+    e->auto_batches.resize(kept);
+    if (changed) e->hot_epoch.fetch_add(1, std::memory_order_release);
+    e->auto_inflight.store((uint32_t)kept, std::memory_order_release);
+}
+
 struct Resolved {
     std::vector<DevDesc> descs;
     std::vector<PlanGroup> groups;
     uint64_t bytes = 0, n_bags = 0, n_indices = 0;
     std::vector<char> image;
     hipStream_t stream = nullptr;
+    std::vector<AutoCand> auto_cands;
 
     void build_image() {
         size_t off = 0, di = 0;
@@ -470,10 +658,25 @@
         g.ranged = row_lo != nullptr;
         if (g.ranged && g.kind == pimemb::KERNEL_GROUP) g.kind = pimemb::KERNEL_WAVEBATCH;
         if (g.pool && g.kind == pimemb::KERNEL_WAVEBATCH2) g.kind = pimemb::KERNEL_WAVEBATCH;
+        struct HotView {
+            const void *rows = nullptr;
+            const uint64_t *hash = nullptr;
+            uint32_t n = 0, log2 = 0;
+        };
+        std::vector<HotView> hot_of;
         if (g.kind == pimemb::KERNEL_GROUP && !g.pool && !g.out_half) {
-            for (uint32_t i : kv.second) {
-                const Table &t = e->tables[descs[i].table_id];
-                if (t.n_hot && t.hot_lds > g.hot_lds) g.hot_lds = (uint32_t)t.hot_lds;
+            const bool learns = e->auto_hot.load(std::memory_order_relaxed) && !st_indices && group_idx > 2 * group_bags && !g.geom.scalar_lanes &&
+                                (g.dtype == EMB_F32 || g.dtype == EMB_F16 || g.dtype == EMB_BF16);
+            std::lock_guard<std::mutex> lk(e->mu);
+            hot_of.resize(kv.second.size());
+            for (size_t k = 0; k < kv.second.size(); k++) {
+                const emb_lookup_desc &u = descs[kv.second[k]];
+                const Table &t = e->tables[u.table_id];
+                if (t.n_hot) {
+                    hot_of[k] = HotView{t.hot_rows, t.hot_hash, t.n_hot, t.hot_log2};
+                    if (t.hot_lds > g.hot_lds) g.hot_lds = (uint32_t)t.hot_lds;
+                }
+                if (learns && t.auto_state == kAutoOpen && u.n_indices > 2 * u.n_bags) r->auto_cands.push_back(AutoCand{u.table_id, u.indices, u.n_indices});
             }
             if (g.hot_lds) g.kind = pimemb::KERNEL_HOT;
         }
@@ -512,10 +715,11 @@
                 if (weighted) r->bytes += u.n_indices * 4;
             }
             if (g.kind == pimemb::KERNEL_HOT) {
-                d.hot_rows = t.hot_rows;
-                d.hot_hash = t.hot_hash;
-                d.n_hot = t.n_hot;
-                d.hot_log2 = t.hot_log2;
+                const HotView &hv = hot_of[tiles_of.size()];
+                d.hot_rows = hv.rows;
+                d.hot_hash = hv.hash;
+                d.n_hot = hv.n;
+                d.hot_log2 = hv.log2;
             }
             if (d.n_tiles > g.max_tiles) g.max_tiles = d.n_tiles;
             tiles_of.push_back(d.n_tiles);
@@ -1008,6 +1212,10 @@
     e->check_inputs = cfg && (cfg->flags & EMB_FLAG_CHECK_INPUTS);
     e->defer_check = cfg && (cfg->flags & EMB_FLAG_DEFER_CHECK);
     {
+        const char *a = getenv("PIMEMB_AUTO_HOT_ROWS");
+        e->auto_hot.store(!(cfg && (cfg->flags & EMB_FLAG_NO_AUTO_HOT_ROWS)) && !(a && atoi(a) == 0));
+    }
+    {
         const char *m = getenv("PIMEMB_DESC_MODE");
         for (ImageRing &rg : e->ring) {
             rg.desc_mode = (m && m[0] == 'c') ? 0 : 1;
@@ -1046,6 +1254,7 @@
         clear_hot(t);
         if (t.rows) (void)hipFree(t.rows);
     }
+    for (emb_engine::AutoBatch &b : e->auto_batches) auto_drop_batch(b);
     for (ImageRing &rg : e->ring) rg.release();
     for (XmapCacheEntry &c : e->xmap_cache) (void)hipFree(c.d_map);
     for (XmapGrave &gv : e->xmap_graveyard) {
@@ -1090,11 +1299,15 @@
         clear_hot(t);
         t.generation = e->next_generation++;
     }
+    if (t.auto_state != kAutoOpen) e->hot_epoch.fetch_add(1, std::memory_order_release);
+    auto_reset(t);
     if (t.rows && t.bytes != bytes) {
         HIP_TRY(hipDeviceSynchronize());
         HIP_TRY(hipFree(t.rows));
         e->table_bytes -= t.bytes;
+        const uint32_t token = t.auto_token;
         t = Table{};
+        t.auto_token = token;
     }
     if (!t.rows) {
         HIP_TRY(hipMalloc(&t.rows, bytes));
@@ -1149,6 +1362,7 @@
         clear_hot(t);
         t.generation = e->next_generation++;
     }
+    auto_reset(t);
     size_t bytes = nr_rows * sizeof(int32_t);
     int rc = ensure_stage(e, bytes, bytes);
     if (rc) return rc;
@@ -1175,30 +1389,36 @@
     HIP_TRY(hipDeviceSynchronize());
     clear_hot(t);
     t.generation = e->next_generation++;
-    if (n_rows == 0) return EMB_OK;
-    if (t.geom.scalar_lanes) return EMB_OK;
-    const uint32_t row_bytes = t.geom.chunks * 16u;
-    pimemb::HotSet hs = pimemb::build_hot_set(row_ids, n_rows, t.nr_rows, row_bytes, pimemb::kHotLdsBudget);
-    if (hs.rows.empty()) return EMB_OK;
-    HIP_TRY(hipMalloc(&t.hot_rows, hs.rows.size() * (size_t)row_bytes));
-    hipError_t err = hipMalloc((void **)&t.hot_hash, hs.hash.size() * 8);
-    {
-        unsigned long long *d_ids = nullptr;
-        std::vector<unsigned long long> ids(hs.rows.begin(), hs.rows.end());
-        if (err == hipSuccess) err = hipMalloc((void **)&d_ids, ids.size() * 8);
-        if (err == hipSuccess) err = hipMemcpy(d_ids, ids.data(), ids.size() * 8, hipMemcpyHostToDevice);
-        if (err == hipSuccess) err = pimemb::launch_gather_rows(t.hot_rows, t.rows, d_ids, (uint32_t)ids.size(), row_bytes, nullptr);
-        if (err == hipSuccess) err = hipStreamSynchronize(nullptr);
-        if (d_ids) (void)hipFree(d_ids);
-    }
-    if (err == hipSuccess) err = hipMemcpy(t.hot_hash, hs.hash.data(), hs.hash.size() * 8, hipMemcpyHostToDevice);
-    if (err != hipSuccess) {
-        clear_hot(t);
-        return fail(EMB_ERR_DEVICE, "emb_set_hot_rows: %s", hipGetErrorString(err));
-    }
-    t.n_hot = (uint32_t)hs.rows.size();
-    t.hot_log2 = hs.log2size;
-    t.hot_lds = hs.lds_bytes(row_bytes);
+    auto_reset(t, kAutoExplicit);
+    const hipError_t err = stage_hot_rows(t, row_ids, n_rows);
+    if (err != hipSuccess) return fail(err == hipErrorOutOfMemory ? EMB_ERR_NOMEM : EMB_ERR_DEVICE, "emb_set_hot_rows: %s", hipGetErrorString(err));
+    return EMB_OK;
+}
+
+int emb_set_auto_hot_rows(emb_engine *e, int on) {
+    if (!e) return fail(EMB_ERR_INVALID, "engine is NULL");
+    e->auto_hot.store(on != 0);
+    return EMB_OK;
+}
+
+int emb_get_auto_hot_stats(emb_engine *e, emb_auto_hot_stats *out) {
+    if (!e || !out) return fail(EMB_ERR_INVALID, "engine or out is NULL");
+    out->enabled = e->auto_hot.load() ? 1 : 0;
+    out->n_tables_learnt = e->n_auto_learnt.load();
+    out->n_tables_none = e->n_auto_none.load();
+    out->n_samples = e->n_auto_samples.load();
+    out->n_plan_reresolves = e->n_plan_reresolves.load();
+    return EMB_OK;
+}
+
+int emb_pick_hot_rows(const void *sample, uint64_t n_sample, emb_index_type itype, uint64_t nr_rows, uint32_t max_rows, float min_share,
+                      uint64_t *row_ids, uint32_t *n_chosen, float *share) {
+    if (itype != EMB_IDX_U32 && itype != EMB_IDX_I64) return fail(EMB_ERR_INVALID, "bad index type");
+    if ((n_sample && !sample) || (max_rows && !row_ids) || !n_chosen) return fail(EMB_ERR_INVALID, "emb_pick_hot_rows: NULL argument");
+    const pimemb::HotPick pick = pimemb::pick_hot_rows(sample, n_sample, itype == EMB_IDX_I64, nr_rows, max_rows, min_share);
+    for (size_t i = 0; i < pick.ids.size(); i++) row_ids[i] = pick.ids[i];
+    *n_chosen = (uint32_t)pick.ids.size();
+    if (share) *share = pick.share;
     return EMB_OK;
 }
 
@@ -1212,51 +1432,24 @@
         return fail(EMB_ERR_UNSUPPORTED, "emb_learn_hot_rows: table %u is MXFP4, which has no hot-row kernel", table_id);
     if (n_chosen) *n_chosen = 0;
     if (share) *share = 0.f;
-    constexpr uint64_t kRun = 65536, kRuns = 4;
     const size_t isz = index_size(itype);
-    std::vector<char> host;
-    uint64_t n_sample = 0;
+    const pimemb::HotSampleRuns runs(n_indices);
+    std::vector<char> host((size_t)runs.n_sample() * isz);
     if (n_indices) {
         DeviceGuard g(e->device);
-        const uint64_t runs = n_indices <= kRun * kRuns ? 1 : kRuns;
-        const uint64_t len = runs == 1 ? n_indices : kRun;
-        host.resize((size_t)(runs * len) * isz);
         hipStream_t s = static_cast<hipStream_t>(stream);
-        for (uint64_t r = 0; r < runs; r++) {
-            const uint64_t at = runs == 1 ? 0 : r * ((n_indices - len) / (runs - 1));
-            const char *src = static_cast<const char *>(indices) + at * isz;
-            if (space == EMB_MEM_DEVICE) HIP_TRY(hipMemcpyAsync(host.data() + (size_t)(r * len) * isz, src, (size_t)len * isz, hipMemcpyDeviceToHost, s));
-            else memcpy(host.data() + (size_t)(r * len) * isz, src, (size_t)len * isz);
+        for (uint64_t r = 0; r < runs.runs; r++) {
+            const char *src = static_cast<const char *>(indices) + runs.run_start(r) * isz;
+            if (space == EMB_MEM_DEVICE) HIP_TRY(hipMemcpyAsync(host.data() + (size_t)(r * runs.len) * isz, src, (size_t)runs.len * isz, hipMemcpyDeviceToHost, s));
+            else memcpy(host.data() + (size_t)(r * runs.len) * isz, src, (size_t)runs.len * isz);
         }
         if (space == EMB_MEM_DEVICE) HIP_TRY(hipStreamSynchronize(s));
-        n_sample = runs * len;
-    }
-    const uint64_t nr_rows = e->tables[table_id].nr_rows;
-    std::unordered_map<uint64_t, uint32_t> count;
-    count.reserve((size_t)std::min<uint64_t>(n_sample, 1u << 20));
-    for (uint64_t i = 0; i < n_sample; i++) {
-        const uint64_t id = itype == EMB_IDX_I64 ? (uint64_t)reinterpret_cast<const int64_t *>(host.data())[i]
-                                                 : (uint64_t)reinterpret_cast<const uint32_t *>(host.data())[i];
-        if (id < nr_rows) count[id]++;
-    }
-    std::vector<std::pair<uint32_t, uint64_t>> by_count;
-    by_count.reserve(count.size());
-    for (const auto &kv : count) by_count.emplace_back(kv.second, kv.first);
-    const size_t k = std::min<size_t>(max_rows, by_count.size());
-    std::partial_sort(by_count.begin(), by_count.begin() + (long)k, by_count.end(),
-                      [](const std::pair<uint32_t, uint64_t> &a, const std::pair<uint32_t, uint64_t> &b) {
-                          return a.first != b.first ? a.first > b.first : a.second < b.second;
-                      });
-    uint64_t covered = 0;
-    std::vector<uint64_t> ids(k);
-    for (size_t i = 0; i < k; i++) {
-        ids[i] = by_count[i].second;
-        covered += by_count[i].first;
-    }
-    const float sh = n_sample ? (float)((double)covered / (double)n_sample) : 0.f;
-    if (share) *share = sh;
-    if (k == 0 || sh < min_share) return emb_set_hot_rows(e, table_id, nullptr, 0);
-    int rc = emb_set_hot_rows(e, table_id, ids.data(), (uint32_t)k);
+    }
+    const pimemb::HotPick pick = pimemb::pick_hot_rows(host.data(), runs.n_sample(), itype == EMB_IDX_I64, e->tables[table_id].nr_rows,
+                                                       max_rows, min_share);
+    if (share) *share = pick.share;
+    if (pick.ids.empty()) return emb_set_hot_rows(e, table_id, nullptr, 0);
+    int rc = emb_set_hot_rows(e, table_id, pick.ids.data(), (uint32_t)pick.ids.size());
     if (rc == EMB_OK && n_chosen) *n_chosen = e->tables[table_id].n_hot;
     return rc;
 }
@@ -1303,6 +1496,8 @@
     if (g_prof.on) g_prof.resolve += now_us() - p0;
     rc = check ? checked_launch(e, r, itype, s, true, n_bad, defer) : launch_resolved(e, r, itype, s);
     if (rc != EMB_OK && !(defer && rc == EMB_ERR_RANGE)) return rc;
+    auto_hot_poll(e, s);
+    if (!r.auto_cands.empty()) (void)auto_hot_sample(e, r.auto_cands, itype, s);
     e->n_bags.fetch_add(r.n_bags, std::memory_order_relaxed);
     e->n_indices.fetch_add(r.n_indices, std::memory_order_relaxed);
     return rc;
@@ -1417,19 +1612,10 @@
     return plan_create(e, descs, nullptr, nullptr, n_descs, itype, out, live_pools(pools, n_descs));
 }
 
-static int plan_create(emb_engine *e, const emb_lookup_desc *descs, const uint64_t *row_lo, uint32_t *const *served,
-                       uint32_t n_descs, emb_index_type itype, emb_plan **out, const emb_pool_spec *pools) {
-    if (!e || !out) return fail(EMB_ERR_INVALID, "engine or out is NULL");
-    *out = nullptr;
-    if (!descs || n_descs == 0) return fail(EMB_ERR_INVALID, "plan needs at least one descriptor");
-    DeviceGuard g(e->device);
-    Resolved r;
-    int rc = resolve(e, descs, n_descs, itype, nullptr, nullptr, nullptr, &r, false, row_lo, served, pools);
-    if (rc) return rc;
-    emb_plan *p = new (std::nothrow) emb_plan();
+static int plan_image_of(Resolved &r, emb_index_type itype, uint64_t epoch, PlanImage **out) {
+    PlanImage *p = new (std::nothrow) PlanImage();
     if (!p) return fail(EMB_ERR_NOMEM, "out of host memory");
-    p->e = e;
-    p->itype = itype;
+    p->hot_epoch.store(epoch, std::memory_order_relaxed);
     {
         uint64_t h = 1469598103934665603ull;
         auto mix = [&h](uint64_t v) { h = (h ^ v) * 1099511628211ull; };
@@ -1453,9 +1639,6 @@
         }
         p->signature = h;
     }
-    p->bytes = r.bytes;
-    p->n_bags = r.n_bags;
-    p->n_indices = r.n_indices;
     char *d = nullptr;
     hipError_t err = hipMalloc((void **)&d, r.image.size());
     if (err == hipSuccess) err = hipMemcpy(d, r.image.data(), r.image.size(), hipMemcpyHostToDevice);
@@ -1467,11 +1650,90 @@
     r.bind(d);
     p->d_image = d;
     p->groups = r.groups;
+    *out = p;
+    return EMB_OK;
+}
+
+static void hot_gens_of(emb_engine *e, const emb_lookup_desc *descs, uint32_t n_descs, std::vector<std::pair<uint32_t, uint64_t>> *out) {
+    std::lock_guard<std::mutex> lk(e->mu);
+    out->clear();
+    for (uint32_t i = 0; i < n_descs; i++)
+        if (descs[i].table_id < e->tables.size()) out->emplace_back(descs[i].table_id, e->tables[descs[i].table_id].hot_generation);
+}
+
+static int plan_create(emb_engine *e, const emb_lookup_desc *descs, const uint64_t *row_lo, uint32_t *const *served,
+                       uint32_t n_descs, emb_index_type itype, emb_plan **out, const emb_pool_spec *pools) {
+    if (!e || !out) return fail(EMB_ERR_INVALID, "engine or out is NULL");
+    *out = nullptr;
+    if (!descs || n_descs == 0) return fail(EMB_ERR_INVALID, "plan needs at least one descriptor");
+    DeviceGuard g(e->device);
+    const uint64_t epoch = e->hot_epoch.load(std::memory_order_acquire);
+    std::vector<std::pair<uint32_t, uint64_t>> hot_gens;
+    hot_gens_of(e, descs, n_descs, &hot_gens);
+    Resolved r;
+    int rc = resolve(e, descs, n_descs, itype, nullptr, nullptr, nullptr, &r, false, row_lo, served, pools);
+    if (rc) return rc;
+    emb_plan *p = new (std::nothrow) emb_plan();
+    if (!p) return fail(EMB_ERR_NOMEM, "out of host memory");
+    p->e = e;
+    p->itype = itype;
+    p->bytes = r.bytes;
+    p->n_bags = r.n_bags;
+    p->n_indices = r.n_indices;
+    PlanImage *im = nullptr;
+    rc = plan_image_of(r, itype, epoch, &im);
+    if (rc) {
+        delete p;
+        return rc;
+    }
+    p->image.store(im, std::memory_order_release);
     for (uint32_t i = 0; i < n_descs; i++)
         p->table_gens.emplace_back(descs[i].table_id, e->tables[descs[i].table_id].generation);
+    p->table_hot_gens.swap(hot_gens);
+    if (!row_lo) {
+        p->descs.assign(descs, descs + n_descs);
+        if (pools) p->pools.assign(pools, pools + n_descs);
+        p->auto_cands = r.auto_cands;
+        p->auto_open.store(!r.auto_cands.empty());
+    }
     e->live_plans.fetch_add(1);
     *out = p;
     return EMB_OK;
+}
+
+static PlanImage *plan_refresh(emb_plan *p) {
+    emb_engine *e = p->e;
+    std::lock_guard<std::mutex> swap_lk(p->swap_mu);
+    PlanImage *cur = p->image.load(std::memory_order_acquire);
+    const uint64_t epoch = e->hot_epoch.load(std::memory_order_acquire);
+    if (cur->hot_epoch.load(std::memory_order_acquire) == epoch) return cur;
+    std::vector<std::pair<uint32_t, uint64_t>> hot_gens;
+    hot_gens_of(e, p->descs.data(), (uint32_t)p->descs.size(), &hot_gens);
+    if (p->descs.empty() || hot_gens == p->table_hot_gens) {
+        if (!p->auto_cands.empty()) {
+            std::lock_guard<std::mutex> lk(e->mu);
+            for (const AutoCand &c : p->auto_cands)
+                if (e->tables[c.table].auto_state == kAutoOpen) p->auto_open.store(true);
+        }
+        cur->hot_epoch.store(epoch, std::memory_order_release);
+        return cur;
+    }
+    Resolved r;
+    PlanImage *im = nullptr;
+    int rc = resolve(e, p->descs.data(), (uint32_t)p->descs.size(), p->itype, nullptr, nullptr, nullptr, &r, false, nullptr, nullptr,
+                     p->pools.empty() ? nullptr : p->pools.data());
+    if (rc == EMB_OK) rc = plan_image_of(r, p->itype, epoch, &im);
+    if (rc != EMB_OK) {
+        cur->hot_epoch.store(epoch, std::memory_order_release);
+        return cur;
+    }
+    p->table_hot_gens.swap(hot_gens);
+    p->auto_cands = r.auto_cands;
+    p->auto_open.store(!r.auto_cands.empty());
+    p->retired.push_back(cur);
+    p->image.store(im, std::memory_order_release);
+    e->n_plan_reresolves.fetch_add(1, std::memory_order_relaxed);
+    return im;
 }
 
 int emb_plan_launch(emb_plan *p, void *stream) {
@@ -1481,8 +1743,20 @@
         if (e->tables[tg.first].generation != tg.second)
             return fail(EMB_ERR_INVALID, "plan is stale: table %u was re-allocated after emb_plan_create", tg.first);
     DeviceGuard g(e->device);
-    int rc = launch_groups(e, p->groups, p->itype, static_cast<hipStream_t>(stream));
+    hipStream_t s = static_cast<hipStream_t>(stream);
+    PlanImage *im = p->image.load(std::memory_order_acquire);
+    if (im->hot_epoch.load(std::memory_order_relaxed) != e->hot_epoch.load(std::memory_order_acquire)) im = plan_refresh(p);
+    int rc = launch_groups(e, im->groups, p->itype, s);
     if (rc) return rc;
+    auto_hot_poll(e, s);
+    if (p->auto_open.load(std::memory_order_relaxed)) {
+        std::vector<AutoCand> cands;
+        {
+            std::lock_guard<std::mutex> swap_lk(p->swap_mu);
+            cands = p->auto_cands;
+        }
+        if (!auto_hot_sample(e, cands, p->itype, s)) p->auto_open.store(false, std::memory_order_relaxed);
+    }
     e->n_lookup_calls.fetch_add(1, std::memory_order_relaxed);
     e->n_bags.fetch_add(p->n_bags, std::memory_order_relaxed);
     e->n_indices.fetch_add(p->n_indices, std::memory_order_relaxed);
@@ -1493,7 +1767,11 @@
     if (!p) return EMB_OK;
     DeviceGuard g(p->e->device);
     (void)hipDeviceSynchronize();
-    if (p->d_image) (void)hipFree(p->d_image);
+    p->retired.push_back(p->image.load());
+    for (PlanImage *im : p->retired) {
+        if (im && im->d_image) (void)hipFree(im->d_image);
+        delete im;
+    }
     p->e->live_plans.fetch_sub(1);
     delete p;
     return EMB_OK;
@@ -1512,7 +1790,7 @@
     if (!p || !buf || capacity == 0) return fail(EMB_ERR_INVALID, "emb_plan_describe: NULL argument");
     size_t at = 0;
     buf[0] = 0;
-    for (const PlanGroup &g : p->groups) {
+    for (const PlanGroup &g : p->image.load(std::memory_order_acquire)->groups) {
         const uint32_t block = g.kind == pimemb::KERNEL_ANYDIM ? 256u : (g.geom.lanes_per_row ? pimemb::bags_per_tile(g.kind, g.geom) : 0u);
         const int n = snprintf(buf + at, capacity - at, "%skind=%u dtype=%d itype=%d lanes_per_row=%u chunks=%u scalar_lanes=%u anydim_vec=%d ranged=%d descs=%u "
                                "grid=%u bags_per_tile=%u", at ? ";" : "", (unsigned)g.kind, (int)g.dtype, (int)p->itype, g.geom.lanes_per_row, g.geom.chunks,
@@ -1535,7 +1813,7 @@
 
 int emb_plan_signature(const emb_plan *p, uint64_t *signature) {
     if (!p || !signature) return fail(EMB_ERR_INVALID, "emb_plan_signature: NULL argument");
-    *signature = p->signature;
+    *signature = p->image.load(std::memory_order_acquire)->signature;
     return EMB_OK;
 }
 
diff --git a/pim-embedding-lookup_amd/csrc/pimemb_hot_rows.h b/pim-embedding-lookup_amd/csrc/pimemb_hot_rows.h
--- a/pim-embedding-lookup_amd/csrc/pimemb_hot_rows.h
+++ b/pim-embedding-lookup_amd/csrc/pimemb_hot_rows.h
@@ -2,6 +2,7 @@
 
 #include <stdint.h>
 
+#include <algorithm>
 #include <unordered_set>
 #include <vector>
 
@@ -48,4 +49,66 @@
     return hs;
 }
 
+struct HotPick {
+    std::vector<uint64_t> ids;
+    float share = 0.f;
+};
+
+inline HotPick pick_hot_rows(const void *sample, uint64_t n_sample, bool ids_are_i64, uint64_t nr_rows, uint32_t max_rows,
+                             float min_share) {
+    HotPick pick;
+    if (n_sample == 0 || max_rows == 0) return pick;
+    uint32_t log2 = 4;
+    while ((1ull << log2) < 2 * n_sample) log2++;
+    const uint64_t mask = (1ull << log2) - 1u;
+    std::vector<uint64_t> keys((size_t)1 << log2, ~0ull);
+    std::vector<uint32_t> counts((size_t)1 << log2, 0u);
+    size_t distinct = 0;
+    for (uint64_t i = 0; i < n_sample; i++) {
+        const uint64_t id = ids_are_i64 ? (uint64_t)static_cast<const int64_t *>(sample)[i]
+                                        : (uint64_t)static_cast<const uint32_t *>(sample)[i];
+        if (id >= nr_rows || id == ~0ull) continue;
+        uint64_t at = (id * 0x9E3779B97F4A7C15ull) >> (64u - log2);
+        while (keys[at] != id && keys[at] != ~0ull) at = (at + 1) & mask;
+        if (keys[at] == ~0ull) {
+            keys[at] = id;
+            distinct++;
+        }
+        counts[at]++;
+    }
+    struct Counted {
+        uint32_t count;
+        uint64_t id;
+    };
+    std::vector<Counted> by_count;
+    by_count.reserve(distinct);
+    for (size_t at = 0; at < keys.size(); at++)
+        if (counts[at]) by_count.push_back(Counted{counts[at], keys[at]});
+    const size_t k = max_rows < by_count.size() ? max_rows : by_count.size();
+    std::partial_sort(by_count.begin(), by_count.begin() + (long)k, by_count.end(), [](const Counted &a, const Counted &b) {
+        return a.count != b.count ? a.count > b.count : a.id < b.id;
+    });
+    uint64_t covered = 0;
+    pick.ids.resize(k);
+    for (size_t i = 0; i < k; i++) {
+        pick.ids[i] = by_count[i].id;
+        covered += by_count[i].count;
+    }
+    pick.share = (float)((double)covered / (double)n_sample);
+    if (k == 0 || pick.share < min_share) pick.ids.clear();
+    return pick;
 }
+
+struct HotSampleRuns {
+    static constexpr uint64_t kRun = 65536, kRuns = 4;
+    uint64_t runs = 0, len = 0, n_indices = 0;
+    explicit HotSampleRuns(uint64_t n) : n_indices(n) {
+        if (n == 0) return;
+        runs = n <= kRun * kRuns ? 1 : kRuns;
+        len = runs == 1 ? n : kRun;
+    }
+    uint64_t run_start(uint64_t r) const { return runs == 1 ? 0 : r * ((n_indices - len) / (runs - 1)); }
+    uint64_t n_sample() const { return runs * len; }
+};
+
+}
diff --git a/pim-embedding-lookup_amd/engine.py b/pim-embedding-lookup_amd/engine.py
--- a/pim-embedding-lookup_amd/engine.py
+++ b/pim-embedding-lookup_amd/engine.py
@@ -263,11 +263,13 @@
 class EmbeddingEngine:
 
     def __init__(self, device: int = -1, max_tables: int = 1024, lib_path: str | None = None,
-                 check_inputs: bool | str = False):
+                 check_inputs: bool | str = False, auto_hot_rows: bool | None = None):
         self._L = _l.load(lib_path)
         flags = _l.EMB_FLAG_CHECK_INPUTS if check_inputs else 0
         if check_inputs == "deferred":
             flags |= _l.EMB_FLAG_DEFER_CHECK
+        if auto_hot_rows is not None and not auto_hot_rows:
+            flags |= _l.EMB_FLAG_NO_AUTO_HOT_ROWS
         cfg = _l.EmbConfig(device, max_tables, flags)
         h = C.c_void_p()
         _l.check(self._L.emb_create(C.byref(cfg), C.byref(h)))
@@ -359,6 +361,14 @@
         _l.check(self._L.emb_learn_hot_rows(self._h, table_id, a.ptr, a.n, itype, a.space, int(max_rows), float(min_share), stream,
                                             C.byref(n), C.byref(sh)))
         return n.value, sh.value
+
+    def set_auto_hot_rows(self, on: bool) -> None:
+        _l.check(self._L.emb_set_auto_hot_rows(self._h, int(bool(on))))
+
+    def auto_hot_stats(self) -> dict:
+        s = _l.EmbAutoHotStats()
+        _l.check(self._L.emb_get_auto_hot_stats(self._h, C.byref(s)))
+        return {k: int(getattr(s, k)) for k, _ in s._fields_}
 
     def table_tensor(self, table_id: int):
         import torch
@@ -875,6 +885,7 @@
         _l.check(self._L.emb_get_stats(self._h, C.byref(s)))
         d = {k: getattr(s, k) for k, _ in s._fields_}
         d["n_launches_by_kind"] = list(d["n_launches_by_kind"])
+        d["auto_hot_rows"] = self.auto_hot_stats()
         return d
 
     def reset_stats(self) -> None:
diff --git a/pim-embedding-lookup_amd/lib.py b/pim-embedding-lookup_amd/lib.py
--- a/pim-embedding-lookup_amd/lib.py
+++ b/pim-embedding-lookup_amd/lib.py
@@ -13,6 +13,7 @@
 EMB_IDX_U32, EMB_IDX_I64 = 0, 1
 EMB_MEM_HOST, EMB_MEM_DEVICE = 0, 1
 EMB_FLAG_STAGE_TIMING, EMB_FLAG_CHECK_INPUTS, EMB_FLAG_DEFER_CHECK = 1, 2, 4
+EMB_FLAG_NO_AUTO_HOT_ROWS = 8
 
 
 class EmbConfig(C.Structure):
@@ -32,6 +33,11 @@
                 ("us_launch", C.c_double), ("us_copy_out", C.c_double),
                 ("us_post_process", C.c_double), ("us_sync", C.c_double),
                 ("n_launches_by_kind", C.c_uint64 * 5)]
+
+
+class EmbAutoHotStats(C.Structure):
+    _fields_ = [("enabled", C.c_uint64), ("n_tables_learnt", C.c_uint64), ("n_tables_none", C.c_uint64),
+                ("n_samples", C.c_uint64), ("n_plan_reresolves", C.c_uint64)]
 
 
 class EmbRouteTable(C.Structure):
@@ -102,6 +108,9 @@
     "emb_load_table_column": (C.c_int, [_vp, _u32, _u32, _vp, _u64]),
     "emb_set_hot_rows": (C.c_int, [_vp, _u32, C.POINTER(_u64), _u32]),
     "emb_learn_hot_rows": (C.c_int, [_vp, _u32, _vp, _u64, C.c_int, C.c_int, _u32, C.c_float, _vp, C.POINTER(_u32), C.POINTER(C.c_float)]),
+    "emb_set_auto_hot_rows": (C.c_int, [_vp, C.c_int]),
+    "emb_get_auto_hot_stats": (C.c_int, [_vp, C.POINTER(EmbAutoHotStats)]),
+    "emb_pick_hot_rows": (C.c_int, [_vp, _u64, C.c_int, _u64, _u32, C.c_float, C.POINTER(_u64), C.POINTER(_u32), C.POINTER(C.c_float)]),
     "emb_comm_unique_id": (C.c_int, [_vp]),
     "emb_comm_create": (C.c_int, [_vp, _vp, C.c_int32, C.c_int32, _pp]),
     "emb_comm_all_to_all": (C.c_int, [_vp, _vp, C.POINTER(_u64), _vp, C.POINTER(_u64), _vp]),
```

Result: no change. 51.44 billion (-0.0%).
